# we1pingyu/CALD

Hardware: AMD Instinct MI355X
Metric: unlabeled images scored/sec (CALD consistency sweep) (higher is better)
Workload: dtype f32

## Files before the change

### cald_amd/_ffi.py

```python
import ctypes as C
import os

_HERE = os.path.dirname(os.path.abspath(__file__))
LIB_PATH = os.path.join(_HERE, "lib", "libcaldhip.so")
_lib = None

c_f = C.POINTER(C.c_float)
c_i = C.POINTER(C.c_int)
c_i64 = C.POINTER(C.c_int64)
c_d = C.POINTER(C.c_double)
c_u8 = C.POINTER(C.c_uint8)
c_i8 = C.POINTER(C.c_int8)


class ModelCfg(C.Structure):
    _fields_ = [("arch", C.c_int), ("depth", C.c_int), ("num_classes", C.c_int), ("min_size", C.c_int),
                ("max_size", C.c_int), ("box_score_thresh", C.c_float), ("box_nms_thresh", C.c_float),
                ("detections_per_img", C.c_int), ("rpn_pre_nms_top_n", C.c_int), ("rpn_post_nms_top_n", C.c_int),
                ("rpn_nms_thresh", C.c_float), ("precision", C.c_int)]


PRECISION = {"fp32": 0, "f16x3": 1}


class View(C.Structure):
    _fields_ = [("image_dev", C.c_void_p), ("H", C.c_int), ("W", C.c_int), ("flip", C.c_int), ("nrect", C.c_int),
                ("rects", C.c_int * 16), ("noise_dev", C.c_void_p)]


class Dets(C.Structure):
    _fields_ = [("boxes_dev", C.c_void_p), ("scores_dev", C.c_void_p), ("labels_dev", C.c_void_p),
                ("props_dev", C.c_void_p), ("prob_max_dev", C.c_void_p), ("scores_cls_dev", C.c_void_p),
                ("count_dev", C.c_void_p), ("cap", C.c_int)]


MAX_AUGS = 32
N_MARGINS = 16
MARGIN_NAMES = ['rpn_topk', 'rpn_iou', 'rpn_order', 'rpn_trunc', 'rpn_small', 'roi_level', 'roi_edge', 'post_thr', 'post_iou', 'post_order',
                'post_cap', 'ref_subsample', 'argmax', 'zero_row', 'cutout', 'reserved']
MARGIN_NOISE_F16X3 = [2e-5, 2e-6, 2e-5, 2e-5, 1e-5, 1e-6, 1e-4, 5e-6, 2e-6, 5e-6, 5e-6, 5e-6, 2e-6, 5e-6, 2e-6, 0.0]
AUG_FLIP, AUG_GAUSS, AUG_COLOR_ADJUST, AUG_COLOR_SWAP, AUG_SALT_PEPPER, AUG_CUTOUT, AUG_RESIZE, AUG_ROTATE = range(1, 9)
MAX_NOISE_SEG = 16


class AugSpec(C.Structure):
    _fields_ = [("kind", C.c_int), ("param", C.c_double)]


class PackJob(C.Structure):
    _fields_ = [("weight", C.c_void_p), ("bias", C.c_void_p), ("bn_scale", C.c_void_p), ("bn_shift", C.c_void_p),
                ("Cout", C.c_int), ("Cin", C.c_int), ("KH", C.c_int), ("KW", C.c_int), ("CinK", C.c_int), ("mode", C.c_int),
                ("packed", C.c_void_p)]


class LLCfg(C.Structure):
    _fields_ = [("batch_views", C.c_int), ("levels", C.c_int * 4)]


class VaalCfg(C.Structure):
    _fields_ = [("bn_mode", C.c_int), ("batch_images", C.c_int)]


VAAL_BN_BATCH, VAAL_BN_RUNNING = 0, 1


class LossNetTensors(C.Structure):
    _fields_ = [("fc_w", C.c_void_p * 4), ("fc_b", C.c_void_p * 4), ("lin_w", C.c_void_p), ("lin_b", C.c_void_p)]


class SweepCfg(C.Structure):
    _fields_ = [("base_seed", C.c_uint64), ("bp", C.c_float), ("batch_images", C.c_int), ("n_augs", C.c_int),
                ("augs", AugSpec * MAX_AUGS)]


PROBE_MAX_VIEWS = 8
PROBE_MAX_RECTS = 8


class ConvProbe(C.Structure):
    _fields_ = [("V", C.c_int), ("in_hw", (C.c_int * 2) * PROBE_MAX_VIEWS), ("up_hw", (C.c_int * 2) * PROBE_MAX_VIEWS),
                ("dyn_rows", C.c_int * PROBE_MAX_VIEWS), ("has_dyn", C.c_int), ("gather", C.c_int), ("nrect", C.c_int * PROBE_MAX_VIEWS),
                ("rect", ((C.c_int * 4) * PROBE_MAX_RECTS) * PROBE_MAX_VIEWS),
                ("Cin", C.c_int), ("Cout", C.c_int), ("KH", C.c_int), ("KW", C.c_int), ("stride", C.c_int), ("pad", C.c_int),
                ("relu", C.c_int), ("in_relu", C.c_int), ("out_ld", C.c_int), ("cin_true", C.c_int),
                ("weight", c_f), ("bias", c_f), ("bn_scale", c_f), ("bn_shift", c_f), ("in_", c_f), ("in16", C.POINTER(C.c_uint32)),
                ("residual", c_f), ("up", c_f), ("ex16", C.c_int), ("mask", c_f), ("row_map", c_i),
                ("out", c_f), ("out_n", C.c_int64), ("out16", C.POINTER(C.c_uint32)), ("out16_n", C.c_int64),
                ("energy4", c_f), ("energy4_n", C.c_int64),
                ("head_w", c_f), ("head_b", c_f), ("head_out", c_f), ("head_out_n", C.c_int64), ("head_ld", C.c_int)]


PRUNE_PROBE_MAX_VIEWS = 8


class RpnPruneProbe(C.Structure):
    _fields_ = [("V", C.c_int), ("guard", C.c_int), ("hw", ((C.c_int * 2) * PRUNE_PROBE_MAX_VIEWS) * 2),
                ("pre_n", C.c_int), ("head_ld", C.c_int), ("c1", C.c_float * 3), ("c0", C.c_float * 3),
                ("energy", c_f * 2), ("exact", c_f * 2), ("head", c_f * 2), ("pnorm", c_f * 2),
                ("tau_key", C.POINTER(C.c_uint32)), ("row_map", (c_i * 2) * 2), ("nsel", c_i * 2),
                ("check", C.c_float * 2), ("stat", C.c_uint64 * 4)]


class WgradPlan(C.Structure):
    _fields_ = [("variant", C.c_int), ("reduce", C.c_int), ("MT", C.c_int), ("JT", C.c_int), ("S", C.c_longlong), ("chunk", C.c_longlong),
                ("csplit", C.c_longlong), ("rows_per_block", C.c_longlong), ("scratch_bytes", C.c_longlong),
                ("kernel", C.c_char * 48), ("reduce_kernel", C.c_char * 32)]


SIGNATURES = {
    "cald_last_error": (C.c_char_p, []),
    "cald_version": (C.c_int, []),
    "cald_ctx_create": (C.c_int, [C.c_int, C.c_void_p, C.POINTER(C.c_void_p)]),
    "cald_ctx_destroy": (C.c_int, [C.c_void_p]),
    "cald_ctx_sync": (C.c_int, [C.c_void_p]),
    "cald_model_create": (C.c_int, [C.c_void_p, C.POINTER(ModelCfg), C.POINTER(C.c_void_p)]),
    "cald_model_load_tensor": (C.c_int, [C.c_void_p, C.c_char_p, c_f, c_i64, C.c_int]),
    "cald_model_finalize": (C.c_int, [C.c_void_p]),
    "cald_model_set_rpn_prune": (C.c_int, [C.c_void_p, C.c_int, c_i]),
    "cald_model_set_rpn_prune_capture": (C.c_int, [C.c_void_p, C.c_int]),
    "cald_model_rpn_prune_bound": (C.c_int, [C.c_void_p, c_f, c_f]),
    "cald_model_set_rpn_prune_bound": (C.c_int, [C.c_void_p, c_f, c_f]),
    "cald_profile_prune_fallbacks": (C.c_int, [C.c_void_p, C.POINTER(C.c_int64)]),
    "cald_model_destroy": (C.c_int, [C.c_void_p]),
    "cald_forward": (C.c_int, [C.c_void_p, C.c_int, C.POINTER(View), C.POINTER(Dets)]),
    "cald_sweep": (C.c_int, [C.c_void_p, C.c_int, C.POINTER(C.c_void_p), c_i, c_i, c_i64, C.POINTER(SweepCfg), c_d, c_d]),
    "cald_sweep_audit": (C.c_int, [C.c_void_p, C.c_int, C.POINTER(C.c_void_p), c_i, c_i, c_i64, C.POINTER(SweepCfg), c_d, c_d, c_f]),
    "cald_sweep_ltc": (C.c_int, [C.c_void_p, C.c_int, C.POINTER(C.c_void_p), c_i, c_i, C.c_int, c_d]),
    "cald_sweep_ssm": (C.c_int, [C.c_void_p, C.c_int, C.POINTER(C.c_void_p), c_i, c_i, C.c_int, C.c_int64, c_i, c_i, c_f, c_f, c_i8, c_i64]),
    "cald_sweep_lsc": (C.c_int, [C.c_void_p, C.c_int, C.POINTER(C.c_void_p), c_i, c_i, c_i64, C.c_uint64, C.c_int, c_d]),
    "cald_lossnet_create": (C.c_int, [C.c_void_p, C.POINTER(C.c_void_p)]),
    "cald_lossnet_load_tensor": (C.c_int, [C.c_void_p, C.c_char_p, c_f, c_i64, C.c_int]),
    "cald_lossnet_finalize": (C.c_int, [C.c_void_p]),
    "cald_lossnet_destroy": (C.c_int, [C.c_void_p]),
    "cald_sweep_ll": (C.c_int, [C.c_void_p, C.c_void_p, C.c_int, C.POINTER(C.c_void_p), c_i, c_i, c_i, C.POINTER(LLCfg), c_d, c_f]),
    "cald_vaal_create": (C.c_int, [C.c_void_p, C.POINTER(C.c_void_p)]),
    "cald_vaal_load_tensor": (C.c_int, [C.c_void_p, C.c_char_p, c_f, c_i64, C.c_int]),
    "cald_vaal_finalize": (C.c_int, [C.c_void_p]),
    "cald_vaal_destroy": (C.c_int, [C.c_void_p]),
    "cald_sweep_vaal": (C.c_int, [C.c_void_p, C.c_void_p, C.c_int, C.POINTER(C.c_void_p), c_i, c_i, C.POINTER(VaalCfg), c_f, c_f]),
    "cald_op_vaal_resize": (C.c_int, [C.c_void_p, c_u8, C.c_int, C.c_int, c_f]),
    "cald_op_vaal_bn_relu": (C.c_int, [C.c_void_p, c_f, C.c_longlong, C.c_int, C.c_int, C.c_int, c_f, c_f, c_f]),
    "cald_op_vaal_fc_mu": (C.c_int, [C.c_void_p, C.c_int, c_f, c_f]),
    "cald_op_vaal_head": (C.c_int, [C.c_void_p, C.c_int, c_f, c_f]),
    "cald_train_gap": (C.c_int, [C.c_void_p, C.c_int, C.POINTER(C.c_void_p), c_i, C.c_void_p]),
    "cald_lossnet_train_fwd": (C.c_int, [C.c_void_p, C.c_int, C.c_int, C.POINTER(LossNetTensors), C.c_void_p, C.c_void_p, C.c_void_p]),
    "cald_lossnet_train_bwd": (C.c_int, [C.c_void_p, C.c_int, C.c_int, C.POINTER(LossNetTensors), C.c_void_p, C.c_void_p, C.c_void_p, C.c_void_p,
                                         C.POINTER(LossNetTensors), C.c_int, C.c_void_p]),
    "cald_loss_pred_loss": (C.c_int, [C.c_void_p, C.c_int, C.c_void_p, C.c_void_p, C.c_float, C.c_int, C.c_void_p, C.c_void_p, C.c_void_p, C.c_void_p]),
    "cald_op_gap": (C.c_int, [C.c_void_p, c_f, C.c_int, C.c_int, C.c_int, c_f]),
    "cald_op_lossnet": (C.c_int, [C.c_void_p, C.c_int, c_f, c_f]),
    "cald_op_consistency": (C.c_int, [C.c_void_p, C.c_int, c_f, c_f, c_f, C.c_int, c_f, c_f, c_f, C.c_int, C.c_float, c_f]),
    "cald_op_cls_corr": (C.c_int, [C.c_void_p, C.c_int, c_f, c_i64, C.c_int, c_f]),
    "cald_op_pil_resize": (C.c_int, [C.c_void_p, C.c_void_p, C.c_int, C.c_int, C.c_void_p, C.c_int, C.c_int]),
    "cald_op_cutout_rects": (C.c_int, [C.c_uint64, C.c_int, C.c_int, C.c_int, c_f, C.c_int, c_i, c_i]),
    "cald_op_cutout_geometry": (C.c_int, [C.c_int, C.c_int, C.c_int, C.c_int, C.c_int, c_i, C.c_int, c_i, c_i]),
    "cald_op_augment": (C.c_int, [C.c_void_p, C.c_int, C.c_double, C.c_uint64, C.c_void_p, C.c_int, C.c_int, C.c_int, c_f,
                                  C.c_void_p, c_f, c_i]),
    "cald_op_noise_stream": (C.c_int, [C.c_void_p, C.c_uint64, C.c_void_p, C.c_int, C.c_int, C.c_int, c_i, c_d, C.POINTER(C.c_void_p)]),
    "cald_op_frcnn_postprocess": (C.c_int, [C.c_void_p, C.c_int, C.c_int, c_f, c_f, c_f, C.c_int, C.c_int, C.c_int, C.c_int, C.c_float, C.c_float,
                                            C.c_int, c_f, c_f, c_i64, c_f, c_f, c_f, c_i]),
    "cald_op_frcnn_postprocess_min": (C.c_int, [C.c_void_p, C.c_int, C.c_int, c_f, c_f, c_f, C.c_int, C.c_int, C.c_int, C.c_int, C.c_float, C.c_float,
                                                C.c_int, C.c_float, c_f, c_f, c_i64, c_f, c_f, c_f, c_i]),
    "cald_op_ssm_postprocess": (C.c_int, [C.c_void_p, C.c_int, C.c_int, c_f, c_f, c_f, C.c_int, C.c_int, C.c_int, C.c_int, C.c_float, C.c_int,
                                          c_i, c_i, c_f, c_f, c_i8]),
    "cald_op_retina_postprocess": (C.c_int, [C.c_void_p, C.POINTER(c_f), C.POINTER(c_f), c_i, C.c_int, C.c_int, c_f] + [C.c_int] * 6
                                   + [C.c_float, C.c_float, C.c_int, c_f, c_f, c_i64, c_f, c_f, c_i]),
    "cald_op_rpn_prune": (C.c_int, [C.c_void_p, C.POINTER(RpnPruneProbe)]),
    "cald_op_roi_align": (C.c_int, [C.c_void_p, C.POINTER(c_f), c_i, C.c_int, C.c_int, c_f, c_f]),
    "cald_op_conv2d": (C.c_int, [C.c_void_p, c_f, C.c_int, C.c_int, C.c_int, c_f, C.c_int, C.c_int, C.c_int, C.c_int,
                                 C.c_int, c_f, c_f, c_f, c_f, C.c_int, c_f]),
    "cald_op_conv_probe": (C.c_int, [C.c_void_p, C.c_int, C.POINTER(ConvProbe), C.c_int, C.c_int, C.c_int, C.c_char_p, C.c_int]),
    "cald_op_mfma_f16": (C.c_int, [C.c_void_p, C.POINTER(C.c_uint16), C.POINTER(C.c_uint16), C.POINTER(C.c_uint32), C.POINTER(C.c_uint32), C.c_int64]),
    "cald_op_conv2d_f16x3": (C.c_int, [C.c_void_p, c_f, C.c_int, C.c_int, C.c_int, c_f, C.c_int, C.c_int, C.c_int, C.c_int,
                                       C.c_int, c_f, c_f, c_f, c_f, C.c_int, c_f]),
    "cald_op_conv_bench": (C.c_int, [C.c_void_p] + [C.c_int] * 12 + [c_d, c_d]),
    "cald_op_transform_size": (C.c_int, [C.c_int, C.c_int, C.c_int, C.c_int, c_i, c_i, c_i, c_i]),
    "cald_debug_tensor": (C.c_int, [C.c_void_p, C.c_char_p, C.c_int, c_f, C.c_int64, c_i64]),
    "cald_jpeg_info": (C.c_int, [C.c_void_p, C.c_size_t, c_i, c_i, c_i]),
    "cald_jpeg_decode_batch": (C.c_int, [C.c_void_p, C.c_int, C.POINTER(C.c_void_p), C.POINTER(C.c_size_t), C.POINTER(C.c_void_p)]),
    "cald_jpeg_probe": (C.c_int, [C.c_void_p, C.c_size_t, c_i, c_i, c_i, c_i]),
    "cald_jpeg_decode_batch_any": (C.c_int, [C.c_void_p, C.c_int, C.POINTER(C.c_void_p), C.POINTER(C.c_size_t), C.POINTER(C.c_void_p)]),
    "cald_jpeg_decode_host": (C.c_int, [C.c_void_p, C.c_size_t, C.c_void_p]),
    "cald_profile_enable": (C.c_int, [C.c_void_p, C.c_int]),
    "cald_profile_read": (C.c_int, [C.c_void_p, c_d, c_d, c_i64, c_d]),
    "cald_profile_prune": (C.c_int, [C.c_void_p, c_d, c_d, c_d, c_d, c_d]),
    "cald_profile_roi_rows": (C.c_int, [C.c_void_p, c_d, c_i64]),
    "cald_profile_cutout": (C.c_int, [C.c_void_p, c_d, c_d, c_i64, c_i64]),
    "cald_model_set_cutout_reuse": (C.c_int, [C.c_void_p, C.c_int, c_i]),
    "cald_model_set_look_fuse": (C.c_int, [C.c_void_p, C.c_int, c_i]),
    "cald_model_set_box_min_size": (C.c_int, [C.c_void_p, C.c_float, c_f]),
    "cald_profile_dump": (C.c_int, [C.c_void_p, C.c_char_p]),
    "cald_train_packed_floats": (C.c_int, [C.c_int] * 6 + [c_i64]),
    "cald_train_pack_conv": (C.c_int, [C.c_void_p] * 5 + [C.c_int] * 6 + [C.c_void_p]),
    "cald_train_pack_plan_scratch_floats": (C.c_int, [C.c_int, C.POINTER(PackJob), c_i64]),
    "cald_train_pack_plan_create": (C.c_int, [C.c_void_p, C.c_int, C.POINTER(PackJob), C.c_void_p, C.c_int64, C.POINTER(C.c_void_p)]),
    "cald_train_pack_plan_run": (C.c_int, [C.c_void_p, C.c_void_p]),
    "cald_train_pack_plan_destroy": (C.c_int, [C.c_void_p]),
    "cald_train_conv": (C.c_int, [C.c_void_p, C.c_int, C.c_int, C.c_int, C.c_void_p, C.c_int, C.c_void_p] + [C.c_int] * 8
                        + [C.c_void_p, C.c_void_p, C.c_int, C.c_int, C.c_void_p, C.c_void_p, C.c_int]),
    "cald_train_conv_group": (C.c_int, [C.c_void_p, C.c_int, C.c_int, c_i, C.POINTER(C.c_void_p), C.c_int, C.POINTER(C.c_void_p)] + [C.c_int] * 8
                              + [C.POINTER(C.c_void_p), C.POINTER(C.c_void_p), C.c_int]),
    "cald_train_conv_wgrad": (C.c_int, [C.c_void_p, C.c_int, C.c_int, C.c_int, C.c_void_p, C.c_int, C.c_int, C.c_void_p, C.c_int,
                                        C.c_int, C.c_int, C.c_int, C.c_int, C.c_int, C.c_void_p, C.c_void_p, C.c_void_p, C.c_int]),
    "cald_train_linear_wgrad": (C.c_int, [C.c_void_p, C.c_int, C.c_void_p, C.c_int, C.c_void_p, C.c_int, C.c_int, C.c_int,
                                          C.c_void_p, C.c_void_p, C.c_int]),
    "cald_train_wgrad_plan": (C.c_int, [C.c_longlong] + [C.c_int] * 12 + [C.POINTER(WgradPlan)]),
    "cald_train_relu_bwd": (C.c_int, [C.c_void_p, C.c_longlong, C.c_int, C.c_void_p, C.c_void_p, C.c_void_p]),
    "cald_train_add": (C.c_int, [C.c_void_p, C.c_longlong, C.c_void_p, C.c_void_p, C.c_void_p]),
    "cald_train_dilate": (C.c_int, [C.c_void_p] + [C.c_int] * 7 + [C.c_void_p, C.c_void_p]),
    "cald_train_upsample_bwd": (C.c_int, [C.c_void_p] + [C.c_int] * 6 + [C.c_void_p, C.c_void_p]),
    "cald_train_rpn_proposals": (C.c_int, [C.c_void_p, C.c_int, C.c_int, C.c_int, c_i, C.POINTER(C.c_void_p), c_i, C.c_int, C.c_int, C.c_int,
                                           C.c_float, C.c_float, C.c_void_p, C.c_void_p]),
    "cald_train_roi_sample_host": (C.c_int, [C.c_int, c_i, c_i, c_i, C.c_void_p, C.c_void_p, C.c_void_p, C.c_int, C.c_double, C.c_int, C.c_int,
                                             C.c_void_p, C.c_void_p, C.c_void_p, C.c_void_p, C.c_void_p, C.c_void_p, c_i, c_i, c_i]),
    "cald_train_roi_gather": (C.c_int, [C.c_void_p, C.c_void_p, C.c_void_p, C.c_void_p, C.c_int, C.c_int, C.c_int] + [C.c_float] * 4 + [C.c_void_p, C.c_void_p]),
    "cald_train_anchors": (C.c_int, [C.c_void_p, C.c_int, C.c_int, C.c_int, c_i, C.c_void_p]),
    "cald_train_match": (C.c_int, [C.c_void_p, C.c_int, C.c_void_p, C.c_int, C.c_void_p, C.c_float, C.c_float, C.c_int, C.c_void_p, C.c_void_p]),
    "cald_train_box_encode": (C.c_int, [C.c_void_p, C.c_int, C.c_void_p, C.c_void_p, C.c_float, C.c_float, C.c_float, C.c_float, C.c_void_p]),
    "cald_train_roi_align": (C.c_int, [C.c_void_p, C.POINTER(C.c_void_p), c_i, C.c_int, C.c_int, C.c_void_p, C.c_void_p]),
    "cald_train_roi_align_bwd": (C.c_int, [C.c_void_p, C.c_int, C.POINTER(C.c_void_p), c_i, C.c_int, C.c_int, C.c_void_p, C.c_void_p]),
    "cald_train_softmax_ce": (C.c_int, [C.c_void_p, C.c_int, C.c_int, C.c_int, C.c_void_p, C.c_void_p, C.c_float, C.c_void_p, C.c_void_p]),
    "cald_train_smooth_l1": (C.c_int, [C.c_void_p, C.c_int, C.c_void_p, C.c_void_p, C.c_void_p, C.c_float, C.c_float, C.c_void_p, C.c_float,
                                       C.c_void_p, C.c_void_p]),
    "cald_train_focal_loss": (C.c_int, [C.c_void_p, C.c_int, c_i, C.c_int, C.c_int, C.c_int, C.c_void_p, C.c_void_p, C.c_void_p, C.c_void_p,
                                        C.c_void_p, C.c_float, C.c_float, C.c_void_p, C.c_void_p]),
    "cald_train_bce_logits": (C.c_int, [C.c_void_p, C.c_int, C.c_void_p, C.c_void_p, C.c_void_p, C.c_float, C.c_void_p, C.c_void_p]),
    "cald_train_softmax_ce_seg": (C.c_int, [C.c_void_p, C.c_int, c_i, C.c_int, C.c_int, C.c_void_p, C.c_void_p, C.c_void_p, C.c_void_p, C.c_void_p]),
    "cald_train_smooth_l1_seg": (C.c_int, [C.c_void_p, C.c_int, c_i, C.c_void_p, C.c_void_p, C.c_void_p, C.c_float, c_f, C.c_void_p, C.c_void_p,
                                           C.c_void_p]),
    "cald_train_bce_logits_seg": (C.c_int, [C.c_void_p, C.c_int, c_i, C.c_void_p, C.c_void_p, C.c_void_p, C.c_void_p, C.c_void_p, C.c_void_p]),
    "cald_train_focal_loss_seg": (C.c_int, [C.c_void_p, C.c_int, c_i, C.c_int, C.c_int, C.c_int, C.c_void_p, C.c_void_p, C.c_void_p, C.c_void_p,
                                            c_f, C.c_float, C.c_void_p, C.c_void_p, C.c_void_p, C.c_void_p]),
    "cald_train_seg_mean": (C.c_int, [C.c_void_p, C.c_int, C.c_void_p, C.c_void_p]),
    "cald_train_add_bcast": (C.c_int, [C.c_void_p, C.c_int, C.c_longlong, C.c_int, C.c_void_p, C.c_void_p, C.c_void_p, C.c_void_p, C.c_longlong]),
    "cald_train_preprocess": (C.c_int, [C.c_void_p, C.c_int, C.POINTER(C.c_void_p), C.POINTER(C.c_void_p), c_i, C.c_int, C.c_int, C.c_void_p]),
    "cald_train_maxpool": (C.c_int, [C.c_void_p, C.c_int, C.c_int, C.c_int, C.c_int, C.c_void_p, C.c_void_p]),
    "cald_train_subsample2": (C.c_int, [C.c_void_p, C.c_int, C.c_int, C.c_int, C.c_int, C.c_void_p, C.c_void_p]),
    "cald_train_sgd": (C.c_int, [C.c_void_p, C.c_longlong, C.c_void_p, C.c_void_p, C.c_void_p, C.c_float, C.c_float, C.c_float, C.c_int]),
    "cald_train_seg_cache_size": (C.c_int, []),
    "cald_comm_unique_id": (C.c_int, [C.c_void_p]),
    "cald_comm_init_rank": (C.c_int, [C.c_void_p, C.c_void_p, C.c_int, C.c_int, C.POINTER(C.c_void_p)]),
    "cald_comm_adopt": (C.c_int, [C.c_void_p, C.c_void_p, C.POINTER(C.c_void_p)]),
    "cald_comm_info": (C.c_int, [C.c_void_p, c_i, c_i]),
    "cald_comm_destroy": (C.c_int, [C.c_void_p]),
    "cald_allgather_scores": (C.c_int, [C.c_void_p, C.c_void_p, C.c_void_p, C.c_int64, C.c_int]),
}


def lib():
    global _lib
    if _lib is None:
        if not os.path.exists(LIB_PATH):
            raise RuntimeError("libcaldhip.so is not built (%s missing): run `python -c 'import __graft_entry__ as g; "
                               "g.build()'` or `make -C cald_amd/csrc`; there is no CPU fallback" % LIB_PATH)
        import torch
        L = C.CDLL(LIB_PATH, mode=C.RTLD_GLOBAL)
        for name, (res, args) in SIGNATURES.items():
            fn = getattr(L, name)
            fn.restype = res
            fn.argtypes = args
        _lib = L
    return _lib


ERR_UNSUPPORTED = -5


def check(rc):
    if rc == ERR_UNSUPPORTED:
        raise NotImplementedError("libcaldhip: %s (code %d)" % (lib().cald_last_error().decode(), rc))
    if rc != 0:
        raise RuntimeError("libcaldhip: %s (code %d)" % (lib().cald_last_error().decode(), rc))


def ptr(a, t=c_f):
    return a.ctypes.data_as(t) if a is not None else None
```

### cald_amd/csrc/common.h

```cpp
#pragma once
#include <hip/hip_runtime.h>
#include <stdint.h>
#include <math.h>

#define CALD_MAX_VIEWS 128
#define CALD_MAX_LEVELS 9
#define CALD_ROI_CAP 1000
#define CALD_MAX_CUT 4

struct LevelSeg {
    long long pix_off;
    int H, W;
    int tile_start;
    int pad_;
};

#if defined(__HIPCC__)
__device__ __forceinline__ int seg_find_view(const LevelSeg* __restrict__ seg, const int V, const int mt) {
    int lo = 0, hi = V - 1;
    while (lo < hi) {
        const int mid = (lo + hi + 1) >> 1;
        if (seg[mid].tile_start <= mt) lo = mid; else hi = mid - 1;
    }
    return lo;
}
#endif

struct BatchPlan {
    LevelSeg seg[CALD_MAX_LEVELS][CALD_MAX_VIEWS + 1];
};

#define CALD_GATHER_RECTS 8
struct GatherSet {
    int nr;
    int cum[CALD_GATHER_RECTS + 1];
    int x0[CALD_GATHER_RECTS], y0[CALD_GATHER_RECTS], w[CALD_GATHER_RECTS];
};
__device__ __forceinline__ int gather_pixel(const GatherSet& g, const int m, const int W) {
    int k = 0;
    while (k + 1 < g.nr && m >= g.cum[k + 1]) k++;
    const int j = m - g.cum[k], w = g.w[k], ry = j / w;
    return (g.y0[k] + ry) * W + g.x0[k] + (j - ry * w);
}

struct ConvArgs {
    const float* in;
    float* out;
    const float* w;
    const float* w4;
    const void* w16;
    float w16_unscale;
    const float* bias;
    const float* scale;
    const float* shift;
    const float* residual;
    const float* up;
    const LevelSeg* seg_in;
    const LevelSeg* seg_out;
    const LevelSeg* seg_up;
    const int* dyn_rows;
    const int* row_map;
    int V;
    int Cin, Cout, CoutPad, Kpad;
    int KH, KW, stride, pad;
    int relu;
    int total_mtiles;
    int out_ld;
    const float* zeros;
    int in_relu;
    const float* mask;
    const float* wstem;
    const unsigned* in16;
    unsigned* out16;
    float* energy4;
    int ex16;
    unsigned long long* trace;
    const GatherSet* gather;
    const float* head_w;
    float head_b[3];
    float* head_out;
    int head_ld;
};

#define CALD_MAX_GROUP 10
struct ConvGroup {
    int n;
    int blk0[CALD_MAX_GROUP + 1];
    ConvArgs p[CALD_MAX_GROUP];
};
static_assert(sizeof(ConvGroup) <= 4096, "ConvGroup is passed by value: it must fit the kernel argument segment");

__host__ __device__ inline int conv_k_index(int tap, int ci, int taps, int cinp) {
    return (cinp % 16 == 0 && taps <= 32) ? ((ci >> 4) * taps + tap) * 16 + (ci & 15) : tap * cinp + ci;
}
__host__ __device__ inline int round_up(int x, int m) { return (x + m - 1) / m * m; }
__host__ __device__ inline int cout_pad(int cout) { return cout >= 128 ? round_up(cout, 128) : (cout >= 64 ? round_up(cout, 64) : round_up(cout, 32)); }

__host__ __device__ inline float det_bits2f(uint32_t u) {
    union { uint32_t u; float f; } c; c.u = u; return c.f;
}
__host__ __device__ inline uint32_t det_f2bits(float f) {
    union { uint32_t u; float f; } c; c.f = f; return c.u;
}

__host__ __device__ inline float det_expf(float x) {
    if (x != x) return x;
    if (x > 88.72283f) return INFINITY;
    if (x < -87.0f) return 0.0f;
    float n = rintf(x * 1.44269504f);
    float r = fmaf(n, -0.693145752f, x);
    r = fmaf(n, -1.42860677e-6f, r);
    float p = 1.9875691500e-4f;
    p = fmaf(p, r, 1.3981999507e-3f);
    p = fmaf(p, r, 8.3334519073e-3f);
    p = fmaf(p, r, 4.1665795894e-2f);
    p = fmaf(p, r, 1.6666665459e-1f);
    p = fmaf(p, r, 5.0000001201e-1f);
    float r2 = r * r;
    float y = fmaf(p, r2, r) + 1.0f;
    int ni = (int)n;
    int n1 = ni / 2, n2 = ni - n1;
    y = y * det_bits2f((uint32_t)(n1 + 127) << 23);
    y = y * det_bits2f((uint32_t)(n2 + 127) << 23);
    return y;
}

__host__ __device__ inline float det_logf(float x) {
    if (x != x) return x;
    if (x < 0.0f) return NAN;
    if (x == 0.0f) return -INFINITY;
    if (x == INFINITY) return x;
    int e = 0;
    uint32_t u = det_f2bits(x);
    if (u < 0x00800000u) { x = x * 8388608.0f; u = det_f2bits(x); e = -23; }
    e += (int)(u >> 23) - 126;
    float m = det_bits2f((u & 0x007fffffu) | 0x3f000000u);
    float f;
    if (m < 0.70710678f) { e -= 1; f = (m + m) - 1.0f; } else { f = m - 1.0f; }
    float z = f * f;
    float p = 7.0376836292e-2f;
    p = fmaf(p, f, -1.1514610310e-1f);
    p = fmaf(p, f, 1.1676998740e-1f);
    p = fmaf(p, f, -1.2420140846e-1f);
    p = fmaf(p, f, 1.4249322787e-1f);
    p = fmaf(p, f, -1.6668057665e-1f);
    p = fmaf(p, f, 2.0000714765e-1f);
    p = fmaf(p, f, -2.4999993993e-1f);
    p = fmaf(p, f, 3.3333331174e-1f);
    float y = (p * f) * z;
    float fe = (float)e;
    y = fmaf(fe, -2.12194440e-4f, y);
    y = fmaf(z, -0.5f, y);
    float r = f + y;
    r = fmaf(fe, 0.693359375f, r);
    return r;
}
__host__ __device__ inline void det_sincosf(float x, float* s, float* c) {
    float q = rintf(x * 0.636619772f);
    float r = fmaf(q, -1.5703125f, x);
    r = fmaf(q, -4.837512969970703125e-4f, r);
    r = fmaf(q, -7.54978995489188216e-8f, r);
    float z = r * r;
    float ps = -1.9515295891e-4f;
    ps = fmaf(ps, z, 8.3321608736e-3f);
    ps = fmaf(ps, z, -1.6666654611e-1f);
    float sn = fmaf(ps * z, r, r);
    float pc = 2.443315711809948e-5f;
    pc = fmaf(pc, z, -1.388731625493765e-3f);
    pc = fmaf(pc, z, 4.166664568298827e-2f);
    float cs = fmaf(pc * z, z, fmaf(z, -0.5f, 1.0f));
    int qi = ((int)q) & 3;
    float ss = (qi & 1) ? cs : sn, cc = (qi & 1) ? sn : cs;
    if (qi == 2 || qi == 3) ss = -ss;
    if (qi == 1 || qi == 2) cc = -cc;
    *s = ss; *c = cc;
}
__host__ __device__ inline float det_log2f(float x) { return det_logf(x) * 1.44269504f; }
__host__ __device__ inline float det_sigmoidf(float x) { return 1.0f / (1.0f + det_expf(-x)); }

#ifdef __HIPCC__
__device__ __forceinline__ unsigned split16_word(const float x) {
    const float s = x * 16.0f;
    const _Float16 hi = (_Float16)s;
    const _Float16 lo = (_Float16)(s - (float)hi);
    return (unsigned)__builtin_bit_cast(unsigned short, hi) | ((unsigned)__builtin_bit_cast(unsigned short, lo) << 16);
}
__device__ __forceinline__ uint4 split16_word4(const float4 v) {
    return make_uint4(split16_word(v.x), split16_word(v.y), split16_word(v.z), split16_word(v.w));
}
#endif

#define BBOX_XFORM_CLIP_F 4.135166556742356f

__host__ __device__ inline void det_box_decode(const float* box, const float* d, float wx, float wy, float ww,
                                               float wh, float* o) {
    float width = box[2] - box[0], height = box[3] - box[1];
    float cx = box[0] + 0.5f * width, cy = box[1] + 0.5f * height;
    float dx = d[0] / wx, dy = d[1] / wy, dw = d[2] / ww, dh = d[3] / wh;
    if (dw > BBOX_XFORM_CLIP_F) dw = BBOX_XFORM_CLIP_F;
    if (dh > BBOX_XFORM_CLIP_F) dh = BBOX_XFORM_CLIP_F;
    float pcx = dx * width + cx, pcy = dy * height + cy;
    float pw = det_expf(dw) * width, ph = det_expf(dh) * height;
    o[0] = pcx - 0.5f * pw; o[1] = pcy - 0.5f * ph; o[2] = pcx + 0.5f * pw; o[3] = pcy + 0.5f * ph;
}
__host__ __device__ inline float det_clamp(float v, float lo, float hi) { return v < lo ? lo : (v > hi ? hi : v); }

__host__ __device__ inline uint32_t det_orderable(float f) {
    uint32_t u = det_f2bits(f);
    if ((u << 1) == 0u) u = 0u;
    return (u & 0x80000000u) ? ~u : (u | 0x80000000u);
}

#include <atomic>
struct PerDeviceOnce {
    std::atomic<bool> done[64];
    PerDeviceOnce() { for (auto& d : done) d.store(false); }
    bool first() {
        int dev = 0;
        if (hipGetDevice(&dev) != hipSuccess || dev < 0 || dev >= 64) return true;
        return !done[dev].exchange(true);
    }
};
template <typename K> static inline void allow_big_lds(PerDeviceOnce& once, K kernel) {
    if (once.first())
        hipFuncSetAttribute(reinterpret_cast<const void*>(kernel), hipFuncAttributeMaxDynamicSharedMemorySize, 160 * 1024 - 2048);
}

enum ConvPath { CONV_AUTO = 0, CONV_P4, CONV_P4_GROUP, CONV_P4_FUSED, CONV_GENERIC, CONV_STEM, CONV_H3, CONV_H3_GROUP, CONV_H4, CONV_H4_GROUP };
enum ConvTile { TILE_AUTO = 0, TILE_NARROW, TILE_WIDE };
struct ConvForce { int path = CONV_AUTO; int tile = TILE_AUTO; };

const char* launch_conv(const ConvArgs& a, hipStream_t stream, ConvForce f = ConvForce());
int launch_conv_group(const ConvArgs* probs, int n, hipStream_t stream, const char** names = nullptr, ConvForce f = ConvForce());
const char* launch_conv_p4(const ConvArgs& a, hipStream_t stream, ConvForce f = ConvForce());
// ... 10 lines not shown
```

### cald_amd/csrc/conv_p4.hip

```cpp
#include "h16.h"

typedef float f32x16 __attribute__((ext_vector_type(16)));
typedef int i32x4 __attribute__((ext_vector_type(4)));
typedef float f32x4 __attribute__((ext_vector_type(4)));

template <int EPI, bool MASK, int TM, int TN, bool GATHER = false>
__device__ __forceinline__ void p4_epilogue(const ConvArgs& a, const f32x16 (&acc)[TM][TN], float* smem, const int v, const LevelSeg& so,
                                            const int m0, const int Mv, const int n0) {
    constexpr int BM = 128, WN = 2;
    const int tid = threadIdx.x, lane = tid & 63, wave = tid >> 6;
    const int wm = wave / WN, wn = wave % WN;
    const int kh_lane = lane >> 5, l31 = lane & 31;
    const int Ho = so.H, Wo = so.W;
    const int out_ld = a.out_ld;
    float* __restrict__ out_v = a.out + so.pix_off * (long long)out_ld;
    const float* __restrict__ ex_v = nullptr;
    int upH = 1, upW = 1;
    float uph_s = 0.f, upw_s = 0.f;
    if (EPI == 1) ex_v = a.residual + so.pix_off * (long long)out_ld;
    if (EPI == 2) {
        const LevelSeg su = a.seg_up[v];
        ex_v = a.up + su.pix_off * (long long)out_ld;
        upH = su.H; upW = su.W;
        uph_s = (float)upH / (float)Ho; upw_s = (float)upW / (float)Wo;
    }
    const bool relu = a.relu != 0, has_bias = a.bias != nullptr, has_bn = a.scale != nullptr;
    constexpr bool has_mask = MASK;
    const float* __restrict__ mask_v = has_mask ? a.mask + so.pix_off * (long long)out_ld : out_v;
    const int row_b = out_ld * 4;
    const unsigned long long vb64 = (unsigned long long)(GATHER ? Ho * Wo : Mv) * (unsigned)row_b;
    const unsigned valid_b = vb64 < 0x7FFE0000ull ? (unsigned)vb64 : 0x7FFE0000u;
    const __amdgpu_buffer_rsrc_t rsO = __builtin_amdgcn_make_buffer_rsrc((void*)out_v, 0, valid_b, 0x00020000);
    const __amdgpu_buffer_rsrc_t rsX = __builtin_amdgcn_make_buffer_rsrc((void*)(EPI != 0 ? ex_v : out_v), 0, EPI == 1 ? valid_b : 0x7FFE0000, 0x00020000);
    const __amdgpu_buffer_rsrc_t rsM = __builtin_amdgcn_make_buffer_rsrc((void*)mask_v, 0, valid_b, 0x00020000);
    static_assert(!(GATHER && EPI == 2), "gathered rows take no top-down term");
    const int Mlast = Mv - 1;
    int* const s_src = reinterpret_cast<int*>(smem);
    if (EPI == 2 || GATHER) {
        if (tid < BM) {
            int m = m0 + tid;
            if (GATHER) {
                s_src[tid] = m < Mv ? gather_pixel(a.gather[v], m, Wo) * row_b : 0x7FFF0000;
            } else {
                m = m < Mlast ? m : Mlast;
                const int oy = m / Wo, ox = m - oy * Wo;
                int sy = (int)floorf((float)oy * uph_s); sy = sy > upH - 1 ? upH - 1 : sy;
                int sx = (int)floorf((float)ox * upw_s); sx = sx > upW - 1 ? upW - 1 : sx;
                s_src[tid] = (sy * upW + sx) * out_ld * 4;
            }
        }
        __syncthreads();
    }
    auto gather_offs = [&](const int i, const int n, const bool nok, int (&go)[16]) {
        const int rl = wm * TM * 32 + i * 32 + 4 * kh_lane;
#pragma unroll
        for (int q = 0; q < 4; q++) {
            const i32x4 so4 = *reinterpret_cast<const i32x4*>(s_src + rl + 8 * q);
#pragma unroll
            for (int jj = 0; jj < 4; jj++) go[4 * q + jj] = nok ? so4[jj] + n * 4 : 0x7FFF0000;
        }
    };
    constexpr bool EXTRA = EPI == 0 && !MASK && !GATHER;
    const bool want16 = EXTRA && a.out16 != nullptr, wantE = EXTRA && TN == 2 && a.energy4 != nullptr;
    unsigned char* const out16_v = want16 ? reinterpret_cast<unsigned char*>(a.out16) + so.pix_off * (long long)out_ld * 4 : nullptr;
    const __amdgpu_buffer_rsrc_t rsS = __builtin_amdgcn_make_buffer_rsrc((void*)(want16 ? (void*)out16_v : (void*)out_v), 0, valid_b, 0x00020000);
    const bool odd = (lane & 1) != 0;
    float sq[TM][16];
    if (EXTRA) {
#pragma unroll
        for (int i = 0; i < TM; i++)
#pragma unroll
            for (int r = 0; r < 16; r++) sq[i][r] = 0.0f;
    }
    float bs_[TN], sc_[TN], sh_[TN];
#pragma unroll
    for (int j = 0; j < TN; j++) {
        const int n = n0 + wn * TN * 32 + j * 32 + l31;
        const int nc = n < a.Cout ? n : 0;
        bs_[j] = has_bias ? a.bias[nc] : 0.0f;
        sc_[j] = has_bn ? a.scale[nc] : 1.0f;
        sh_[j] = has_bn ? a.shift[nc] : 0.0f;
    }
    constexpr int NTILE = TM * TN, PRE = GATHER ? 1 : NTILE;
    float extra_[EPI != 0 ? NTILE : 1][16];
    auto load_extra = [&](const int t, float (&extra)[16]) {
        const int j = t / TM, i = t - j * TM;
        const int n = n0 + wn * TN * 32 + j * 32 + l31;
        const bool nok = n < a.Cout;
        const int nc = nok ? n : 0;
        const int mbase = m0 + wm * TM * 32 + i * 32 + 4 * kh_lane;
        if (EPI == 1 && GATHER) {
            int go[16];
            gather_offs(i, n, nok, go);
#pragma unroll
            for (int r = 0; r < 16; r++) extra[r] = __builtin_bit_cast(float, __builtin_amdgcn_raw_buffer_load_b32(rsX, go[r], 0, 0));
        } else if (EPI == 1) {
            const int vo = nok ? (mbase * out_ld + n) * 4 : 0x7FFF0000;
#pragma unroll
            for (int r = 0; r < 16; r++)
                extra[r] = __builtin_bit_cast(float, __builtin_amdgcn_raw_buffer_load_b32(rsX, vo, ((r & 3) + 8 * (r >> 2)) * row_b, 0));
        } else if (EPI == 2) {
            const int rl = wm * TM * 32 + i * 32 + 4 * kh_lane;
#pragma unroll
            for (int q = 0; q < 4; q++) {
                const i32x4 so4 = *reinterpret_cast<const i32x4*>(s_src + rl + 8 * q);
#pragma unroll
                for (int jj = 0; jj < 4; jj++)
                    extra[4 * q + jj] = __builtin_bit_cast(float, __builtin_amdgcn_raw_buffer_load_b32(rsX, so4[jj] + nc * 4, 0, 0));
            }
        }
    };
    if (EPI != 0) {
#pragma unroll
        for (int t = 0; t < PRE; t++) load_extra(t, extra_[EPI != 0 ? t : 0]);
    }
#pragma unroll
    for (int j = 0; j < TN; j++) {
        const int n = n0 + wn * TN * 32 + j * 32 + l31;
        const bool nok = n < a.Cout;
        const int nc = nok ? n : 0;
        const float bs = bs_[j], sc = sc_[j], sh = sh_[j];
#pragma unroll
        for (int i = 0; i < TM; i++) {
            const int mbase = m0 + wm * TM * 32 + i * 32 + 4 * kh_lane;
            const float (&extra)[16] = extra_[EPI != 0 ? j * TM + i : 0];
            float val[16];
#pragma unroll
            for (int r = 0; r < 16; r++) val[r] = acc[i][j][r];
            if (has_bias) {
#pragma unroll
                for (int r = 0; r < 16; r++) val[r] = val[r] + bs;
            }
            if (has_bn) {
#pragma unroll
                for (int r = 0; r < 16; r++) { val[r] = val[r] * sc; val[r] = val[r] + sh; }
            }
            if (EPI != 0) {
#pragma unroll
                for (int r = 0; r < 16; r++) val[r] = val[r] + extra[r];
            }
            if (relu) {
#pragma unroll
                for (int r = 0; r < 16; r++) val[r] = val[r] > 0.0f ? val[r] : 0.0f;
            }
            if (EPI != 0 && j * TM + i + PRE < NTILE) load_extra(j * TM + i + PRE, extra_[EPI != 0 ? j * TM + i + PRE : 0]);
            const int vo = nok ? (mbase * out_ld + n) * 4 : 0x7FFF0000;
            if (has_mask) {
                float mk[16];
#pragma unroll
                for (int r = 0; r < 16; r++)
                    mk[r] = __builtin_bit_cast(float, __builtin_amdgcn_raw_buffer_load_b32(rsM, vo, ((r & 3) + 8 * (r >> 2)) * row_b, 0));
#pragma unroll
                for (int r = 0; r < 16; r++) val[r] = mk[r] > 0.0f ? val[r] : 0.0f;
            }
            if (GATHER) {
                int go[16];
                gather_offs(i, n, nok, go);
#pragma unroll
                for (int r = 0; r < 16; r++) __builtin_amdgcn_raw_buffer_store_b32(__builtin_bit_cast(unsigned, val[r]), rsO, go[r], 0, 0);
            } else {
#pragma unroll
                for (int r = 0; r < 16; r++)
                    __builtin_amdgcn_raw_buffer_store_b32(__builtin_bit_cast(unsigned, val[r]), rsO, vo, ((r & 3) + 8 * (r >> 2)) * row_b, 0);
            }
            if (EXTRA) {
                if (wantE) {
#pragma unroll
                    for (int r = 0; r < 16; r++) sq[i][r] = sq[i][r] + (nok ? val[r] * val[r] : 0.0f);
                }
                if (want16) {
                    const int poff = h16_pair_off(nc);
#pragma unroll
                    for (int r = 0; r < 16; r++) {
                        const unsigned w = h16_split(val[r]);
                        const unsigned pw = h16_pair_word(w, h16_partner(w), odd);
                        __builtin_amdgcn_raw_buffer_store_b32(pw, rsS, nok ? mbase * row_b + poff : 0x7FFF0000, ((r & 3) + 8 * (r >> 2)) * row_b, 0);
                    }
                }
            }
        }
    }
    if (EXTRA) {
        if (wantE) {
            __syncthreads();
            float* const red = smem + wave * (64 * 33);
#pragma unroll
            for (int i = 0; i < TM; i++)
#pragma unroll
                for (int r = 0; r < 16; r++) red[(i * 32 + 4 * kh_lane + (r & 3) + 8 * (r >> 2)) * 33 + l31] = sq[i][r];
            asm volatile("s_waitcnt lgkmcnt(0)" ::: "memory");
            float e = 0.0f;
#pragma unroll
            for (int q = 0; q < 32; q++) e = e + red[lane * 33 + q];
            const int m = m0 + wm * TM * 32 + lane;
            if (m < Mv) a.energy4[(so.pix_off + m) * 4 + (n0 / (64 * TN)) * 2 + wn] = e;
        }
    }
}

template <int EPIX, bool C4, int TN, int TAPS>
__device__ __forceinline__ void conv_p4_body(const ConvArgs& a, const int blk, const ConvArgs* a3 = nullptr) {
    constexpr int EPI = EPIX & 3;
    constexpr bool MASK = (EPIX & 4) != 0;
    constexpr bool FUSE = (EPIX & 8) != 0;
    constexpr bool GATHER = (EPIX & 16) != 0;
    static_assert(!(GATHER && (FUSE || MASK || C4)), "gathered rows: plain EPI 0 / 1 kernels only");
    constexpr int BM = 128, BN = 64 * TN, BK = 16, TM = 2, WN = 2;
    constexpr int TILE_A = 2 * BM * 8, TILE_F = TILE_A + 2 * BN * 8;
    constexpr int FUSE_T = 4 * TILE_A;
    __shared__ __attribute__((aligned(16))) float smem[FUSE ? FUSE_T + 4096 : 3 * TILE_F];

    const int tid = threadIdx.x, lane = tid & 63, wave = tid >> 6;
    const int wm = wave / WN, wn = wave % WN;
    const int NT = a.CoutPad / BN;
    unsigned long long* const trace = (a.trace && blockIdx.x < (1u << 17)) ? a.trace + (size_t)blockIdx.x * 8 : nullptr;
    if (trace && tid == 0) {
        trace[0] = __builtin_amdgcn_s_memtime();
        trace[5] = (unsigned)__builtin_amdgcn_s_getreg((31 << 11) | 4);
        trace[6] = (unsigned)__builtin_amdgcn_s_getreg((31 << 11) | 20);
        trace[7] = blockIdx.x;
    }
    int mt, nt;
    if (a.KH * a.KW > 1) {
        const int MT = a.total_mtiles, CH = (MT + 7) >> 3;
        const int xcd = blk & 7, idx = blk >> 3;
        mt = xcd * CH + idx / NT; nt = idx % NT;
        if (idx / NT >= CH || mt >= MT) return;
    } else {
        const int b = blk, MT = a.total_mtiles, MT8 = MT & ~7;
        if (b < MT8 * NT) { const int xcd = b & 7, idx = b >> 3; mt = (idx / NT) * 8 + xcd; nt = idx % NT; }
        else { const int r = b - MT8 * NT; mt = MT8 + r / NT; nt = r % NT; }
    }
    const int n0 = nt * BN;
    const int v = seg_find_view(a.seg_out, a.V, mt);
    const LevelSeg so = a.seg_out[v];
    const LevelSeg si = a.seg_in[v];
    const int Ho = so.H, Wo = so.W, Hi = si.H, Wi = si.W;
    int Mv = Ho * Wo;
    if (a.dyn_rows) { const int d = a.dyn_rows[v]; Mv = d < Mv ? d : Mv; }
    if (GATHER) Mv = a.gather[v].cum[a.gather[v].nr];
    const int m0 = (mt - so.tile_start) * BM;
    if (m0 >= Mv) return;
    const float* __restrict__ in_v = a.in + si.pix_off * (long long)a.Cin;
    const int Cin = a.Cin, KW = a.KW, KH = a.KH, CoutPad = a.CoutPad;
    const bool in_relu = a.in_relu != 0;

    const int g = tid & 3, arow = tid >> 2;
    unsigned rowmask[2];
    int rowvoff[2], riy0[2], rix0[2];
#pragma unroll
    for (int p = 0; p < 2; p++) {
        const int m = m0 + arow + 64 * p;
        const int mp = GATHER ? (m < Mv ? gather_pixel(a.gather[v], m, Wo) : 0) : (a.row_map && m < Mv) ? a.row_map[so.pix_off + m] : m;
        const int oy = mp / Wo, ox = mp - oy * Wo;
        const int iy0 = oy * a.stride - a.pad, ix0 = ox * a.stride - a.pad;
        unsigned msk = 0;
        if (!C4 && m < Mv)
            for (int t = 0; t < KH * KW; t++) {
                const int th = t / KW, tw = t - th * KW;
                const int iy = iy0 + th, ix = ix0 + tw;
                if (iy >= 0 && iy < Hi && ix >= 0 && ix < Wi) msk |= 1u << t;
            }
        rowmask[p] = msk;
        rowvoff[p] = (((oy * a.stride) * Wi + ox * a.stride) * Cin + (C4 ? 0 : 4 * g)) * 4;
        riy0[p] = m < Mv ? iy0 : -0x40000000; rix0[p] = ix0;
    }
    const __amdgpu_buffer_rsrc_t rsA = __builtin_amdgcn_make_buffer_rsrc(
        (void*)(in_v - (long long)a.pad * (Wi + 1) * Cin), 0, 0x7FFE0000, 0x00020000);
    const __amdgpu_buffer_rsrc_t rsB = __builtin_amdgcn_make_buffer_rsrc((void*)(a.w4 + (long long)n0 * 8), 0, 0x7FFE0000, 0x00020000);
    int u_kh = 0, u_kw = 0, u_ci = 0, u_kt = 0;
    const int a_kq = g >> 1, a_j = 2 * (g & 1);
    int aw_off[2][2];
#pragma unroll
    for (int p = 0; p < 2; p++) {
        const int r = arow + 64 * p;
#pragma unroll
        for (int h = 0; h < 2; h++) aw_off[p][h] = ((a_kq * BM + r) * 2 + (h ^ ((r >> 3) & 1))) * 4 + a_j;
    }
    const int b_t = TN == 2 ? tid : (tid & 127), b_kq = TN == 2 ? 0 : (tid >> 7);
    const int b_nl = b_t >> 1, b_h = b_t & 1;
    const int bvoff0 = (b_kq * CoutPad * 8 + b_nl * 8 + b_h * 4) * 4, bvoff1 = bvoff0 + CoutPad * 8 * 4;
    const int bw_off0 = TILE_A + ((b_kq * BN + b_nl) * 2 + (b_h ^ ((b_nl >> 3) & 1))) * 4, bw_off1 = bw_off0 + BN * 8;

    f32x4 ra0, ra1, rb0, rb1 = {0.f, 0.f, 0.f, 0.f};

#define P4_LOAD()                                                                                          \
    {                                                                                                      \
        const int soffB = u_kt * 2 * CoutPad * 8 * 4;                                                      \
        int soffA, v0, v1;                                                                                 \
        if (C4) {                                                                                          \
            const int tap = u_kt * 4 + g, th = tap / KW, tw = tap - th * KW;                               \
            const int toff = (th * Wi + tw) * 16;                                                          \
            const bool ok0 = th < KH && (unsigned)(riy0[0] + th) < (unsigned)Hi && (unsigned)(rix0[0] + tw) < (unsigned)Wi; \
            const bool ok1 = th < KH && (unsigned)(riy0[1] + th) < (unsigned)Hi && (unsigned)(rix0[1] + tw) < (unsigned)Wi; \
            soffA = 0;                                                                                     \
            v0 = ok0 ? rowvoff[0] + toff : 0x7FFF0000;                                                     \
            v1 = ok1 ? rowvoff[1] + toff : 0x7FFF0000;                                                     \
        } else {                                                                                           \
            const unsigned u_bit = 1u << (u_kh * KW + u_kw);                                               \
            soffA = ((u_kh * Wi + u_kw) * Cin + u_ci) * 4;                                                 \
            v0 = (rowmask[0] & u_bit) ? rowvoff[0] : 0x7FFF0000;                                           \
            v1 = (rowmask[1] & u_bit) ? rowvoff[1] : 0x7FFF0000;                                           \
        }                                                                                                  \
        ra0 = __builtin_bit_cast(f32x4, __builtin_amdgcn_raw_buffer_load_b128(rsA, v0, soffA, 0));         \
        ra1 = __builtin_bit_cast(f32x4, __builtin_amdgcn_raw_buffer_load_b128(rsA, v1, soffA, 0));         \
        rb0 = __builtin_bit_cast(f32x4, __builtin_amdgcn_raw_buffer_load_b128(rsB, bvoff0, soffB, 0));     \
        if (TN == 2) rb1 = __builtin_bit_cast(f32x4, __builtin_amdgcn_raw_buffer_load_b128(rsB, bvoff1, soffB, 0)); \
        u_kt++;                                                                                            \
                                        \
        u_kw++; if (u_kw == KW) { u_kw = 0; u_kh++; if (u_kh == KH) { u_kh = 0; u_ci += BK; } }            \
    }
#define P4_STORE(BUF)                                                                                      \
    {                                                                                                      \
        if (in_relu) {                                                                                     \
            _Pragma("unroll") for (int q = 0; q < 4; q++) { ra0[q] = ra0[q] < 0.f ? 0.f : ra0[q]; ra1[q] = ra1[q] < 0.f ? 0.f : ra1[q]; } \
        }                                                                                                  \
        float* tb = smem + (BUF) * TILE_F;                                                                 \
        *reinterpret_cast<float2*>(tb + aw_off[0][0]) = make_float2(ra0[0], ra0[2]);                       \
        *reinterpret_cast<float2*>(tb + aw_off[0][1]) = make_float2(ra0[1], ra0[3]);                       \
        *reinterpret_cast<float2*>(tb + aw_off[1][0]) = make_float2(ra1[0], ra1[2]);                       \
        *reinterpret_cast<float2*>(tb + aw_off[1][1]) = make_float2(ra1[1], ra1[3]);                       \
        *reinterpret_cast<f32x4*>(tb + bw_off0) = rb0;                                                     \
        if (TN == 2) *reinterpret_cast<f32x4*>(tb + bw_off1) = rb1;                                        \
    }

    f32x16 acc[TM][TN];
#pragma unroll
    for (int i = 0; i < TM; i++)
#pragma unroll
        for (int j = 0; j < TN; j++)
#pragma unroll
            for (int r = 0; r < 16; r++) acc[i][j][r] = 0.0f;

    const int KT = a.Kpad / BK;
    int voffA[2][TAPS > 0 ? TAPS : 1];
    int ci_ld = 0;
    if (TAPS == 13) {
#pragma unroll
        for (int p = 0; p < 2; p++)
#pragma unroll
            for (int t = 0; t < 13; t++) {
                const int tap = 4 * t + g, th = tap / 7, tw = tap - th * 7;
                const bool ok = th < 7 && (unsigned)(riy0[p] + th) < (unsigned)Hi && (unsigned)(rix0[p] + tw) < (unsigned)Wi;
                voffA[p][t] = ok ? rowvoff[p] + (th * Wi + tw) * 16 : 0x7FFF0000;
            }
    } else if (TAPS > 0) {
#pragma unroll
        for (int p = 0; p < 2; p++)
#pragma unroll
            for (int t = 0; t < (TAPS > 0 ? TAPS : 1); t++) voffA[p][t] = ((rowmask[p] >> t) & 1u) ? rowvoff[p] : 0x7FFF0000;
    }
    if (TAPS == 0) {
        P4_LOAD();
        P4_STORE(0);
        if (KT > 1) P4_LOAD();
    } else {
#define U_LOAD0(T)                                                                                         \
    {                                                                                                      \
        const int soffB = u_kt * 2 * CoutPad * 8 * 4;                                                      \
        const int soffA = (TAPS == 9 ? ((((T) / 3) * Wi + ((T) % 3)) * Cin + ci_ld) : ci_ld) * 4;          \
        ra0 = __builtin_bit_cast(f32x4, __builtin_amdgcn_raw_buffer_load_b128(rsA, voffA[0][T], soffA, 0)); \
        ra1 = __builtin_bit_cast(f32x4, __builtin_amdgcn_raw_buffer_load_b128(rsA, voffA[1][T], soffA, 0)); \
        rb0 = __builtin_bit_cast(f32x4, __builtin_amdgcn_raw_buffer_load_b128(rsB, bvoff0, soffB, 0));     \
        if (TN == 2) rb1 = __builtin_bit_cast(f32x4, __builtin_amdgcn_raw_buffer_load_b128(rsB, bvoff1, soffB, 0)); \
        u_kt++;                                                                                            \
        if ((T) == TAPS - 1) ci_ld += BK;                                                                  \
    }
        U_LOAD0(0)
        P4_STORE(0);
        if (KT > 1) U_LOAD0((TAPS == 9 || TAPS == 13) ? 1 : 0)
#undef U_LOAD0
    }
    asm volatile("s_waitcnt lgkmcnt(0)" ::: "memory");
    __builtin_amdgcn_s_barrier();
    if (trace && tid == 0) trace[1] = __builtin_amdgcn_s_memtime();

    const int kh_lane = lane >> 5, l31 = lane & 31;
    int fo_a[TM], fo_b[TN];
#pragma unroll
    for (int t = 0; t < TM; t++) { const int m = wm * 64 + t * 32 + l31; fo_a[t] = (m * 2 + (kh_lane ^ ((m >> 3) & 1))) * 4; }
#pragma unroll
    for (int t = 0; t < TN; t++) { const int n = wn * 32 * TN + t * 32 + l31; fo_b[t] = TILE_A + (n * 2 + (kh_lane ^ ((n >> 3) & 1))) * 4; }
    f32x4 fa0[TM], fb0[TN], fa1[TM], fb1[TN];
#pragma unroll
    for (int t = 0; t < TM; t++) fa0[t] = *reinterpret_cast<const f32x4*>(smem + fo_a[t]);
#pragma unroll
    for (int t = 0; t < TN; t++) fb0[t] = *reinterpret_cast<const f32x4*>(smem + fo_b[t]);

#define P4_MFMA(FA, FB, Q)                                                                                 \
    _Pragma("unroll") for (int i = 0; i < TM; i++)                                                         \
        _Pragma("unroll") for (int j = 0; j < TN; j++)                                                     \
            acc[i][j] = __builtin_amdgcn_mfma_f32_32x32x2f32(FA[i][Q], FB[j][Q], acc[i][j], 0, 0, 0);
#define P4_TILE(CUR, NXT)                                                                                  \
    {                                                                                                      \
        const float* tc = smem + (CUR) * TILE_F;                                                           \
        const float* tn = smem + (NXT) * TILE_F;                                                           \
        const bool has1 = kt + 1 < KT, has2 = kt + 2 < KT;                                                 \
        _Pragma("unroll") for (int t = 0; t < TM; t++) fa1[t] = *reinterpret_cast<const f32x4*>(tc + fo_a[t] + BM * 8); \
        _Pragma("unroll") for (int t = 0; t < TN; t++) fb1[t] = *reinterpret_cast<const f32x4*>(tc + fo_b[t] + BN * 8); \
        P4_MFMA(fa0, fb0, 0)                                                                               \
        P4_MFMA(fa0, fb0, 1)                                                                               \
        if (has1) P4_STORE(NXT)                                                                            \
        P4_MFMA(fa0, fb0, 2)                                                                               \
        if (has2) P4_LOAD()                                                                                \
        P4_MFMA(fa0, fb0, 3)                                                                               \
        P4_MFMA(fa1, fb1, 0)                                                                               \
        P4_MFMA(fa1, fb1, 1)                                                                               \
        asm volatile("s_waitcnt lgkmcnt(0)" ::: "memory");                                                 \
        __builtin_amdgcn_s_barrier();                                                                      \
        if (has1) {                                                                                        \
            _Pragma("unroll") for (int t = 0; t < TM; t++) fa0[t] = *reinterpret_cast<const f32x4*>(tn + fo_a[t]); \
            _Pragma("unroll") for (int t = 0; t < TN; t++) fb0[t] = *reinterpret_cast<const f32x4*>(tn + fo_b[t]); \
        }                                                                                                  \
        P4_MFMA(fa1, fb1, 2)                                                                               \
        P4_MFMA(fa1, fb1, 3)                                                                               \
    }

    if (TAPS == 0) {
        int cur = 0;
        for (int kt = 0; kt < KT; kt++) {
            const int nxtb = cur == 2 ? 0 : cur + 1;
            P4_TILE(cur, nxtb);
            cur = nxtb;
        }
    } else {
        unsigned awa[3][4];
#pragma unroll
        for (int b = 0; b < 3; b++) {
            awa[b][0] = (unsigned)(uintptr_t)(smem + b * TILE_F + aw_off[0][0]); awa[b][1] = (unsigned)(uintptr_t)(smem + b * TILE_F + aw_off[0][1]);
            awa[b][2] = (unsigned)(uintptr_t)(smem + b * TILE_F + aw_off[1][0]); awa[b][3] = (unsigned)(uintptr_t)(smem + b * TILE_F + aw_off[1][1]);
        }
        float* const bwp0 = smem + bw_off0; float* const bwp1 = smem + bw_off1;
        const float* fpa[TM]; const float* fpb[TN];
#pragma unroll
        for (int t = 0; t < TM; t++) fpa[t] = smem + fo_a[t];
#pragma unroll
        for (int t = 0; t < TN; t++) fpb[t] = smem + fo_b[t];
#define U_LOAD(T)                                                                                          \
    {                                                                                                      \
        const int soffB = u_kt * 2 * CoutPad * 8 * 4;                                                      \
        const int soffA = (TAPS == 9 ? ((((T) / 3) * Wi + ((T) % 3)) * Cin + ci_ld) : ci_ld) * 4;          \
        ra0 = __builtin_bit_cast(f32x4, __builtin_amdgcn_raw_buffer_load_b128(rsA, voffA[0][T], soffA, 0)); \
        ra1 = __builtin_bit_cast(f32x4, __builtin_amdgcn_raw_buffer_load_b128(rsA, voffA[1][T], soffA, 0)); \
        rb0 = __builtin_bit_cast(f32x4, __builtin_amdgcn_raw_buffer_load_b128(rsB, bvoff0, soffB, 0));     \
        if (TN == 2) rb1 = __builtin_bit_cast(f32x4, __builtin_amdgcn_raw_buffer_load_b128(rsB, bvoff1, soffB, 0)); \
        u_kt++;                                                                                            \
        if ((T) == TAPS - 1) ci_ld += BK;                                                                  \
    }
#define U_W2(ADDR, D0, D1)                                                                                 \
    asm volatile("ds_write2_b32 %0, %1, %2 offset1:1" ::"v"(ADDR), "v"(D0), "v"(D1) : "memory");
#define U_STORE(BUF)                                                                                       \
    {                                                                                                      \
        if (in_relu) {                                                                                     \
            _Pragma("unroll") for (int q = 0; q < 4; q++) { ra0[q] = ra0[q] < 0.f ? 0.f : ra0[q]; ra1[q] = ra1[q] < 0.f ? 0.f : ra1[q]; } \
        }                                                                                                  \
                                   \
        U_W2(awa[BUF][0], ra0[0], ra0[2]) U_W2(awa[BUF][1], ra0[1], ra0[3])                                \
        U_W2(awa[BUF][2], ra1[0], ra1[2]) U_W2(awa[BUF][3], ra1[1], ra1[3])                                \
        *reinterpret_cast<f32x4*>(bwp0 + (BUF) * TILE_F) = rb0;                                            \
        if (TN == 2) *reinterpret_cast<f32x4*>(bwp1 + (BUF) * TILE_F) = rb1;                               \
    }
#define U_TILE(CUR, NXT, TLD, KTX)                                                                         \
    {                                                                                                      \
        const bool has1 = (KTX) + 1 < KT, has2 = (KTX) + 2 < KT;                                           \
        _Pragma("unroll") for (int t = 0; t < TM; t++) fa1[t] = *reinterpret_cast<const f32x4*>(fpa[t] + (CUR) * TILE_F + BM * 8); \
        _Pragma("unroll") for (int t = 0; t < TN; t++) fb1[t] = *reinterpret_cast<const f32x4*>(fpb[t] + (CUR) * TILE_F + BN * 8); \
        P4_MFMA(fa0, fb0, 0)                                                                               \
        P4_MFMA(fa0, fb0, 1)                                                                               \
        if (has1) U_STORE(NXT)                                                                             \
        P4_MFMA(fa0, fb0, 2)                                                                               \
        if (has2) U_LOAD(TLD)                                                                              \
        P4_MFMA(fa0, fb0, 3)                                                                               \
        P4_MFMA(fa1, fb1, 0)                                                                               \
        P4_MFMA(fa1, fb1, 1)                                                                               \
        asm volatile("s_waitcnt lgkmcnt(0)" ::: "memory");                                                 \
        __builtin_amdgcn_s_barrier();                                                                      \
        if (has1) {                                                                                        \
            _Pragma("unroll") for (int t = 0; t < TM; t++) fa0[t] = *reinterpret_cast<const f32x4*>(fpa[t] + (NXT) * TILE_F); \
            _Pragma("unroll") for (int t = 0; t < TN; t++) fb0[t] = *reinterpret_cast<const f32x4*>(fpb[t] + (NXT) * TILE_F); \
        }                                                                                                  \
        P4_MFMA(fa1, fb1, 2)                                                                               \
        P4_MFMA(fa1, fb1, 3)                                                                               \
    }
        if (TAPS == 13) {
            U_TILE(0, 1, 2, 0)  U_TILE(1, 2, 3, 1)  U_TILE(2, 0, 4, 2)  U_TILE(0, 1, 5, 3)  U_TILE(1, 2, 6, 4)
            U_TILE(2, 0, 7, 5)  U_TILE(0, 1, 8, 6)  U_TILE(1, 2, 9, 7)  U_TILE(2, 0, 10, 8) U_TILE(0, 1, 11, 9)
            U_TILE(1, 2, 12, 10) U_TILE(2, 0, 12, 11) U_TILE(0, 1, 12, 12)
        } else if (TAPS == 9) {
            for (int kt = 0; kt < KT; kt += 9) {
                U_TILE(0, 1, 2, kt)     U_TILE(1, 2, 3, kt + 1) U_TILE(2, 0, 4, kt + 2)
                U_TILE(0, 1, 5, kt + 3) U_TILE(1, 2, 6, kt + 4) U_TILE(2, 0, 7, kt + 5)
                U_TILE(0, 1, 8, kt + 6) U_TILE(1, 2, 0, kt + 7) U_TILE(2, 0, 1, kt + 8)
            }
        } else {
            for (int kt = 0; kt < KT; kt += 3) {
                U_TILE(0, 1, 0, kt)
                if (kt + 1 < KT) U_TILE(1, 2, 0, kt + 1)
                if (kt + 2 < KT) U_TILE(2, 0, 0, kt + 2)
            }
        }
#undef U_LOAD
#undef U_STORE
#undef U_W2
#undef U_TILE
    }
#undef P4_LOAD
#undef P4_STORE
#undef P4_MFMA
#undef P4_TILE

    if (trace && tid == 0) trace[2] = __builtin_amdgcn_s_memtime();
    if constexpr (FUSE) {
        const ConvArgs& b = *a3;
        float* const Tl = smem;
        float* const Wl = smem + FUSE_T;
        {
            const int c = wn * 32 + l31;
            const float sc = a.scale ? a.scale[c] : 1.0f, sh = a.scale ? a.shift[c] : 0.0f, bs = a.bias ? a.bias[c] : 0.0f;
            const bool relu2 = a.relu != 0, has_bias2 = a.bias != nullptr, has_bn2 = a.scale != nullptr;
            float* const tc = Tl + (c >> 4) * TILE_A + ((c >> 3) & 1) * BM * 8 + ((c & 7) >> 1) + (wm * 64 + 4 * kh_lane) * 8;
            float* const tcb[2] = {tc + (c & 1) * 4, tc + ((c & 1) ^ 1) * 4};
#pragma unroll
            for (int i = 0; i < TM; i++)
#pragma unroll
                for (int r = 0; r < 16; r++) {
                    float val = acc[i][0][r];
                    if (has_bias2) val = val + bs;
                    if (has_bn2) { val = val * sc; val = val + sh; }
                    if (relu2) val = val > 0.0f ? val : 0.0f;
                    tcb[(r >> 2) & 1][(i * 32 + (r & 3) + 8 * (r >> 2)) * 8] = val;
                }
        }
        const int CoutPad3 = b.CoutPad;
        const LevelSeg so3 = b.seg_out[v];
        const int ld3 = b.out_ld;
        const bool relu3 = b.relu != 0;
        const __amdgpu_buffer_rsrc_t rsO3 = __builtin_amdgcn_make_buffer_rsrc((void*)(b.out + so3.pix_off * (long long)ld3), 0, Mv * ld3 * 4, 0x00020000);
        const __amdgpu_buffer_rsrc_t rsX3 = __builtin_amdgcn_make_buffer_rsrc((void*)(b.residual + so3.pix_off * (long long)ld3), 0, Mv * ld3 * 4, 0x00020000);
        int foa2[2], fob2;
#pragma unroll
        for (int t = 0; t < 2; t++) { const int m = wm * 64 + t * 32 + l31; foa2[t] = (m * 2 + (kh_lane ^ ((m >> 3) & 1))) * 4; }
        { const int n = wn * 32 + l31; fob2 = (n * 2 + (kh_lane ^ ((n >> 3) & 1))) * 4; }
        const int w_t = tid & 127, w_kq = tid >> 7, w_nl = w_t >> 1, w_h = w_t & 1;
        const int wvoff = (w_kq * CoutPad3 * 8 + w_nl * 8 + w_h * 4) * 4;
        const int ww_off = ((w_kq * 64 + w_nl) * 2 + (w_h ^ ((w_nl >> 3) & 1))) * 4;
        f32x4 wr[4];
        auto fetch_w = [&](int n0c) {
            const __amdgpu_buffer_rsrc_t rsW = __builtin_amdgcn_make_buffer_rsrc((void*)(b.w4 + (long long)n0c * 8), 0, 0x7FFE0000, 0x00020000);
#pragma unroll
            for (int kt = 0; kt < 4; kt++)
                wr[kt] = __builtin_bit_cast(f32x4, __builtin_amdgcn_raw_buffer_load_b128(rsW, wvoff, kt * 2 * CoutPad3 * 8 * 4, 0));
        };
        fetch_w(0);
        for (int n0c = 0; n0c < CoutPad3; n0c += 64) {
            if (n0c > 0) __syncthreads();
#pragma unroll
            for (int kt = 0; kt < 4; kt++) *reinterpret_cast<f32x4*>(Wl + kt * 1024 + ww_off) = wr[kt];
            __syncthreads();
            if (n0c + 64 < CoutPad3) fetch_w(n0c + 64);
            const int n3 = n0c + wn * 32 + l31;
            int vo3[2];
            float ex[2][16];
#pragma unroll
            for (int i = 0; i < 2; i++) vo3[i] = ((m0 + wm * 64 + i * 32 + 4 * kh_lane) * ld3 + n3) * 4;
#pragma unroll
            for (int i = 0; i < 2; i++)
#pragma unroll
                for (int r = 0; r < 16; r++)
                    ex[i][r] = __builtin_bit_cast(float, __builtin_amdgcn_raw_buffer_load_b32(rsX3, vo3[i], ((r & 3) + 8 * (r >> 2)) * ld3 * 4, 0));
            __builtin_amdgcn_sched_barrier(0);
            f32x16 acc2[2][1];
#pragma unroll
            for (int i = 0; i < 2; i++)
#pragma unroll
                for (int r = 0; r < 16; r++) acc2[i][0][r] = 0.0f;
#pragma unroll
            for (int kt = 0; kt < 4; kt++) {
                f32x4 ga0[2], ga1[2];
#pragma unroll
                for (int t = 0; t < 2; t++) {
                    ga0[t] = *reinterpret_cast<const f32x4*>(Tl + kt * TILE_A + foa2[t]);
                    ga1[t] = *reinterpret_cast<const f32x4*>(Tl + kt * TILE_A + foa2[t] + BM * 8);
                }
                const f32x4 gb0 = *reinterpret_cast<const f32x4*>(Wl + kt * 1024 + fob2);
                const f32x4 gb1 = *reinterpret_cast<const f32x4*>(Wl + kt * 1024 + fob2 + 64 * 8);
#pragma unroll
                for (int q = 0; q < 4; q++)
#pragma unroll
                    for (int i = 0; i < 2; i++) acc2[i][0] = __builtin_amdgcn_mfma_f32_32x32x2f32(ga0[i][q], gb0[q], acc2[i][0], 0, 0, 0);
#pragma unroll
                for (int q = 0; q < 4; q++)
#pragma unroll
                    for (int i = 0; i < 2; i++) acc2[i][0] = __builtin_amdgcn_mfma_f32_32x32x2f32(ga1[i][q], gb1[q], acc2[i][0], 0, 0, 0);
            }
            {
                const float sc3 = b.scale[n3], sh3 = b.shift[n3];
#pragma unroll
                for (int i = 0; i < 2; i++) {
#pragma unroll
                    for (int r = 0; r < 16; r++) {
                        float val = acc2[i][0][r] * sc3;
                        val = val + sh3;
                        val = val + ex[i][r];
                        if (relu3) val = val > 0.0f ? val : 0.0f;
                        __builtin_amdgcn_raw_buffer_store_b32(__builtin_bit_cast(unsigned, val), rsO3, vo3[i], ((r & 3) + 8 * (r >> 2)) * ld3 * 4, 0);
                    }
                }
            }
        }
    } else {
        p4_epilogue<EPI, MASK, TM, TN, GATHER>(a, acc, smem, v, so, m0, Mv, n0);
    }
    if (trace && tid == 0) {
        trace[3] = __builtin_amdgcn_s_memtime();
        asm volatile("s_waitcnt vmcnt(0)" ::: "memory");
        trace[4] = __builtin_amdgcn_s_memtime();
    }
}

template <int EPI, bool C4, int TN, int TAPS>
__global__ __launch_bounds__(256, 3) void conv_p4_kernel(const ConvArgs a) { conv_p4_body<EPI, C4, TN, TAPS>(a, blockIdx.x); }
template <int EPI, bool C4, int TN, int TAPS>
__global__ __launch_bounds__(256, 3) void conv_p4_group_kernel(const ConvGroup g) {
    int i = 0;
    while (i + 1 < g.n && g.blk0[i + 1] <= (int)blockIdx.x) i++;
    conv_p4_body<EPI, C4, TN, TAPS>(g.p[i], (int)blockIdx.x - g.blk0[i]);
}
__global__ __launch_bounds__(256, 3) void conv_p4_fused_kernel(const ConvGroup g) { conv_p4_body<8, false, 1, 9>(g.p[0], blockIdx.x, &g.p[1]); }

static inline int p4_taps(const ConvArgs& a) {
    if (a.Cin % 16 != 0) return 0;
    if (a.KH == 3 && a.KW == 3) return 9;
    if (a.KH == 1 && a.KW == 1) return 1;
    return 0;
}

static inline int p4_grid_mtiles(const ConvArgs& a) { return a.KH * a.KW > 1 ? 8 * ((a.total_mtiles + 7) / 8) : a.total_mtiles; }

static inline bool p4_refuses(const ConvArgs& a) {
    if (!a.w4 || !a.out || a.in16 || a.ex16 || a.CoutPad % 64 != 0 || (a.residual && a.up)) return true;
    const bool extra = a.out16 || a.energy4;
    if (extra && (a.residual || a.up || a.mask || a.gather)) return true;
    if (a.energy4 && a.CoutPad != 256) return true;
    if (a.row_map && (a.residual || a.up || a.mask || a.gather)) return true;
    return false;
}
static inline bool p4_tile_ok(const ConvArgs& a, const bool wide, const ConvForce f) {
    if (f.tile == TILE_NARROW && wide) return false;
    if (f.tile == TILE_WIDE && !wide) return false;
    return !(a.energy4 && !wide);
}

#define P4_NAME(K, EPIV, C4V, TNV, TAPSV) K "<" #EPIV "," #C4V "," #TNV "," #TAPSV ">"
template <int EPI, bool C4, int TN, int TAPS>
static const char* p4_go(const dim3 grid, hipStream_t stream, const ConvArgs& a, const char* name) {
    hipLaunchKernelGGL((conv_p4_kernel<EPI, C4, TN, TAPS>), grid, dim3(256), 0, stream, a);
    return name;
}
template <int EPI, int TN, int TAPS>
static const char* p4_group_go(const dim3 grid, hipStream_t stream, const ConvGroup& g, const char* name) {
    hipLaunchKernelGGL((conv_p4_group_kernel<EPI, false, TN, TAPS>), grid, dim3(256), 0, stream, g);
    return name;
}

const char* launch_conv_p4_group(const ConvArgs* p, int n, hipStream_t stream, ConvForce f) {
    if (n < 1 || n > CALD_MAX_GROUP) return nullptr;
    const bool wide = f.tile == TILE_NARROW ? false : p[0].CoutPad % 128 == 0;
    ConvGroup g; g.n = n; int blk = 0;
    for (int i = 0; i < n; i++) {
        const ConvArgs& a = p[i];
        if (p4_refuses(a) || !p4_tile_ok(a, wide, f) || (a.CoutPad % 128 == 0) != (p[0].CoutPad % 128 == 0)) return nullptr;
        if (a.Cin % 16 != 0 || a.KH * a.KW > 32 || a.residual || a.up || a.gather) return nullptr;
        if ((a.mask != nullptr) != (p[0].mask != nullptr)) return nullptr;
        if (a.mask && (a.out16 || a.energy4)) return nullptr;
        g.blk0[i] = blk; blk += p4_grid_mtiles(a) * (a.CoutPad / (wide ? 128 : 64)); g.p[i] = a;
    }
    g.blk0[n] = blk;
    const int taps = p4_taps(p[0]);
    for (int i = 1; i < n; i++) if (p4_taps(p[i]) != taps) return nullptr;
    const dim3 grid((unsigned)blk);
#define P4_GROUP(EV, TNV, TAPSV) p4_group_go<EV, TNV, TAPSV>(grid, stream, g, P4_NAME("conv_p4_group_kernel", EV, false, TNV, TAPSV))
#define P4_GROUP_T(EV) (wide ? (taps == 9 ? P4_GROUP(EV, 2, 9) : taps == 1 ? P4_GROUP(EV, 2, 1) : P4_GROUP(EV, 2, 0)) \
                             : (taps == 9 ? P4_GROUP(EV, 1, 9) : taps == 1 ? P4_GROUP(EV, 1, 1) : P4_GROUP(EV, 1, 0)))
    const char* name = p[0].mask ? P4_GROUP_T(4) : P4_GROUP_T(0);
#undef P4_GROUP_T
#undef P4_GROUP
    return name;
}

const char* launch_conv_p4_fused(const ConvArgs& c2, const ConvArgs& c3, hipStream_t stream) {
    if (!c2.w4 || !c3.w4 || c2.w16 || c3.w16) return nullptr;
    if (c2.KH != 3 || c2.KW != 3 || c2.stride != 1 || c2.pad != 1 || c2.Cin % 16 || c2.Cout != 64 || c2.CoutPad != 64 || c2.out_ld != 64) return nullptr;
    if (c2.residual || c2.up || c2.mask || c2.dyn_rows || c2.in_relu || c2.gather || c3.gather || p4_taps(c2) != 9) return nullptr;
    if (c3.KH != 1 || c3.KW != 1 || c3.stride != 1 || c3.pad != 0 || c3.Cin != 64 || c3.Kpad != 64 || c3.CoutPad % 64 || c3.Cout != c3.CoutPad) return nullptr;
    if (!c3.residual || !c3.scale || c3.bias || c3.out_ld != c3.Cout || c3.up || c3.mask || c3.dyn_rows || c3.in_relu || c3.in != c2.out || c3.total_mtiles != c2.total_mtiles || c3.V != c2.V) return nullptr;
    if (c2.row_map || c3.row_map || c2.in16 || c3.in16 || c2.out16 || c3.out16 || c2.energy4 || c3.energy4 || c2.ex16 || c3.ex16 || !c3.out) return nullptr;
    ConvGroup g; g.n = 2; g.blk0[0] = 0; g.p[0] = c2; g.p[1] = c3;
    const unsigned grid = (unsigned)p4_grid_mtiles(c2);
    hipLaunchKernelGGL(conv_p4_fused_kernel, dim3(grid), dim3(256), 0, stream, g);
    return "conv_p4_fused_kernel";
}

const char* launch_conv_p4(const ConvArgs& a, hipStream_t stream, ConvForce f) {
    if (p4_refuses(a)) return nullptr;
    bool wide = a.CoutPad % 128 == 0;
    if (wide) {
        const long long b2 = (long long)a.total_mtiles * (a.CoutPad / 128), b1 = 2 * b2;
        const double e2 = (double)b2 / (double)(((b2 + 767) / 768) * 768), e1 = 0.88 * (double)b1 / (double)(((b1 + 767) / 768) * 768);
        if (e1 > e2 && !a.dyn_rows && !a.energy4) wide = false;
    }
    if (f.tile == TILE_NARROW) wide = false;
    else if (f.tile == TILE_WIDE) wide = a.CoutPad % 128 == 0;
    if (!p4_tile_ok(a, wide, f)) return nullptr;
    const dim3 grid((unsigned)(p4_grid_mtiles(a) * (a.CoutPad / (wide ? 128 : 64))));
#define P4_ONE(EPIV, C4V, TNV, TAPSV) p4_go<EPIV, C4V, TNV, TAPSV>(grid, stream, a, P4_NAME("conv_p4_kernel", EPIV, C4V, TNV, TAPSV))
    if (a.gather) {
        const int taps = p4_taps(a);
        if (a.Cin == 4 || a.up || a.mask || a.in_relu || a.dyn_rows || a.row_map || (taps != 1 && taps != 9)) return nullptr;
        if (a.total_mtiles == 0) return "none (no gathered rows)";
#define P4_G(EPIV, TNV) (taps == 9 ? P4_ONE(EPIV, false, TNV, 9) : P4_ONE(EPIV, false, TNV, 1))
        return wide ? (a.residual ? P4_G(17, 2) : P4_G(16, 2)) : (a.residual ? P4_G(17, 1) : P4_G(16, 1));
#undef P4_G
    }
    if (a.Cin == 4) {
        if (a.residual || a.up || a.in_relu || a.mask) return nullptr;
        if (a.KH == 7 && a.KW == 7 && a.Kpad == 208)
            return wide ? P4_ONE(0, true, 2, 13) : P4_ONE(0, true, 1, 13);
        return wide ? P4_ONE(0, true, 2, 0) : P4_ONE(0, true, 1, 0);
    }
    if (a.Cin % 16 != 0 || a.KH * a.KW > 32) return nullptr;
    const int taps = p4_taps(a);
#define P4_TAPS(EPIV, TNV) (taps == 9 ? P4_ONE(EPIV, false, TNV, 9) : taps == 1 ? P4_ONE(EPIV, false, TNV, 1) : P4_ONE(EPIV, false, TNV, 0))
    const char* name;
    if (a.mask) {
        if (a.up) return nullptr;
        name = wide ? (a.residual ? P4_TAPS(5, 2) : P4_TAPS(4, 2)) : (a.residual ? P4_TAPS(5, 1) : P4_TAPS(4, 1));
    } else if (wide) {
        name = a.residual ? P4_TAPS(1, 2) : a.up ? P4_TAPS(2, 2) : P4_TAPS(0, 2);
    } else {
        name = a.residual ? P4_TAPS(1, 1) : a.up ? P4_TAPS(2, 1) : P4_TAPS(0, 1);
    }
#undef P4_TAPS
#undef P4_ONE
    return name;
}
#undef P4_NAME
```

### cald_amd/csrc/forward.hip

```cpp
#include "host.h"

#define ROI_DENSE_VIEWS 32
void cald_host::build_plan(BatchPlan& P, int V, const ViewDesc* views, const int (*hp)[2], bool retina) {
    memset(&P, 0, sizeof(P));
    for (int l = 0; l < CALD_MAX_LEVELS; l++) {
        long long off = 0; int tile = 0;
        for (int v = 0; v <= V; v++) {
            LevelSeg& s = P.seg[l][v];
            s.pix_off = off; s.tile_start = tile;
            if (v == V) break;
            int H, W;
            if (l == 7 && retina) { int h6 = (hp[v][0] / 32 - 1) / 2 + 1, w6 = (hp[v][1] / 32 - 1) / 2 + 1; H = (h6 - 1) / 2 + 1; W = (w6 - 1) / 2 + 1; }
            else if (l == 7) { H = 1; W = CALD_ROI_CAP; }
            else if (l == 8) {
                const int first = v * ROI_DENSE_VIEWS, cnt = first < V ? (V - first < ROI_DENSE_VIEWS ? V - first : ROI_DENSE_VIEWS) : 0;
                H = cnt ? 1 : 0; W = cnt * CALD_ROI_CAP;
            }
            else if (l == 6) { H = (hp[v][0] / 32 - 1) / 2 + 1; W = (hp[v][1] / 32 - 1) / 2 + 1; }
            else { H = hp[v][0] >> l; W = hp[v][1] >> l; }
            s.H = H; s.W = W;
            off += (long long)H * W;
            tile += (H * W + 127) / 128;
        }
    }
}
static int level_tiles(const BatchPlan& P, int l, int V) { return P.seg[l][V].tile_start; }

struct SplitReg {
    cald_model* m; Bump& B; bool on;
    void only(float* t) { if (on) m->split[t] = {reinterpret_cast<unsigned*>(t), true}; }
    void both(float* t, unsigned*& twin, size_t n) { if (on) { twin = B.get<unsigned>(n); m->split[t] = {twin, false}; } }
};
static const int CCH[4] = {256, 512, 1024, 2048};
struct BodyBufs {
    float *in0, *c1, *p1, *X[2], *T1, *T2, *D, *Cf[4];
    void layout(Bump& B, SplitReg& S, const long long* px) {
        in0 = B.get<float>(px[0] * 4); c1 = B.get<float>(px[1] * 64); p1 = B.get<float>(px[2] * 64);
        X[0] = B.get<float>(px[2] * 256); X[1] = B.get<float>(px[2] * 256);
        T1 = B.get<float>(px[2] * 128); T2 = B.get<float>(px[2] * 64); D = B.get<float>(px[2] * 256);
        for (int i = 0; i < 4; i++) { Cf[i] = B.get<float>(px[2 + i] * CCH[i]); S.only(Cf[i]); }
        S.only(p1); S.only(T1); S.only(T2); S.only(X[0]); S.only(X[1]); S.only(D);
    }
};
struct PyramidBufs {
    float *inner[4], *Pf[5]; unsigned* Pf16[5];
    void layout(Bump& B, SplitReg& S, const long long* px, bool retina) {
        const int first = retina ? 3 : 2, nl = retina ? 3 : 4;
        for (int i = 0; i < nl; i++) { inner[i] = B.get<float>(px[first + i] * 256); S.only(inner[i]); }
        for (int i = 0; i < 5; i++) {
            Pf[i] = B.get<float>(px[first + i] * 256);
            if (i == 4 || (retina && i < 3)) S.only(Pf[i]); else S.both(Pf[i], Pf16[i], px[first + i] * 256);
        }
    }
};
void cald_host::RetinaTailBufs::layout(Bump& B, int V, int K, int per_class, int maxa) {
    max_anchors = maxa;
    cand_cap = 1024; while (cand_cap < maxa) cand_cap <<= 1;
    cand_count = B.get<int>((size_t)V * K); cand_key = B.get<unsigned long long>((size_t)V * K * cand_cap);
    cand_box = B.get<float>((size_t)V * K * cand_cap * 4); cand_skip = B.get<unsigned char>((size_t)V * K * cand_cap);
    kept_anchor = B.get<int>((size_t)V * K * per_class); kept_box = B.get<float>((size_t)V * K * per_class * 4); kept_count = B.get<int>((size_t)V * K);
}
struct RetinaBufs {
    float *ret_t[2][2][5], *cls_h[5], *reg_h[5]; RetinaTailBufs tail;
    void layout(Bump& B, SplitReg& S, const long long* px, int V, int cls_ld, int K, int per_class, int max_anchors) {
        for (int h = 0; h < 2; h++) for (int q = 0; q < 2; q++) for (int i = 0; i < 5; i++) { ret_t[h][q][i] = B.get<float>(px[3 + i] * 256); S.only(ret_t[h][q][i]); }
        for (int i = 0; i < 5; i++) { cls_h[i] = B.get<float>(px[3 + i] * cls_ld); reg_h[i] = B.get<float>(px[3 + i] * 36); }
        tail.layout(B, V, K, per_class, max_anchors);
    }
};
void cald_host::ProposalBufs::layout(Bump& B, int V) { proposals = B.get<float>((size_t)V * CALD_ROI_CAP * 4); prop_count = B.get<int>(V); }
struct RpnBufs {
    float *rpn_tl[5], *rpn_h[5], *cand_box, *sorted_box, *sorted_raw; unsigned long long* cand_key; int* sorted_count; ProposalBufs prop;
    void layout(Bump& B, const long long* px, int V, int pre) {
        for (int i = 0; i < 5; i++) { rpn_tl[i] = B.get<float>(px[2 + i] * 256); rpn_h[i] = B.get<float>(px[2 + i] * 15); }
        cand_key = B.get<unsigned long long>((size_t)V * 5 * pre); cand_box = B.get<float>((size_t)V * 5 * pre * 4);
        sorted_box = B.get<float>((size_t)V * 5 * pre * 4); sorted_raw = B.get<float>((size_t)V * 5 * pre * 4); sorted_count = B.get<int>(V);
        prop.layout(B, V);
    }
};
struct PruneBufs {
    float *energy[2] = {}, *pn[2] = {}, *rows[2][2] = {}; int *map[2][2] = {}, *nsel[2] = {}; unsigned* p16[2] = {}; unsigned* tau = nullptr;
    float* look[2] = {};
    void layout(Bump& B, const long long* px, int V, bool capture) {
        for (int i = 0; i < 2; i++) {
            energy[i] = B.get<float>(px[2 + i] * 4); pn[i] = B.get<float>(px[2 + i]); p16[i] = B.get<unsigned>(px[2 + i] * 256);
            for (int s2 = 0; s2 < 2; s2++) { rows[s2][i] = B.get<float>(px[2 + i] * 15); map[s2][i] = B.get<int>(px[2 + i]); }
            if (capture) look[i] = B.get<float>(px[2 + i] * 15);
        }
        for (int s2 = 0; s2 < 2; s2++) nsel[s2] = B.get<int>((size_t)2 * V);
        tau = B.get<unsigned>((size_t)2 * V);
    }
};
void cald_host::RoiBufs::layout(Bump& B, int V, int C) { order = B.get<int>((size_t)V * 1024); roi = B.get<float>((size_t)V * CALD_ROI_CAP * 49 * C); }
void cald_host::PostBufs::layout(Bump& B, int V, int C, int cap) {
    key_cap = cap;
    prob = B.get<float>((size_t)V * CALD_ROI_CAP * C); pmax = B.get<float>((size_t)V * CALD_ROI_CAP);
    keys = B.get<unsigned long long>((size_t)V * key_cap); cbox = B.get<float>((size_t)V * 2 * key_cap * 4); key_count = B.get<int>(V);
    skip = B.get<unsigned char>((size_t)V * key_cap);
}
void cald_host::SsmBufs::layout(Bump& B, int V, int C, int cap) {
    const size_t K = (size_t)(C - 1), rows = (size_t)V * K * cap;
    prob = B.get<float>((size_t)V * CALD_ROI_CAP * C); vmax = B.get<unsigned>(V);
    kept_prop = B.get<int>(rows); kept_box = B.get<float>(rows * 4); cls_count = B.get<int>((size_t)V * K); row_off = B.get<int>((size_t)V * K);
    al = B.get<int>(V); count = B.get<int>(V); total = B.get<int>(1);
    boxes = B.get<float>(rows * 4); scores = B.get<float>(rows * K); labels = B.get<signed char>(rows * K);
}
struct BoxBufs {
    RoiBufs roi; float *f6, *f7, *pr; PostBufs post;
    void layout(Bump& B, SplitReg& S, int V, int pred_ld, int C, int key_cap) {
        roi.layout(B, V, 256);
        f6 = B.get<float>((size_t)V * CALD_ROI_CAP * 1024); f7 = B.get<float>((size_t)V * CALD_ROI_CAP * 1024);
        S.only(roi.roi); S.only(f6); S.only(f7);
        pr = B.get<float>((size_t)V * CALD_ROI_CAP * pred_ld);
        post.layout(B, V, C, key_cap);
    }
};
struct AuditBufs {
    unsigned long long *next_key, *trunc_key, *kept_key; float* post_maxc;
    void layout(Bump& B, int V, int det_cap) {
        next_key = B.get<unsigned long long>((size_t)V * 10); trunc_key = B.get<unsigned long long>((size_t)V * 2);
        kept_key = B.get<unsigned long long>((size_t)V * det_cap); post_maxc = B.get<float>(V);
    }
};

RoiArgs cald_host::roi_args(const RoiBufs& S, const float* const* feat, const BatchPlan* plan, int C, int V, const ProposalBufs& P, bool out16) {
    RoiArgs ro{};
    for (int i = 0; i < 4; i++) { ro.feat[i] = feat[i]; ro.seg[i] = plan->seg[2 + i]; }
    ro.C = C; ro.V = V; ro.proposals = P.proposals; ro.prop_count = P.prop_count; ro.out = S.roi; ro.order = S.order; ro.out16 = out16 ? 1 : 0;
    return ro;
}
PostArgs cald_host::post_args(const PostBufs& S, const float* pred, int pred_ld, int C, int V, const ProposalBufs& P, const ViewDesc* views,
                              float score_thr, float nms_thr, const DetBuffers& det) {
    PostArgs pa{};
    pa.pred = pred; pa.pred_ld = pred_ld; pa.C = C; pa.V = V; pa.proposals = P.proposals; pa.prop_count = P.prop_count; pa.views = views; pa.score_thr = score_thr; pa.nms_thr = nms_thr;
    pa.prob = S.prob; pa.pmax = S.pmax; pa.keys = S.keys; pa.cbox = S.cbox; pa.key_count = S.key_count; pa.key_cap = S.key_cap; pa.det = det;
    pa.skip = S.skip;
    return pa;
}
SsmArgs cald_host::ssm_args(const SsmBufs& S, const float* pred, int pred_ld, int C, int V, const ProposalBufs& P, const ViewDesc* views, float score_thr, int cap) {
    SsmArgs sa{};
    sa.pred = pred; sa.pred_ld = pred_ld; sa.C = C; sa.V = V; sa.proposals = P.proposals; sa.prop_count = P.prop_count; sa.views = views;
    sa.score_thr = score_thr; sa.nms_thr = SSM_NMS_THR; sa.conf_thr = SSM_CONF_THR; sa.cap = cap;
    sa.prob = S.prob; sa.vmax = S.vmax; sa.kept_prop = S.kept_prop; sa.kept_box = S.kept_box; sa.cls_count = S.cls_count; sa.row_off = S.row_off;
    sa.al = S.al; sa.count = S.count; sa.total = S.total; sa.boxes = S.boxes; sa.scores = S.scores; sa.labels = S.labels;
    return sa;
}
RetinaArgs cald_host::retina_args(const RetinaTailBufs& S, const float* const* cls, const float* const* reg, const BatchPlan* plan, const ViewDesc* views,
                                  const float* base_anchors, int A, int K, int V, float score_thr, float nms_thr, int per_class, const DetBuffers& det) {
    RetinaArgs ra{};
    for (int i = 0; i < 5; i++) { ra.cls[i] = cls[i]; ra.reg[i] = reg[i]; ra.seg[i] = plan->seg[3 + i]; }
    ra.seg0 = plan->seg[0]; ra.views = views; ra.base_anchors = base_anchors;
    ra.cls_ld = A * K; ra.reg_ld = A * 4; ra.A = A; ra.K = K; ra.V = V; ra.score_thr = score_thr; ra.nms_thr = nms_thr; ra.min_box = 1e-2f;
    ra.per_class = per_class; ra.cand_cap = S.cand_cap;
    ra.cand_count = S.cand_count; ra.cand_key = S.cand_key; ra.cand_box = S.cand_box; ra.cand_skip = S.cand_skip;
    ra.kept_anchor = S.kept_anchor; ra.kept_box = S.kept_box; ra.kept_count = S.kept_count; ra.det = det;
    return ra;
}

bool cald_host::stem_grid_exact(const LevelSeg* seg, int V) {
    for (int v = 0; v < V; v++) {
        const LevelSeg& s = seg[v];
        if (!(s.H % 8 == 0 && s.W % 16 == 0 && seg[v + 1].tile_start - s.tile_start == (s.H / 8) * (s.W / 16))) return false;
    }
    return true;
}
static double fill_conv_args(cald_model* m, ConvArgs& a, const ConvLayer& L, const float* in, float* out, int lin, int lout, int V, bool relu,
                             const float* residual = nullptr, const float* up = nullptr, int lup = 0, const int* dyn = nullptr,
                             bool in_relu = false) {
    const BatchPlan* dp = m->ctx->d_plan;
    a.in = in; a.out = out; a.w = L.w; a.w4 = L.w4; a.w16 = L.w16; a.w16_unscale = L.w16_unscale; a.bias = L.bias; a.scale = L.scale; a.shift = L.shift;
    a.residual = residual; a.up = up;
    a.seg_in = dp->seg[lin]; a.seg_out = dp->seg[lout]; a.seg_up = dp->seg[lup];
    a.dyn_rows = dyn; a.row_map = nullptr; a.gather = nullptr; a.V = V;
    a.Cin = L.Cin; a.Cout = L.Cout; a.CoutPad = L.CoutPad; a.Kpad = L.Kpad;
    a.KH = L.KH; a.KW = L.KW; a.stride = L.stride; a.pad = L.pad; a.relu = relu ? 1 : 0;
    a.total_mtiles = level_tiles(m->plan, lout, V);
    a.out_ld = L.Cout; a.in_relu = in_relu ? 1 : 0; a.zeros = m->ctx->d_zeros;
    a.mask = nullptr;
    for (int v = 0; v < V; v++) {
        const long long pin = (long long)m->plan.seg[lin][v].H * m->plan.seg[lin][v].W, pout = (long long)m->plan.seg[lout][v].H * m->plan.seg[lout][v].W;
        if (pin * L.Cin * 4 > 0x7FFE0000LL || pout * L.Cout * 4 > 0x7FFE0000LL) {
            return (double)fail(CALD_ERR_UNSUPPORTED, "a view's activation tensor exceeds 2 GB (level %d -> %d, %lld x %d / %lld x %d elements)", lin, lout, pin, L.Cin, pout, L.Cout);
        }
    }
    a.in16 = nullptr; a.out16 = nullptr; a.ex16 = 0; a.energy4 = nullptr; a.trace = nullptr;
    a.head_w = nullptr; a.head_out = nullptr; a.head_ld = 0; a.head_b[0] = a.head_b[1] = a.head_b[2] = 0.0f;
    if (!m->split.empty()) {
        const float* ex = residual ? residual : up;
        if (ex) {
            auto fe = m->split.find(ex);
            if (fe != m->split.end() && fe->second.fp32_dead) {
                if (!a.w16) return (double)fail(CALD_ERR_STATE, "a layer outside conv_h3 / conv_h4 adds a tensor kept in split form only");
                a.ex16 = 1;
            }
        }
        auto fi = m->split.find(in);
        if (fi != m->split.end()) {
            if (a.w16 && !in_relu) a.in16 = fi->second.s16;
            else if (fi->second.fp32_dead) return (double)fail(CALD_ERR_STATE, "a layer outside conv_h3 reads a tensor kept in split form only");
        }
        auto fo = m->split.find(out);
        if (fo != m->split.end()) {
            if (!a.w16) return (double)fail(CALD_ERR_STATE, "a layer outside conv_h3 writes a tensor with a split twin");
            a.out16 = fo->second.s16;
            if (fo->second.fp32_dead) a.out = nullptr;
        }
    }
    a.wstem = L.wstem && stem_grid_exact(m->plan.seg[lout], V) ? L.wstem : nullptr;
    return 2.0 * (double)level_pix(m->plan, lout, V) * (double)L.Cout * (double)(L.KH * L.KW * L.CinTrue);
}
static int conv_on(cald_model* m, const ConvLayer& L, const float* in, float* out, int lin, int lout, int V, bool relu,
                   const float* residual = nullptr, const float* up = nullptr, int lup = 0, const int* dyn = nullptr,
                   bool in_relu = false) {
    ConvArgs a;
    const double flops = fill_conv_args(m, a, L, in, out, lin, lout, V, relu, residual, up, lup, dyn, in_relu);
    if (flops < 0.0) return (int)flops;
    return run_conv(m->ctx, a, flops);
}
static int conv_pair_on(cald_model* m, const ConvLayer& L2, const ConvLayer& L3, const float* in, float* mid, float* out, int lin, int lout,
                        int V, const float* residual) {
    cald_ctx* c = m->ctx;
    if (m->cfg.precision == CALD_PRECISION_FP32 && L2.stride == 1 && lin == lout) {
        ConvArgs a2, a3;
            const double f2 = fill_conv_args(m, a2, L2, in, mid, lin, lout, V, true);
        const double f3 = fill_conv_args(m, a3, L3, mid, out, lout, lout, V, true, residual);
        if (f2 < 0.0 || f3 < 0.0) return (int)(f2 < 0.0 ? f2 : f3);
        ProfLaunch t; int rc;
        if ((rc = prof_begin(c, t))) return rc;
        if (launch_conv_p4_fused(a2, a3, c->stream) != nullptr)
            return prof_end(c, t, f2 + f3, 0, "mt=%d,Cin=%d,Cout=%d,k=3x3+1x1,s=1,fused->%d", a2.total_mtiles, a2.Cin, a2.Cout, a3.Cout);
        if (c->prof) { hipEventDestroy(t.e0); hipEventDestroy(t.e1); }
    }
    int rc = conv_on(m, L2, in, mid, lin, lout, V, true);
    if (rc) return rc;
    return conv_on(m, L3, mid, out, lout, lout, V, true, residual);
}
static int conv_group_on(cald_model* m, const ConvSpec* sp, int n, int V) {
    ConvArgs a[CALD_MAX_GROUP];
    double flops = 0.0; int tiles = 0;
    for (int i = 0; i < n; i++) {
        const double f = fill_conv_args(m, a[i], *sp[i].L, sp[i].in, sp[i].out, sp[i].level, sp[i].level, V, sp[i].relu, nullptr, nullptr, 0, sp[i].dyn);
        if (f < 0.0) return (int)f;
        a[i].row_map = sp[i].row_map;
        if (sp[i].in16) a[i].in16 = sp[i].in16;
        if (sp[i].out16) a[i].out16 = sp[i].out16;
        a[i].energy4 = sp[i].energy4;
        flops += f; tiles += a[i].total_mtiles;
    }
    cald_ctx* c = m->ctx;
    const char* names[CALD_MAX_GROUP];
    ProfLaunch t; int rc;
    if ((rc = prof_begin(c, t))) return rc;
    const int launches = launch_conv_group(a, n, c->stream, names);
    if (c->prof) c->prof_extra_launches += launches - 1;
    if ((rc = prof_end(c, t, flops, c->prof_tag_now, "mt=%d,Cin=%d,Cout=%d,k=%dx%d,s=%d,group=%d", tiles, a[0].Cin, a[0].Cout, a[0].KH, a[0].KW, a[0].stride, n))) return rc;
    for (int i = 0; i < n; i++) if (!names[i]) return conv_refused(a[i]);
    return 0;
}

static int gconv_on(cald_model* m, const ConvLayer& L, const float* in, float* out, int lin, int lout, int V, bool relu, const float* residual,
                    const FwdReuse& ru, int b, int kind) {
    if (!ru.tiles[b][kind]) return 0;
    ConvArgs a;
    const double f = fill_conv_args(m, a, L, in, out, lin, lout, V, relu, residual);
    if (f < 0.0) return (int)f;
    const char* base = ru.d_gp + (size_t)(2 * b + kind) * cut_plan_set_bytes(V);
    a.seg_out = reinterpret_cast<const LevelSeg*>(base);
    a.gather = reinterpret_cast<const GatherSet*>(base + (size_t)(V + 1) * sizeof(LevelSeg));
    a.total_mtiles = ru.tiles[b][kind];
    return run_conv(m->ctx, a, 2.0 * ru.rows[b][kind] * (double)L.Cout * (double)(L.KH * L.KW * L.CinTrue));
}

__global__ void accumulate_rows_kernel(const int* __restrict__ counts, int V, unsigned long long* acc) {
    unsigned long long s = 0;
    for (int v = threadIdx.x; v < V; v += 64) s += (unsigned long long)counts[v];
    for (int o = 32; o > 0; o >>= 1) s += __shfl_down(s, o);
    if (threadIdx.x == 0) atomicAdd(acc, s);
}

static const float RPN_MIN_SIZE = 1e-3f;
struct ForwardRun {
    cald_model* m; int V; ViewDesc* views; const DetBuffers& det; float* audit_out; bool prune_ok; const FwdReuse* ru; FwdFeatures* feat; FwdSsm* ssm;
    cald_ctx* c = nullptr; hipStream_t st = nullptr; const BatchPlan* dp = nullptr;
    bool retina = false, prune = false;
    int hp[CALD_MAX_VIEWS][2], max_pix0 = 0, max_pix2 = 0, max_pix6 = 0;
    BodyBufs Fb; PyramidBufs Fp; RetinaBufs Fr; RpnBufs Fn; PruneBufs Fq; BoxBufs Fx; AuditBufs Fa;
    void layout(Bump& B) {
        const BatchPlan& P = m->plan; long long px[8];
        for (int l = 0; l < 8; l++) px[l] = level_pix(P, l, V);
        m->split.clear();
        static const bool split_on = !(getenv("CALD_H3_S16") && atoi(getenv("CALD_H3_S16")) == 0);
        SplitReg S{m, B, m->cfg.precision == CALD_PRECISION_F16X3 && split_on};
        Fb.layout(B, S, px);
        Fp.layout(B, S, px, retina);
        if (feat) return;
        if (retina) {
            int maxa = 0;
            for (int v = 0; v < V; v++) { int t = 0; for (int l = 3; l < 8; l++) t += P.seg[l][v].H * P.seg[l][v].W * 9; if (t > maxa) maxa = t; }
            Fr.layout(B, S, px, V, m->cls_out.Cout, m->cfg.num_classes, m->cfg.detections_per_img, maxa);
            return;
        }
        Fn.layout(B, px, V, m->cfg.rpn_pre_nms_top_n);
        if (m->prune) Fq.layout(B, px, V, m->prune_capture);
        Fx.layout(B, S, V, m->pred.Cout, m->cfg.num_classes, m->key_cap);
        Fa.layout(B, V, m->det_cap());
        if (ssm) ssm->out.layout(B, V, m->cfg.num_classes, m->cfg.detections_per_img);
    }
    int prepare() {
        c = m->ctx;
        if (!m->finalized) return fail(CALD_ERR_STATE, "model not finalized (call cald_model_finalize)");
        if (V < 1 || V > CALD_MAX_VIEWS) return fail(CALD_ERR_INVALID, "n_views must be 1..%d", CALD_MAX_VIEWS);
        if (feat && (audit_out || prune_ok || ru)) return fail(CALD_ERR_INVALID, "a features-only forward takes no audit, pruning or cut_out reuse");
        if (ssm && (feat || audit_out || ru || m->cfg.arch != CALD_ARCH_FRCNN)) return fail(CALD_ERR_INVALID, "the SSM forward is a plain Faster R-CNN forward");
        if (!feat && !ssm && det.cap < m->det_cap()) return fail(CALD_ERR_INVALID, "detection capacity %d < required %d", det.cap, m->det_cap());
        HIPCHK(hipSetDevice(c->device));
        for (int v = 0; v < V; v++) {
            ViewDesc& d = views[v];
            if (!d.src || d.H <= 0 || d.W <= 0 || d.nrect < 0 || d.nrect > CALD_MAX_CUT) return fail(CALD_ERR_INVALID, "view %d is malformed", v);
            int Hp, Wp;
            transform_size(d.H, d.W, m->cfg.min_size, m->cfg.max_size, &d.Hr, &d.Wr, &Hp, &Wp);
            d.Ho = d.H; d.Wo = d.W;
            if (feat && feat->pad_to) {
                const int Hq = feat->pad_to[v][0], Wq = feat->pad_to[v][1];
                if (Hq % 32 || Wq % 32 || Hq < Hp || Wq < Wp)
                    return fail(CALD_ERR_INVALID, "view %d: pad_to %d x %d must be a multiple of 32 and at least the view's own %d x %d", v, Hq, Wq, Hp, Wp);
                Hp = Hq; Wp = Wq;
            }
            hp[v][0] = Hp; hp[v][1] = Wp;
            if (Hp * Wp > max_pix0) max_pix0 = Hp * Wp;
        }
        retina = m->cfg.arch == CALD_ARCH_RETINANET;
        prune = m->prune && prune_ok;
        if (audit_out && m->box_min_size > 0.0f) return fail(CALD_ERR_UNSUPPORTED, "the decision-margin audit does not cover small-box removal (box_min_size > 0)");
        if (audit_out && (retina || m->cfg.rpn_pre_nms_top_n > 1024 || m->det_cap() > 512))
            return fail(CALD_ERR_UNSUPPORTED, "the decision-margin audit covers Faster R-CNN with rpn_pre_nms_top_n <= 1024 and <= 512 detections per image");
        build_plan(m->plan, V, views, hp, retina);
        m->last_V = V; m->last_views.assign(views, views + V);
        for (int v = 0; v < V; v++) {
            int p2 = m->plan.seg[2][v].H * m->plan.seg[2][v].W; if (p2 > max_pix2) max_pix2 = p2;
            int p6 = m->plan.seg[6][v].H * m->plan.seg[6][v].W; if (p6 > max_pix6) max_pix6 = p6;
        }
        { Bump dry(nullptr, true); layout(dry); int rc = arena_reserve(c, dry.off); if (rc) return rc; }
        { Bump real(c->arena, false); layout(real); }
        const int si = c->stage_i; c->stage_i = (si + 1) % cald_ctx::NSTAGE;
        HIPCHK(hipEventSynchronize(c->stage_ev[si]));
        memcpy(c->h_stage[si], &m->plan, sizeof(BatchPlan));
        memcpy(c->h_stage[si] + sizeof(BatchPlan), views, sizeof(ViewDesc) * V);
        HIPCHK(hipMemcpyAsync(c->d_plan, c->h_stage[si], sizeof(BatchPlan), hipMemcpyHostToDevice, c->stream));
        HIPCHK(hipMemcpyAsync(c->d_views, c->h_stage[si] + sizeof(BatchPlan), sizeof(ViewDesc) * V, hipMemcpyHostToDevice, c->stream));
        HIPCHK(hipEventRecord(c->stage_ev[si], c->stream));
        dp = c->d_plan; st = c->stream;
        m->dbg.clear();
        return 0;
    }
    int dense_block(const Bottleneck& B, const float* cur, float* dst, int lvl, int lout) {
        int rc; const float* idn = cur;
        if (B.has_down) { if ((rc = conv_on(m, B.down, cur, Fb.D, lvl, lout, V, false))) return rc; idn = Fb.D; }
        if ((rc = conv_on(m, B.c1, cur, Fb.T1, lvl, lvl, V, true))) return rc;
        return conv_pair_on(m, B.c2, B.c3, Fb.T1, Fb.T2, dst, lvl, lout, V, idn);
    }
    int gathered_block(const Bottleneck& B, int b, const float* cur, float* dst, int lvl, int lout) {
        int rc; const float* idn = cur;
        if (B.has_down) { if ((rc = gconv_on(m, B.down, cur, Fb.D, lvl, lout, V, false, nullptr, *ru, b, 0))) return rc; idn = Fb.D; }
        if ((rc = gconv_on(m, B.c1, cur, Fb.T1, lvl, lvl, V, true, nullptr, *ru, b, 1))) return rc;
        if ((rc = gconv_on(m, B.c2, Fb.T1, Fb.T2, lvl, lout, V, true, nullptr, *ru, b, 0))) return rc;
        return gconv_on(m, B.c3, Fb.T2, dst, lout, lout, V, true, idn, *ru, b, 0);
    }
    int body() {
        int rc;
        launch_preprocess(c->d_views, dp->seg[0], Fb.in0, V, max_pix0, st);
        m->dbg["input"] = {Fb.in0, 0, 4, 0};
        if ((rc = conv_on(m, m->conv1, Fb.in0, Fb.c1, 0, 1, V, true))) return rc;
        m->dbg["conv1"] = {Fb.c1, 1, 64, 0};
        launch_maxpool(Fb.c1, Fb.p1, dp->seg[1], dp->seg[2], 64, V, max_pix2, st, m->split.count(Fb.p1) != 0);
        m->dbg["pool1"] = {Fb.p1, 2, 64, 0};
        const float* cur = Fb.p1; int lvl = 2, layer = 0, xi = 0;
        for (size_t b = 0; b < m->blocks.size(); b++) {
            const Bottleneck& B = m->blocks[b];
            const int lout = lvl + (B.c2.stride == 2 ? 1 : 0);
            const bool kept = ru && (int)b < ru->nblk;
            float* dst = kept ? ru->out[b] : (B.layer_end ? Fb.Cf[layer] : Fb.X[xi]);
            if ((rc = kept && ru->mode == 2 && ru->gather[layer] ? gathered_block(B, (int)b, cur, dst, lvl, lout) : dense_block(B, cur, dst, lvl, lout))) return rc;
            if (B.layer_end) Fb.Cf[layer] = dst;
            cur = dst; lvl = lout;
            if (B.layer_end) layer++; else xi ^= 1;
        }
        const char* cn[4] = {"C2", "C3", "C4", "C5"};
        for (int i = 0; i < 4; i++) m->dbg[cn[i]] = {Fb.Cf[i], 2 + i, CCH[i], 0};
        return 0;
    }
    void name_pyramid(int first, int n) { for (int i = 0; i < n; i++) m->dbg["P" + std::to_string(first + i)] = {Fp.Pf[i], first + i, 256, 0}; }
    int fpn() {
        const int first = retina ? 3 : 2, nl = retina ? 3 : 4, c0 = 4 - nl;
        int rc; ConvSpec sp[4];
        if ((rc = conv_on(m, m->fpn_inner[nl - 1], Fb.Cf[3], Fp.inner[nl - 1], 5, 5, V, false))) return rc;
        for (int i = nl - 2; i >= 0; i--)
            if ((rc = conv_on(m, m->fpn_inner[i], Fb.Cf[c0 + i], Fp.inner[i], first + i, first + i, V, false, nullptr, Fp.inner[i + 1], first + 1 + i))) return rc;
        for (int i = 0; i < nl; i++) sp[i] = {&m->fpn_layer[i], Fp.inner[i], Fp.Pf[i], first + i, false};
        if (prune)
// ... 253 lines not shown
```

### cald_amd/csrc/host.h

```cpp
#pragma once
#include "../../include/cald_hip.h"
#include "common.h"
#include "kernels.h"
#include "host_logic.h"

#include <climits>
#include <cmath>
#include <cstdarg>
#include <cstdio>
#include <cstring>
#include <algorithm>
#include <map>
#include <string>
#include <vector>

namespace cald_host {
int fail(int code, const char* fmt, ...);
#define HIPCHK(x) do { hipError_t e_ = (x); if (e_ != hipSuccess) return fail(CALD_ERR_HIP, "%s failed: %s (%s:%d)", #x, hipGetErrorString(e_), __FILE__, __LINE__); } while (0)

struct PilCoef { int ksize; int* d_bounds; int* d_kk; };
struct PilKey { int in, out, fid; bool operator<(const PilKey& o) const { return in != o.in ? in < o.in : (out != o.out ? out < o.out : fid < o.fid); } };
struct ProfLaunch {
    hipEvent_t e0 = nullptr, e1 = nullptr;
    double flops = 0.0;
    int tag = 0;
    std::string desc;
};
}
using namespace cald_host;

#define CALD_PRUNE_LOG 4096
struct cald_ctx {
    int device = 0;
    hipStream_t stream = nullptr;
    bool own_stream = false;
    char* arena = nullptr; size_t arena_cap = 0, arena_off = 0;
    BatchPlan* d_plan = nullptr;
    ViewDesc* d_views = nullptr;
    float* d_zeros = nullptr;
    static const int NSTAGE = 8;
    char* h_stage[NSTAGE] = {nullptr}; hipEvent_t stage_ev[NSTAGE] = {nullptr}; int stage_i = 0;
    bool prof = false;
    std::vector<ProfLaunch> prof_launches;
    double prof_flops = 0.0; int64_t prof_extra_launches = 0;
    int prof_tag_now = 0;
    double prof_prune_flops_cap[2] = {0.0, 0.0};
    hipEvent_t tot0 = nullptr, tot1 = nullptr; bool tot_open = false; double tot_ms = 0.0;
    float prune_worst = 0.0f;
    long long prune_fallbacks = 0;
    float* d_prune_check = nullptr;
    unsigned long long* d_prune_stat = nullptr;
    unsigned long long* d_prune_log = nullptr; int prune_log_n = 0;
    struct GatherNote { int log; double cap[2]; };
    std::map<size_t, GatherNote> prof_gather;
    unsigned long long* d_roi_rows = nullptr; double prof_roi_rows_cap = 0.0, prof_roi_flops_cap = 0.0; long long prof_roi_views = 0;
    std::map<PilKey, PilCoef> pil;
    char* train_scratch = nullptr; size_t train_scratch_cap = 0;
    double cut_rows[3] = {0.0, 0.0, 0.0}, cut_dense[3] = {0.0, 0.0, 0.0};
    long long cut_batches = 0, cut_fallbacks = 0;
};

namespace cald_host {
struct ScopedDev {
    std::vector<void*> ptrs;
    hipStream_t st;
    explicit ScopedDev(hipStream_t s) : st(s) {}
    ~ScopedDev() { if (!ptrs.empty()) { hipStreamSynchronize(st); for (void* p : ptrs) hipFree(p); } }
    void release() { ptrs.clear(); }
    template <typename T> int alloc(T** out, size_t bytes) {
        HIPCHK(hipMalloc((void**)out, bytes ? bytes : 1));
        ptrs.push_back((void*)*out);
        return 0;
    }
    template <typename T> int upload(T** out, const void* h, size_t bytes) {
        *out = nullptr;
        if (!h) return 0;
        if (int rc = alloc(out, bytes)) return rc;
        HIPCHK(hipMemcpy((void*)*out, h, bytes, hipMemcpyHostToDevice));
        return 0;
    }
};
struct Bump {
    char* base; size_t off = 0; bool dry;
    explicit Bump(char* b, bool d) : base(b), dry(d) {}
    template <typename T> T* get(size_t count) {
        size_t bytes = (count * sizeof(T) + 255) & ~(size_t)255;
        T* p = dry ? nullptr : reinterpret_cast<T*>(base + off);
        off += bytes;
        return p;
    }
};

struct HostTensor { std::vector<float> data; std::vector<int64_t> shape; };
struct ConvLayer {
    float *w = nullptr, *w4 = nullptr, *bias = nullptr, *scale = nullptr, *shift = nullptr;
    float* wstem = nullptr;
    uint16_t* w16 = nullptr; float w16_unscale = 1.0f;
    int Cin = 0, Cout = 0, CoutPad = 0, K = 0, Kpad = 0, KH = 1, KW = 1, stride = 1, pad = 0;
    int CinTrue = 0;
};
struct Bottleneck { ConvLayer c1, c2, c3, down; bool has_down = false; bool layer_end = false; };
struct DebugEntry { const float* ptr; int level; int C; int kind; };
}

struct cald_model {
    cald_ctx* ctx = nullptr;
    cald_model_cfg cfg;
    std::map<std::string, HostTensor> sd;
    bool finalized = false;
    ConvLayer conv1; std::vector<Bottleneck> blocks;
    ConvLayer fpn_inner[4], fpn_layer[4], rpn_conv, rpn_head, fc6, fc7, pred;
    ConvLayer rpn_conv16; bool prune = false; float prune_c1[3] = {0, 0, 0}, prune_c0[3] = {0, 0, 0};
    bool prune_allowed = false;
    int look_fuse = 1; float* look_head_w = nullptr; float look_head_b[3] = {0, 0, 0};
    bool prune_bound_voided = false;
    bool prune_capture = false;
    ConvLayer p6, p7, cls_tower[4], reg_tower[4], cls_out, reg_out;
    int det_cap() const { return cfg.arch == CALD_ARCH_RETINANET ? cfg.num_classes * cfg.detections_per_img : cfg.detections_per_img; }
    float* d_anchors = nullptr;
    std::vector<void*> owned;
    std::map<std::string, DebugEntry> dbg;
    BatchPlan plan; int last_V = 0;
    struct SplitFmt { unsigned* s16; bool fp32_dead; };
    std::map<const float*, SplitFmt> split;
    std::vector<ViewDesc> last_views;
    DetBuffers sweep_det; int sweep_det_views = 0;
    DetBuffers sweep_det2; int sweep_det2_views = 0;
    struct SweepScratch {
        size_t dev_bytes = 0, pin_bytes = 0, aug_cap = 0;
        char* dev = nullptr; char* pin = nullptr; uint8_t* d_aug = nullptr;
        hipEvent_t ev_ref[2] = {nullptr, nullptr}, ev_score[2] = {nullptr, nullptr};
    } ss;
    float box_min_size = 0.0f;
    int key_cap = 32768;
    struct CutReuse {
        int mode = -1;
        char* slot[2] = {nullptr, nullptr}; size_t cap[2] = {0, 0};
        char* h_gp[2] = {nullptr, nullptr}; char* d_gp = nullptr;
    } cr;
};

namespace cald_host {
struct ConvPack {
    std::vector<float> w, w4, wstem;
    std::vector<uint16_t> w16; float w16_unscale = 1.0f;
    int Cout = 0, CoutPad = 0, K = 0, Kpad = 0;
};
struct ConvSpec { const ConvLayer* L; const float* in; float* out; int level; bool relu; const int* dyn = nullptr; const int* row_map = nullptr; const unsigned* in16 = nullptr;
                  unsigned* out16 = nullptr; float* energy4 = nullptr; };

#define CUT_MAX_BLOCKS 32
struct FwdReuse {
    int mode = 0;
    int nblk = 0;
    float* out[CUT_MAX_BLOCKS] = {};
    bool gather[3] = {false, false, false};
    const char* d_gp = nullptr;
    int tiles[CUT_MAX_BLOCKS][2] = {};
    double rows[CUT_MAX_BLOCKS][2] = {};
};
struct FwdFeatures {
    const int (*pad_to)[2] = nullptr;
    bool p7 = false;
    const float* P[5] = {}; bool split_only[5] = {}; int plan_level[5] = {};
};
struct ProposalBufs { float* proposals = nullptr; int* prop_count = nullptr; void layout(Bump& B, int V); };
struct RoiBufs { float* roi = nullptr; int* order = nullptr; void layout(Bump& B, int V, int C); };
struct PostBufs {
    float *prob = nullptr, *pmax = nullptr, *cbox = nullptr; unsigned long long* keys = nullptr; int* key_count = nullptr; int key_cap = 0;
    unsigned char* skip = nullptr;
    void layout(Bump& B, int V, int C, int key_cap);
};
struct SsmBufs {
    float *prob = nullptr, *kept_box = nullptr, *boxes = nullptr, *scores = nullptr; unsigned* vmax = nullptr; signed char* labels = nullptr;
    int *kept_prop = nullptr, *cls_count = nullptr, *row_off = nullptr, *al = nullptr, *count = nullptr, *total = nullptr;
    void layout(Bump& B, int V, int C, int cap);
};
struct FwdSsm { SsmBufs out; };
#define SSM_NMS_THR 0.3f
#define SSM_CONF_THR 0.5f
struct RetinaTailBufs {
    int *cand_count = nullptr, *kept_anchor = nullptr, *kept_count = nullptr, cand_cap = 0, max_anchors = 0; unsigned long long* cand_key = nullptr;
    float *cand_box = nullptr, *kept_box = nullptr; unsigned char* cand_skip = nullptr;
    void layout(Bump& B, int V, int K, int per_class, int max_anchors);
};
RoiArgs roi_args(const RoiBufs& S, const float* const* feat, const BatchPlan* plan, int C, int V, const ProposalBufs& P, bool out16);
PostArgs post_args(const PostBufs& S, const float* pred, int pred_ld, int C, int V, const ProposalBufs& P, const ViewDesc* views,
                   float score_thr, float nms_thr, const DetBuffers& det);
SsmArgs ssm_args(const SsmBufs& S, const float* pred, int pred_ld, int C, int V, const ProposalBufs& P, const ViewDesc* views, float score_thr, int cap);
RetinaArgs retina_args(const RetinaTailBufs& S, const float* const* cls, const float* const* reg, const BatchPlan* plan, const ViewDesc* views,
                       const float* base_anchors, int A, int K, int V, float score_thr, float nms_thr, int per_class, const DetBuffers& det);
inline size_t cut_plan_set_bytes(int V) { return (size_t)(V + 1) * sizeof(LevelSeg) + (size_t)V * sizeof(GatherSet); }
inline long long level_pix(const BatchPlan& P, int l, int V) { return P.seg[l][V].pix_off; }

int arena_reserve(cald_ctx* c, size_t bytes);
int prof_begin(cald_ctx* c, ProfLaunch& t);
int prof_end(cald_ctx* c, ProfLaunch& t, double flops, int tag, const char* fmt, ...);
int conv_refused(const ConvArgs& a);
int run_conv(cald_ctx* c, const ConvArgs& a, double flops);
int pil_resize(cald_ctx* c, const uint8_t* src, int H, int W, uint8_t* dst, int oh, int ow, uint8_t* tmp, int fid = 0);
std::vector<float> pack_w4(const std::vector<float>& w, int Kpad, int CoutPad);
void pack_conv(const std::vector<const float*>& ts, const std::vector<int>& couts, int cin, int cinp, int kh, int kw, int stride, int pad,
               bool want16, ConvPack* P);
void build_plan(BatchPlan& P, int V, const ViewDesc* views, const int (*hp)[2], bool retina);
bool stem_grid_exact(const LevelSeg* seg, int V);
int forward_model(cald_model* m, int V, ViewDesc* views, const DetBuffers& det, float* audit_out = nullptr, bool prune_ok = false,
                  const FwdReuse* ru = nullptr, FwdFeatures* feat = nullptr, FwdSsm* ssm = nullptr);
void free_det(DetBuffers& d);
int alloc_det(DetBuffers& d, int V, int cap, int C);
struct ScopedDet { DetBuffers d{}; ~ScopedDet() { free_det(d); } int alloc(int V, int cap, int C) { return alloc_det(d, V, cap, C); } };
}
```

### cald_amd/csrc/model.hip

```cpp
#include "host.h"

extern "C" int cald_model_create(cald_ctx* ctx, const cald_model_cfg* cfg, cald_model** out) {
    if (!ctx || !cfg || !out) return fail(CALD_ERR_INVALID, "null argument");
    if (cfg->arch != CALD_ARCH_FRCNN && cfg->arch != CALD_ARCH_RETINANET) return fail(CALD_ERR_INVALID, "unknown arch %d", cfg->arch);
    if (cfg->depth != 50 && cfg->depth != 101) return fail(CALD_ERR_INVALID, "depth must be 50 or 101");
    if (cfg->num_classes < 2 || cfg->num_classes > 256) return fail(CALD_ERR_INVALID, "num_classes out of range");
    if (cfg->rpn_pre_nms_top_n > 1024 || cfg->rpn_post_nms_top_n > CALD_ROI_CAP || cfg->rpn_pre_nms_top_n < 1 || cfg->rpn_post_nms_top_n < 1)
        return fail(CALD_ERR_INVALID, "rpn top-n out of range (pre <= 1024, post <= %d)", CALD_ROI_CAP);
    if (cfg->detections_per_img < 1 || cfg->detections_per_img > 1024) return fail(CALD_ERR_INVALID, "detections_per_img out of range");
    if (cfg->precision != CALD_PRECISION_FP32 && cfg->precision != CALD_PRECISION_F16X3) return fail(CALD_ERR_INVALID, "unknown precision %d", cfg->precision);
    cald_model* m = new cald_model();
    m->ctx = ctx; m->cfg = *cfg;
    {
        const float thr = cfg->box_score_thresh;
        long long per = cfg->num_classes - 1;
        if (thr > 0.0f && std::isfinite(thr)) { const long long lim = (long long)std::ceil(1.0 / (double)thr) - 1; if (lim < per) per = lim < 1 ? 1 : lim; }
        long long need = (long long)CALD_ROI_CAP * per;
        int kc = 1024; while (kc < need) kc <<= 1;
        m->key_cap = kc;
    }
    memset(&m->sweep_det, 0, sizeof(m->sweep_det)); memset(&m->sweep_det2, 0, sizeof(m->sweep_det2));
    *out = m;
    return 0;
}
// ... 144 lines not shown
            char pre[128]; snprintf(pre, sizeof(pre), "backbone.body.layer%d.%d", li + 1, bi);
            std::string p(pre);
            int stride = (bi == 0 && li > 0) ? 2 : 1;
            if ((rc = make_conv(m, B.c1, {p + ".conv1.weight"}, {}, p + ".bn1", 1, 0))) return rc;
            if ((rc = make_conv(m, B.c2, {p + ".conv2.weight"}, {}, p + ".bn2", stride, 1))) return rc;
            if ((rc = make_conv(m, B.c3, {p + ".conv3.weight"}, {}, p + ".bn3", 1, 0))) return rc;
            if (m->sd.count(p + ".downsample.0.weight")) {
                B.has_down = true;
                if ((rc = make_conv(m, B.down, {p + ".downsample.0.weight"}, {}, p + ".downsample.1", stride, 0))) return rc;
            }
            B.layer_end = (bi == nb[li] - 1);
            m->blocks.push_back(B);
        }
    const bool retina = m->cfg.arch == CALD_ARCH_RETINANET;
    if (!retina) {
    for (int i = 0; i < 4; i++) {
            char k[128];
            snprintf(k, sizeof(k), "backbone.fpn.inner_blocks.%d", i);
            if ((rc = make_conv(m, m->fpn_inner[i], {std::string(k) + ".weight"}, {std::string(k) + ".bias"}, "", 1, 0))) return rc;
            snprintf(k, sizeof(k), "backbone.fpn.layer_blocks.%d", i);
            if ((rc = make_conv(m, m->fpn_layer[i], {std::string(k) + ".weight"}, {std::string(k) + ".bias"}, "", 1, 1))) return rc;
        }
        if ((rc = make_conv(m, m->rpn_conv, {"rpn.head.conv.weight"}, {"rpn.head.conv.bias"}, "", 1, 1))) return rc;
        if ((rc = make_conv(m, m->rpn_head, {"rpn.head.cls_logits.weight", "rpn.head.bbox_pred.weight"},
                            {"rpn.head.cls_logits.bias", "rpn.head.bbox_pred.bias"}, "", 1, 0))) return rc;
        static const bool prune_env = !(getenv("CALD_RPN_PRUNE") && atoi(getenv("CALD_RPN_PRUNE")) == 0);
        if (prune_env && m->cfg.precision == CALD_PRECISION_FP32 && m->rpn_conv.Cin == 256 && m->rpn_conv.Cout == 256 && m->rpn_head.Cout == 15 &&
            m->cfg.rpn_pre_nms_top_n <= 1024) {
            if ((rc = make_conv(m, m->rpn_conv16, {"rpn.head.conv.weight"}, {"rpn.head.conv.bias"}, "", 1, 1, 0, true))) return rc;
            const HostTensor *wc, *bc, *wl;
            if ((rc = get_t(m, "rpn.head.conv.weight", &wc)) || (rc = get_t(m, "rpn.head.conv.bias", &bc)) || (rc = get_t(m, "rpn.head.cls_logits.weight", &wl))) return rc;
            const int K = 2304;
            const double u = std::ldexp(1.0, -24), gK = K * u / (1.0 - K * u);
            std::vector<double> wn(256, 0.0), wa(256, 0.0);
            for (int c = 0; c < 256; c++) {
                double q = 0.0, qa = 0.0;
                for (int ci = 0; ci < 256; ci++)
                    for (int tap = 0; tap < 9; tap++) {
                        const double t = wc->data[((size_t)c * 256 + ci) * 9 + tap];
                        const double r = (double)(K - conv_k_index(tap, ci, 9, 256));
                        q += t * t; qa += r * r * t * t;
                    }
                wn[c] = std::sqrt(q); wa[c] = std::sqrt(qa);
            }
            const double k_pos = u * (1.0 + gK) + (6.0 / 16.0) * std::ldexp(1.0, -23) * (1.0 + std::ldexp(1.0, -6));
            const double g_h = 257 * u / (1.0 - 257 * u);
            const double k_flat = 10.0 * std::ldexp(1.0, -24) * (1.0 + std::ldexp(1.0, -10)) + 3.0 * std::ldexp(1.0, -22) + 6.0 * std::ldexp(1.0, -23) * (1.0 + std::ldexp(1.0, -6)) + 2.0 * u + 2.0 * g_h;
            const int S16 = -(int)std::lround(std::log2((double)m->rpn_conv16.w16_unscale)) - 4;
            std::vector<double> w1(256, 0.0), wmax(256, 0.0);
            for (int c = 0; c < 256; c++)
                for (size_t q = 0; q < 2304; q++) { const double t = std::fabs((double)wc->data[(size_t)c * 2304 + q]); w1[c] += t; if (t > wmax[c]) wmax[c] = t; }
            const HostTensor* bl; if ((rc = get_t(m, "rpn.head.cls_logits.bias", &bl))) return rc;
            bool finite = true;
            for (int a = 0; a < 3; a++) {
                double c1 = 0.0, c0 = 0.0;
                for (int c = 0; c < 256; c++) {
                    const double v = std::fabs((double)wl->data[(size_t)a * 256 + c]);
                    c1 += v * (k_pos * wa[c] + k_flat * wn[c] + 48.0 * std::ldexp(1.0, -(25 + S16)));
                    c0 += v * (std::fabs((double)bc->data[c]) * (2.0 * u + 2.0 * g_h) + std::ldexp(1.0, -29) * w1[c] + 8640.0 * std::ldexp(1.0, -42) * wmax[c]);
                }
                c0 += 2.0 * u * std::fabs((double)bl->data[a]) * (1.0 + g_h);
                m->prune_c1[a] = (float)(1.02 * c1);
                m->prune_c0[a] = (float)(1.02 * c0);
                finite = finite && std::isfinite(m->prune_c1[a]) && std::isfinite(m->prune_c0[a]) && m->prune_c0[a] > 0.0f;
            }
            m->prune_allowed = finite && m->rpn_conv16.w16 != nullptr;
            m->prune = m->prune_allowed;
            std::vector<float> hw(wl->data.begin(), wl->data.begin() + 3 * 256);
            if ((rc = upload(m, hw, &m->look_head_w))) return rc;
            for (int a = 0; a < 3; a++) m->look_head_b[a] = bl->data[a];
        }
        {
            const HostTensor* t; if ((rc = get_t(m, "roi_heads.box_head.fc6.weight", &t))) return rc;
            if (t->shape.size() != 2 || t->shape[1] != 256 * 49) return fail(CALD_ERR_INVALID, "fc6 weight must be [N][12544]");
            HostTensor p; p.shape = {t->shape[0], t->shape[1]}; p.data.resize(t->data.size());
            int N = (int)t->shape[0];
            for (int n = 0; n < N; n++)
                for (int c = 0; c < 256; c++)
                    for (int b = 0; b < 49; b++) p.data[(size_t)n * 12544 + b * 256 + c] = t->data[(size_t)n * 12544 + c * 49 + b];
            m->sd["__fc6_perm"] = std::move(p);
            if ((rc = make_conv(m, m->fc6, {"__fc6_perm"}, {"roi_heads.box_head.fc6.bias"}, "", 1, 0))) return rc;
            m->sd.erase("__fc6_perm");
        }
        if ((rc = make_conv(m, m->fc7, {"roi_heads.box_head.fc7.weight"}, {"roi_heads.box_head.fc7.bias"}, "", 1, 0))) return rc;
        if ((rc = make_conv(m, m->pred, {"roi_heads.box_predictor.cls_score.weight", "roi_heads.box_predictor.bbox_pred.weight"},
                            {"roi_heads.box_predictor.cls_score.bias", "roi_heads.box_predictor.bbox_pred.bias"}, "", 1, 0))) return rc;
        if (m->pred.Cout != 5 * m->cfg.num_classes) return fail(CALD_ERR_INVALID, "box predictor has %d outputs, expected 5*num_classes=%d", m->pred.Cout, 5 * m->cfg.num_classes);
        {
            std::vector<float> base(5 * 3 * 4);
            const float sizes[5] = {32.f, 64.f, 128.f, 256.f, 512.f}, ratios[3] = {0.5f, 1.0f, 2.0f};
            for (int l = 0; l < 5; l++)
                for (int r = 0; r < 3; r++) {
                    float hr = sqrtf(ratios[r]), wr = 1.0f / hr;
                    float ws = wr * sizes[l], hs = hr * sizes[l];
                    float* b = &base[(l * 3 + r) * 4];
                    b[0] = rintf(-ws / 2.0f); b[1] = rintf(-hs / 2.0f); b[2] = rintf(ws / 2.0f); b[3] = rintf(hs / 2.0f);
                }
            if ((rc = upload(m, base, &m->d_anchors))) return rc;
        }
    } else {
        for (int i = 0; i < 3; i++) {
            char k[128];
            snprintf(k, sizeof(k), "backbone.fpn.inner_blocks.%d", i);
            if ((rc = make_conv(m, m->fpn_inner[i], {std::string(k) + ".weight"}, {std::string(k) + ".bias"}, "", 1, 0))) return rc;
            snprintf(k, sizeof(k), "backbone.fpn.layer_blocks.%d", i);
            if ((rc = make_conv(m, m->fpn_layer[i], {std::string(k) + ".weight"}, {std::string(k) + ".bias"}, "", 1, 1))) return rc;
        }
        if ((rc = make_conv(m, m->p6, {"backbone.fpn.extra_blocks.p6.weight"}, {"backbone.fpn.extra_blocks.p6.bias"}, "", 2, 1))) return rc;
        if ((rc = make_conv(m, m->p7, {"backbone.fpn.extra_blocks.p7.weight"}, {"backbone.fpn.extra_blocks.p7.bias"}, "", 2, 1))) return rc;
        for (int i = 0; i < 4; i++) {
            char k[128];
            snprintf(k, sizeof(k), "head.classification_head.conv.%d", 2 * i);
            if ((rc = make_conv(m, m->cls_tower[i], {std::string(k) + ".weight"}, {std::string(k) + ".bias"}, "", 1, 1))) return rc;
            snprintf(k, sizeof(k), "head.regression_head.conv.%d", 2 * i);
            if ((rc = make_conv(m, m->reg_tower[i], {std::string(k) + ".weight"}, {std::string(k) + ".bias"}, "", 1, 1))) return rc;
        }
        if ((rc = make_conv(m, m->cls_out, {"head.classification_head.cls_logits.weight"}, {"head.classification_head.cls_logits.bias"}, "", 1, 1))) return rc;
        if ((rc = make_conv(m, m->reg_out, {"head.regression_head.bbox_reg.weight"}, {"head.regression_head.bbox_reg.bias"}, "", 1, 1))) return rc;
        if (m->cls_out.Cout != 9 * m->cfg.num_classes || m->reg_out.Cout != 36)
            return fail(CALD_ERR_INVALID, "RetinaNet heads must have 9*num_classes / 36 outputs (got %d / %d)", m->cls_out.Cout, m->reg_out.Cout);
        std::vector<float> base(5 * 9 * 4);
        const float ratios[3] = {0.5f, 1.0f, 2.0f};
        for (int l = 0; l < 5; l++) {
            const int x = 32 << l;
            const float sizes[3] = {(float)x, (float)(int)((double)x * pow(2.0, 1.0 / 3)), (float)(int)((double)x * pow(2.0, 2.0 / 3))};
            for (int r = 0; r < 3; r++) {
                float hr = sqrtf(ratios[r]), wr = 1.0f / hr;
                for (int sidx = 0; sidx < 3; sidx++) {
                    float ws = wr * sizes[sidx], hs = hr * sizes[sidx];
                    float* b = &base[((l * 9) + r * 3 + sidx) * 4];
                    b[0] = rintf(-ws / 2.0f); b[1] = rintf(-hs / 2.0f); b[2] = rintf(ws / 2.0f); b[3] = rintf(hs / 2.0f);
                }
            }
        }
        if ((rc = upload(m, base, &m->d_anchors))) return rc;
    }
    m->sd.clear();
    m->finalized = true;
    return 0;
}
extern "C" int cald_model_set_rpn_prune(cald_model* m, int on, int* was) {
    if (!m) return fail(CALD_ERR_INVALID, "model is null");
    if (!m->finalized) return fail(CALD_ERR_STATE, "model not finalized");
    if (was) *was = m->prune ? 1 : 0;
    m->prune = on != 0 && m->prune_allowed;
    return 0;
}
extern "C" int cald_model_set_cutout_reuse(cald_model* m, int mode, int* was) {
    if (!m || mode < -1 || mode > 2) return fail(CALD_ERR_INVALID, "bad argument");
    if (was) *was = m->cr.mode;
    m->cr.mode = mode;
    return 0;
}
extern "C" int cald_model_set_look_fuse(cald_model* m, int mode, int* was) {
    if (!m || mode < 0 || mode > 2) return fail(CALD_ERR_INVALID, "bad argument");
    if (was) *was = m->look_fuse;
    m->look_fuse = mode;
    return 0;
}
extern "C" int cald_model_set_box_min_size(cald_model* m, float min_size, float* was) {
    if (!m || !(min_size >= 0.0f)) return fail(CALD_ERR_INVALID, "bad argument");
    if (m->cfg.arch != CALD_ARCH_FRCNN) return fail(CALD_ERR_INVALID, "box_min_size belongs to the Faster R-CNN tail (RetinaNet's always removes small boxes)");
    if (was) *was = m->box_min_size;
    m->box_min_size = min_size;
    return 0;
}
extern "C" int cald_model_set_rpn_prune_capture(cald_model* m, int on) {
    if (!m) return fail(CALD_ERR_INVALID, "model is null");
    if (on && !(m->prune && m->prune_allowed)) return fail(CALD_ERR_STATE, "certified RPN pruning is not active on this model");
    m->prune_capture = on != 0;
    return 0;
}
extern "C" int cald_model_rpn_prune_bound(cald_model* m, float* c1, float* c0) {
    if (!m || !c1 || !c0) return fail(CALD_ERR_INVALID, "null argument");
    if (!m->rpn_conv16.w16) return fail(CALD_ERR_STATE, "the model has no look-ahead layer (not an exact Faster R-CNN model)");
    for (int a = 0; a < 3; a++) { c1[a] = m->prune_c1[a]; c0[a] = m->prune_c0[a]; }
    return 0;
}
extern "C" int cald_model_set_rpn_prune_bound(cald_model* m, const float* c1, const float* c0) {
    if (!m || !c1 || !c0) return fail(CALD_ERR_INVALID, "null argument");
    if (!m->rpn_conv16.w16) return fail(CALD_ERR_STATE, "the model has no look-ahead layer (not an exact Faster R-CNN model)");
    for (int a = 0; a < 3; a++) { m->prune_c1[a] = c1[a]; m->prune_c0[a] = c0[a]; }
    m->prune_bound_voided = true;
    return 0;
}
extern "C" int cald_model_destroy(cald_model* m) {
    if (!m) return 0;
    hipSetDevice(m->ctx->device);
    hipStreamSynchronize(m->ctx->stream);
    for (void* p : m->owned) hipFree(p);
    if (m->sweep_det_views) free_det(m->sweep_det);
    if (m->sweep_det2_views) free_det(m->sweep_det2);
    if (m->ss.dev) hipFree(m->ss.dev);
    if (m->ss.pin) hipHostFree(m->ss.pin);
    if (m->ss.d_aug) hipFree(m->ss.d_aug);
    for (int i = 0; i < 2; i++) { if (m->cr.slot[i]) hipFree(m->cr.slot[i]); if (m->cr.h_gp[i]) hipHostFree(m->cr.h_gp[i]); }
    if (m->cr.d_gp) hipFree(m->cr.d_gp);
    for (int i = 0; i < 2; i++) { if (m->ss.ev_ref[i]) hipEventDestroy(m->ss.ev_ref[i]); if (m->ss.ev_score[i]) hipEventDestroy(m->ss.ev_score[i]); }
    delete m;
    return 0;
}
```

### cald_amd/csrc/ops.hip

```cpp
#include "host.h"

extern "C" int cald_op_transform_size(int H, int W, int min_size, int max_size, int* Hr, int* Wr, int* Hp, int* Wp) {
    if (H <= 0 || W <= 0 || min_size <= 0 || max_size <= 0) return fail(CALD_ERR_INVALID, "bad sizes");
    transform_size(H, W, min_size, max_size, Hr, Wr, Hp, Wp);
    return 0;
}

extern "C" int cald_op_cutout_rects(uint64_t seed, int H, int W, int N, const float* boxes, int cut_num, int* rects_out, int* n_out) {
    if (cut_num < 0 || cut_num > CALD_MAX_CUT) return fail(CALD_ERR_INVALID, "cut_num must be 0..%d", CALD_MAX_CUT);
    *n_out = cutout_rects(seed, H, W, N, boxes, cut_num, rects_out);
    return 0;
}

extern "C" int cald_op_cutout_geometry(int H, int W, int min_size, int max_size, int nrect, const int* rects, int nblk, const int* strides, int* out) {
    if (H < 1 || W < 1 || nrect < 0 || nrect > CALD_MAX_CUT || (nrect && !rects) || nblk < 0 || nblk > 64 || (nblk && !strides) || !out)
        return fail(CALD_ERR_INVALID, "bad argument");
    int Hr, Wr, Hp, Wp;
    transform_size(H, W, min_size, max_size, &Hr, &Wr, &Hp, &Wp);
    std::vector<CutSet> o(nblk + 1), t(nblk + 1);
    cut_geometry(H, W, Hr, Wr, Hp, Wp, nrect, rects, nblk, strides, &o[0], o.data() + 1, t.data() + 1);
    t[0].n = 0;
    for (int e = 0; e <= nblk; e++)
        for (int k = 0; k < 2; k++) {
            const CutSet& sset = k ? t[e] : o[e];
// ... 92 lines not shown
        if ((rc = sd.alloc(&tmp, nbytes + 256))) return rc;
        unsigned long long* lsum = reinterpret_cast<unsigned long long*>(tmp + ((nbytes + 7) & ~(size_t)7));
        launch_color_adjust(src_dev, H, W, (float)param, tmp, lsum, reinterpret_cast<uint8_t*>(dst_dev), c->stream);
        const hipError_t e = hipStreamSynchronize(c->stream);
        if (e != hipSuccess) return fail(CALD_ERR_HIP, "color adjust failed: %s", hipGetErrorString(e));
        return CALD_OK;
    }
    if (kind == CALD_AUG_ROTATE) {
        if (n_boxes < 0 || (n_boxes && (!boxes || !boxes_out))) return fail(CALD_ERR_INVALID, "rotate: null boxes");
        int fx[6], nh, nw; pil_rotate_setup(H, W, param, fx, &nh, &nw);
        uint8_t* ws;
        const size_t a = ((size_t)nh * nw * 3 + 255) & ~(size_t)255;
        if ((rc = sd.alloc(&ws, a + (size_t)nh * W * 3))) return rc;
        launch_affine_nearest(src_dev, H, W, ws, nh, nw, fx, c->stream);
        if ((rc = pil_resize(c, ws, nh, nw, reinterpret_cast<uint8_t*>(dst_dev), H, W, ws + a, 1))) return rc;
        const hipError_t e = hipStreamSynchronize(c->stream);
        if (e != hipSuccess) return fail(CALD_ERR_HIP, "rotate failed: %s", hipGetErrorString(e));
        float par[12]; rotate_box_params(H, W, param, nw, nh, par);
        rotate_boxes_host(par, boxes, n_boxes, boxes_out);
        return CALD_OK;
    }
    return fail(CALD_ERR_INVALID, "cald_op_augment: kind %d has its own entry point or needs no device work", kind);
}

static int upload_layer(ScopedDev& sd, const ConvPack& pk, const float* bias, const float* scale, const float* shift, int n, ConvArgs& a) {
    int rc;
    const float* src[3] = {bias, scale, shift}; const float** dst[3] = {&a.bias, &a.scale, &a.shift};
    for (int i = 0; i < 3; i++) {
        std::vector<float> v(pk.CoutPad, 0.0f);
        if (src[i]) std::copy(src[i], src[i] + n, v.begin());
        if ((rc = sd.upload(dst[i], src[i] ? v.data() : nullptr, v.size() * 4))) return rc;
    }
    if ((rc = sd.upload(&a.w, pk.w.data(), pk.w.size() * 4)) || (rc = sd.upload(&a.w4, pk.w4.empty() ? nullptr : pk.w4.data(), pk.w4.size() * 4)) ||
        (rc = sd.upload(&a.w16, pk.w16.empty() ? nullptr : pk.w16.data(), pk.w16.size() * 2)) ||
        (rc = sd.upload(&a.wstem, pk.wstem.empty() ? nullptr : pk.wstem.data(), pk.wstem.size() * 4))) return rc;
    a.w16_unscale = pk.w16_unscale; a.CoutPad = pk.CoutPad; a.Kpad = pk.Kpad;
    return 0;
}
static int op_conv2d(cald_ctx* c, int precision, const float* in, int H, int W, int Cin, const float* weight, int Cout, int KH, int KW,
                     int stride, int pad, const float* bias, const float* bn_scale, const float* bn_shift,
                     const float* residual, int relu, float* out) {
    if (!c || !in || !weight || !out) return fail(CALD_ERR_INVALID, "null argument");
    if (Cin % 4) return fail(CALD_ERR_INVALID, "Cin must be a multiple of 4");
    HIPCHK(hipSetDevice(c->device));
    const int Ho = (H + 2 * pad - KH) / stride + 1, Wo = (W + 2 * pad - KW) / stride + 1;
    ConvPack pk;
    pack_conv({weight}, {Cout}, Cin, Cin, KH, KW, stride, pad, precision == CALD_PRECISION_F16X3, &pk);
    pk.wstem.clear();
    BatchPlan P; memset(&P, 0, sizeof(P));
    P.seg[0][0].H = H; P.seg[0][0].W = W; P.seg[0][1].pix_off = (long long)H * W; P.seg[0][1].tile_start = (H * W + 127) / 128;
    P.seg[1][0].H = Ho; P.seg[1][0].W = Wo; P.seg[1][1].pix_off = (long long)Ho * Wo; P.seg[1][1].tile_start = (Ho * Wo + 127) / 128;
    ScopedDev sd(c->stream);
    ConvArgs a; memset(&a, 0, sizeof(a));
    BatchPlan* d_p; int rc;
    if ((rc = upload_layer(sd, pk, bias, bn_scale, bn_scale ? bn_shift : nullptr, Cout, a)) || (rc = sd.upload(&a.in, in, (size_t)H * W * Cin * 4)) ||
        (rc = sd.alloc(&a.out, (size_t)Ho * Wo * Cout * 4)) || (rc = sd.upload(&a.residual, residual, (size_t)Ho * Wo * Cout * 4)) ||
        (rc = sd.upload(&d_p, &P, sizeof(P)))) return rc;
    a.seg_in = d_p->seg[0]; a.seg_out = d_p->seg[1]; a.seg_up = d_p->seg[1];
    a.V = 1; a.Cin = Cin; a.Cout = Cout; a.KH = KH; a.KW = KW; a.stride = stride; a.pad = pad;
    a.relu = relu; a.total_mtiles = (Ho * Wo + 127) / 128; a.out_ld = Cout; a.zeros = c->d_zeros;
    const bool launched = launch_conv(a, c->stream) != nullptr;
    HIPCHK(hipGetLastError());
    HIPCHK(hipStreamSynchronize(c->stream));
    HIPCHK(hipMemcpy(out, a.out, (size_t)Ho * Wo * Cout * 4, hipMemcpyDeviceToHost));
    return launched ? 0 : conv_refused(a);
}
extern "C" int cald_op_conv2d(cald_ctx* c, const float* in, int H, int W, int Cin, const float* weight, int Cout, int KH, int KW,
                              int stride, int pad, const float* bias, const float* bn_scale, const float* bn_shift,
                              const float* residual, int relu, float* out) {
    return op_conv2d(c, CALD_PRECISION_FP32, in, H, W, Cin, weight, Cout, KH, KW, stride, pad, bias, bn_scale, bn_shift, residual, relu, out);
}
extern "C" int cald_op_conv_probe(cald_ctx* c, int precision, cald_conv_probe* pr, int n, int path, int tile, char* kernel, int kernel_cap) {
    if (!c || !pr || n < 1 || n > CALD_MAX_GROUP || !kernel || kernel_cap < 1) return fail(CALD_ERR_INVALID, "cald_op_conv_probe: bad arguments");
    if (path < CONV_AUTO || path > CONV_H4_GROUP || tile < TILE_AUTO || tile > TILE_WIDE) return fail(CALD_ERR_INVALID, "cald_op_conv_probe: bad path / tile");
    if (path == CONV_P4_FUSED && n != 2) return fail(CALD_ERR_INVALID, "cald_op_conv_probe: the fused mode takes two problems (conv2, conv3)");
    HIPCHK(hipSetDevice(c->device));
    kernel[0] = 0;
    ScopedDev sd(c->stream);
    ConvArgs a[CALD_MAX_GROUP];
    struct Back { void* dev; void* host; size_t bytes; };
    std::vector<Back> back;
    int rc;
    for (int i = 0; i < n; i++) {
        const cald_conv_probe& p = pr[i];
        if (p.V < 1 || p.V > CALD_PROBE_MAX_VIEWS || p.Cin < 4 || p.Cin % 4 || p.Cout < 1 || p.KH < 1 || p.KW < 1 || p.stride < 1 || p.pad < 0 ||
            p.out_ld < p.Cout || !p.weight || !p.in)
            return fail(CALD_ERR_INVALID, "cald_op_conv_probe: problem %d: bad layer", i);
        std::vector<LevelSeg> seg(3 * (CALD_PROBE_MAX_VIEWS + 1));
        memset(seg.data(), 0, seg.size() * sizeof(LevelSeg));
        LevelSeg* si = &seg[0]; LevelSeg* so = &seg[CALD_PROBE_MAX_VIEWS + 1]; LevelSeg* su = &seg[2 * (CALD_PROBE_MAX_VIEWS + 1)];
        std::vector<GatherSet> gs(p.V);
        long long rows_out = 0;
        for (int v = 0; v < p.V; v++) {
            const int H = p.in_hw[v][0], W = p.in_hw[v][1];
            if (H < 0 || W < 0) return fail(CALD_ERR_INVALID, "cald_op_conv_probe: negative view size");
            const int Ho = H && W ? (H + 2 * p.pad - p.KH) / p.stride + 1 : 0, Wo = H && W ? (W + 2 * p.pad - p.KW) / p.stride + 1 : 0;
            if (Ho < 0 || Wo < 0 || (H && W && (Ho < 1 || Wo < 1))) return fail(CALD_ERR_INVALID, "cald_op_conv_probe: view %d smaller than the filter", v);
            si[v].H = H; si[v].W = W; so[v].H = Ho; so[v].W = Wo; su[v].H = p.up_hw[v][0]; su[v].W = p.up_hw[v][1];
            long long m = (long long)Ho * Wo;
            if (p.gather) {
                GatherSet& g = gs[v]; memset(&g, 0, sizeof(g));
                if (p.nrect[v] < 0 || p.nrect[v] > CALD_GATHER_RECTS) return fail(CALD_ERR_INVALID, "cald_op_conv_probe: 0..%d rectangles", CALD_GATHER_RECTS);
                g.nr = p.nrect[v];
                for (int k = 0; k < g.nr; k++) {
                    const int* r = p.rect[v][k];
                    if (r[0] < 0 || r[1] < 0 || r[2] < 1 || r[3] < 1 || r[0] + r[2] > Wo || r[1] + r[3] > Ho)
                        return fail(CALD_ERR_INVALID, "cald_op_conv_probe: rectangle outside view %d", v);
                    g.x0[k] = r[0]; g.y0[k] = r[1]; g.w[k] = r[2]; g.cum[k + 1] = g.cum[k] + r[2] * r[3];
                }
                m = g.cum[g.nr];
            }
            si[v + 1].pix_off = si[v].pix_off + (long long)H * W;
            so[v + 1].pix_off = so[v].pix_off + (long long)Ho * Wo;
            su[v + 1].pix_off = su[v].pix_off + (long long)su[v].H * su[v].W;
            so[v + 1].tile_start = so[v].tile_start + (int)((m + 127) / 128);
            si[v + 1].tile_start = si[v].tile_start + (H * W + 127) / 128;
            rows_out = so[v + 1].pix_off;
        }
        const long long pix_in = si[p.V].pix_off, pix_up = su[p.V].pix_off;
        if ((p.out && p.out_n < rows_out * p.out_ld) || (p.out16 && p.out16_n < rows_out * p.out_ld) || (p.energy4 && p.energy4_n < rows_out * 4))
            return fail(CALD_ERR_INVALID, "cald_op_conv_probe: problem %d: an output buffer is smaller than the output", i);
        ConvPack pk;
        const int cin_true = p.cin_true > 0 ? p.cin_true : p.Cin;
        if (cin_true > p.Cin) return fail(CALD_ERR_INVALID, "cald_op_conv_probe: cin_true > Cin");
        pack_conv({p.weight}, {p.Cout}, cin_true, p.Cin, p.KH, p.KW, p.stride, p.pad, precision == CALD_PRECISION_F16X3, &pk);
        if (!stem_grid_exact(so, p.V)) pk.wstem.clear();
        ConvArgs& A = a[i]; memset(&A, 0, sizeof(A));
        const LevelSeg* d_seg;
        const size_t out_b = (size_t)p.out_ld * 4;
        if ((rc = upload_layer(sd, pk, p.bias, p.bn_scale, p.bn_scale ? p.bn_shift : nullptr, p.Cout, A)) ||
            (rc = sd.upload(&A.in, p.in, (size_t)pix_in * p.Cin * 4)) || (rc = sd.upload(&A.in16, p.in16, (size_t)pix_in * p.Cin * 4)) ||
            (rc = sd.upload(&A.residual, p.residual, (size_t)rows_out * out_b)) || (rc = sd.upload(&A.up, p.up, (size_t)pix_up * out_b)) ||
            (rc = sd.upload(&A.mask, p.mask, (size_t)rows_out * out_b)) || (rc = sd.upload(&A.row_map, p.row_map, (size_t)rows_out * 4)) ||
            (rc = sd.upload(&A.dyn_rows, p.has_dyn ? p.dyn_rows : nullptr, (size_t)p.V * 4)) ||
            (rc = sd.upload(&A.gather, p.gather ? gs.data() : nullptr, gs.size() * sizeof(GatherSet))) ||
            (rc = sd.upload(&d_seg, seg.data(), seg.size() * sizeof(LevelSeg))) || (rc = sd.upload(&A.out, p.out, (size_t)p.out_n * 4)) ||
            (rc = sd.upload(&A.out16, p.out16, (size_t)p.out16_n * 4)) || (rc = sd.upload(&A.energy4, p.energy4, (size_t)p.energy4_n * 4))) return rc;
        if (p.head_out) {
            if (path != CONV_H4_GROUP || !p.head_w || !p.head_b || p.head_ld < 3 || p.head_out_n < rows_out * p.head_ld)
                return fail(CALD_ERR_INVALID, "cald_op_conv_probe: problem %d: head fields need path 9, head_w, head_b, head_ld >= 3 and a buffer of the output's rows", i);
            if ((rc = sd.upload(&A.head_w, p.head_w, (size_t)3 * p.Cout * 4)) || (rc = sd.upload(&A.head_out, p.head_out, (size_t)p.head_out_n * 4))) return rc;
            for (int q = 0; q < 3; q++) A.head_b[q] = p.head_b[q];
            A.head_ld = p.head_ld;
            back.push_back({A.head_out, p.head_out, (size_t)p.head_out_n * 4});
        }
        A.seg_in = d_seg; A.seg_out = d_seg + CALD_PROBE_MAX_VIEWS + 1; A.seg_up = d_seg + 2 * (CALD_PROBE_MAX_VIEWS + 1);
        if (p.out) back.push_back({A.out, p.out, (size_t)p.out_n * 4});
        if (p.out16) back.push_back({A.out16, p.out16, (size_t)p.out16_n * 4});
        if (p.energy4) back.push_back({A.energy4, p.energy4, (size_t)p.energy4_n * 4});
        A.ex16 = p.ex16 ? 1 : 0;
        A.V = p.V; A.Cin = p.Cin; A.Cout = p.Cout;
        A.KH = p.KH; A.KW = p.KW; A.stride = p.stride; A.pad = p.pad; A.relu = p.relu ? 1 : 0; A.in_relu = p.in_relu ? 1 : 0;
        A.total_mtiles = so[p.V].tile_start; A.out_ld = p.out_ld; A.zeros = c->d_zeros;
    }
    if (path == CONV_P4_FUSED) a[1].in = a[0].out;
    const ConvForce f{path, tile};
    const char* names[CALD_MAX_GROUP] = {nullptr};
    if (path == CONV_P4_FUSED) names[0] = names[1] = launch_conv_p4_fused(a[0], a[1], c->stream);
    else if (n > 1 || path == CONV_P4_GROUP || path == CONV_H3_GROUP || path == CONV_H4_GROUP) launch_conv_group(a, n, c->stream, names, f);
    else names[0] = launch_conv(a[0], c->stream, f);
    HIPCHK(hipGetLastError());
    HIPCHK(hipStreamSynchronize(c->stream));
    std::string all;
    for (int i = 0; i < n; i++) {
        if (!names[i]) return fail(CALD_ERR_UNSUPPORTED, "cald_op_conv_probe: problem %d refused under path %d tile %d", i, path, tile);
        if (all.find(names[i]) == std::string::npos) { if (!all.empty()) all += ";"; all += names[i]; }
    }
    for (const Back& b : back) HIPCHK(hipMemcpy(b.host, b.dev, b.bytes, hipMemcpyDeviceToHost));
    snprintf(kernel, (size_t)kernel_cap, "%s", all.c_str());
    return 0;
}
void launch_mfma_f16_probe(const unsigned short* A, const unsigned short* B, const unsigned* C, unsigned* D, long long n, hipStream_t stream);
extern "C" int cald_op_mfma_f16(cald_ctx* c, const uint16_t* A, const uint16_t* B, const uint32_t* C, uint32_t* D, int64_t n) {
    if (!c || !A || !B || !C || !D || n < 1) return fail(CALD_ERR_INVALID, "cald_op_mfma_f16: null argument or n < 1");
    HIPCHK(hipSetDevice(c->device));
    ScopedDev sd(c->stream);
    const unsigned short *dA, *dB; const unsigned* dC; unsigned* dD; int rc;
    if ((rc = sd.upload(&dA, A, (size_t)n * 32)) || (rc = sd.upload(&dB, B, (size_t)n * 32)) || (rc = sd.upload(&dC, C, (size_t)n * 4)) ||
        (rc = sd.alloc(&dD, (size_t)n * 4))) return rc;
    launch_mfma_f16_probe(dA, dB, dC, dD, (long long)n, c->stream);
    HIPCHK(hipGetLastError());
    HIPCHK(hipMemcpyAsync(D, dD, (size_t)n * 4, hipMemcpyDeviceToHost, c->stream));
    HIPCHK(hipStreamSynchronize(c->stream));
    return 0;
}
extern "C" int cald_op_conv2d_f16x3(cald_ctx* c, const float* in, int H, int W, int Cin, const float* weight, int Cout, int KH, int KW,
                                    int stride, int pad, const float* bias, const float* bn_scale, const float* bn_shift,
                                    const float* residual, int relu, float* out) {
    return op_conv2d(c, CALD_PRECISION_F16X3, in, H, W, Cin, weight, Cout, KH, KW, stride, pad, bias, bn_scale, bn_shift, residual, relu, out);
}

__global__ void fill_random_kernel(float* p, long long n, unsigned seed) {
    for (long long i = blockIdx.x * (long long)blockDim.x + threadIdx.x; i < n; i += (long long)gridDim.x * blockDim.x) {
        unsigned x = (unsigned)i * 2654435761u ^ seed; x ^= x >> 15; x *= 2246822519u; x ^= x >> 13; x *= 3266489917u; x ^= x >> 16;
        p[i] = ((float)(x >> 8) * (1.0f / 8388608.0f) - 1.0f) * ((x & 7u) ? 1.0f : 0.0f);
    }
}
extern "C" int cald_op_conv_bench(cald_ctx* c, int V, int H, int W, int Cin, int Cout, int KH, int stride, int pad, int residual,
                                  int relu, int iters, int group, double* ms_out, double* tflops_out) {
    if (!c || V < 1 || V > CALD_MAX_VIEWS || iters < 1 || !ms_out || group < 1 || group > CALD_MAX_GROUP) return fail(CALD_ERR_INVALID, "bad arguments");
    if (Cin % 4) return fail(CALD_ERR_INVALID, "Cin must be a multiple of 4");
    HIPCHK(hipSetDevice(c->device));
    const int KW = KH, Ho = (H + 2 * pad - KH) / stride + 1, Wo = (W + 2 * pad - KW) / stride + 1;
    const int K = KH * KW * Cin;
    ConvPack pk; pk.CoutPad = cout_pad(Cout); pk.Kpad = round_up(K, 16);
    const int CoutPad = pk.CoutPad, Kpad = pk.Kpad;
    pk.w.assign((size_t)Kpad * CoutPad, 0.0f);
    const std::vector<float> b(CoutPad, 0.1f), sc(CoutPad, 1.0f), sh(CoutPad, 0.01f);
    unsigned r = 12345u;
    for (int k = 0; k < K; k++) for (int n = 0; n < Cout; n++) { r = r * 1664525u + 1013904223u; pk.w[(size_t)k * CoutPad + n] = ((float)(r >> 8) / 8388608.0f - 1.0f) * 0.05f; }
    if (CoutPad % 64 == 0 && ((Cin % 16 == 0 && KH * KW <= 32) || Cin == 4)) pk.w4 = pack_w4(pk.w, Kpad, CoutPad);
    BatchPlan P; memset(&P, 0, sizeof(P));
    for (int v = 0; v <= V; v++) {
        P.seg[0][v].pix_off = (long long)v * H * W; P.seg[0][v].tile_start = v * ((H * W + 127) / 128); P.seg[0][v].H = H; P.seg[0][v].W = W;
        P.seg[1][v].pix_off = (long long)v * Ho * Wo; P.seg[1][v].tile_start = v * ((Ho * Wo + 127) / 128); P.seg[1][v].H = Ho; P.seg[1][v].W = Wo;
    }
    ScopedDev sd(c->stream);
    float *d_in, *d_out, *d_res = nullptr; BatchPlan* d_p;
    const size_t n_in = (size_t)V * H * W * Cin, n_out = (size_t)V * Ho * Wo * Cout;
    ConvArgs a[CALD_MAX_GROUP]; memset(a, 0, sizeof(a));
    int rc;
    if ((rc = sd.alloc(&d_in, n_in * 4)) || (rc = sd.alloc(&d_out, n_out * 4 * group)) || (rc = upload_layer(sd, pk, b.data(), sc.data(), sh.data(), CoutPad, a[0])) ||
        (rc = sd.upload(&d_p, &P, sizeof(P)))) return rc;
    if (residual && (rc = sd.alloc(&d_res, n_out * 4))) return rc;
    hipLaunchKernelGGL(fill_random_kernel, dim3(4096), dim3(256), 0, c->stream, d_in, (long long)n_in, 1u);
    if (d_res) hipLaunchKernelGGL(fill_random_kernel, dim3(4096), dim3(256), 0, c->stream, d_res, (long long)n_out, 2u);
    a[0].in = d_in; a[0].residual = d_res; a[0].seg_in = d_p->seg[0]; a[0].seg_out = d_p->seg[1]; a[0].seg_up = d_p->seg[1]; a[0].V = V; a[0].Cin = Cin; a[0].Cout = Cout;
    a[0].KH = KH; a[0].KW = KW; a[0].stride = stride; a[0].pad = pad; a[0].relu = relu; a[0].total_mtiles = V * ((Ho * Wo + 127) / 128); a[0].out_ld = Cout; a[0].zeros = c->d_zeros;
    for (int gi = 0; gi < group; gi++) { a[gi] = a[0]; a[gi].out = d_out + (size_t)gi * n_out; }
    auto launch = [&]() { if (group > 1) launch_conv_group(a, group, c->stream); else launch_conv(a[0], c->stream); };
    launch(); launch();
    HIPCHK(hipGetLastError());
    hipEvent_t e0, e1; HIPCHK(hipEventCreate(&e0)); HIPCHK(hipEventCreate(&e1));
    HIPCHK(hipEventRecord(e0, c->stream));
    for (int i = 0; i < iters; i++) launch();
    HIPCHK(hipEventRecord(e1, c->stream));
    HIPCHK(hipEventSynchronize(e1));
    float ms = 0.f; HIPCHK(hipEventElapsedTime(&ms, e0, e1));
    hipEventDestroy(e0); hipEventDestroy(e1);
    if (const char* tp = getenv("CALD_CONV_TRACE")) {
        const size_t nblk = 1u << 17;
        unsigned long long* d_tr;
        if ((rc = sd.alloc(&d_tr, nblk * 64))) return rc;
        HIPCHK(hipMemsetAsync(d_tr, 0, nblk * 64, c->stream));
        for (int gi = 0; gi < group; gi++) a[gi].trace = d_tr;
        launch();
        HIPCHK(hipStreamSynchronize(c->stream));
        std::vector<unsigned long long> h(nblk * 8);
        HIPCHK(hipMemcpy(h.data(), d_tr, nblk * 64, hipMemcpyDeviceToHost));
        size_t used = nblk; while (used > 0 && h[(used - 1) * 8] == 0) used--;
        if (FILE* f = fopen(tp, "wb")) { fwrite(h.data(), 64, used, f); fclose(f); }
        for (int gi = 0; gi < group; gi++) a[gi].trace = nullptr;
    }
    *ms_out = (double)ms / iters;
    if (tflops_out) *tflops_out = 2.0 * (double)V * Ho * Wo * Cout * (double)K * group / (*ms_out * 1e-3) / 1e12;
    return 0;
}

extern "C" int cald_op_consistency(cald_ctx* c, int N, const float* aug_box, const float* ref_scores_cls, const float* ref_pm,
                                   int M, const float* boxes, const float* scores_cls, const float* pm, int C, float bp,
                                   float* consistency_out) {
    if (!c || !consistency_out || N < 0 || M < 0 || C < 2 || C > 256) return fail(CALD_ERR_INVALID, "bad arguments");
    if (N > 50) return fail(CALD_ERR_INVALID, "at most 50 reference boxes (cald_train.py:110-113)");
    HIPCHK(hipSetDevice(c->device));
    const int cap = (N > M ? N : M) > 0 ? (N > M ? N : M) : 1;
    ScopedDev sd(c->stream); ScopedDet sdet;
    int rc = sdet.alloc(2, cap, C); if (rc) return rc;
    const DetBuffers& d = sdet.d;
    if (N) {
        HIPCHK(hipMemcpy(d.boxes, aug_box, (size_t)N * 16, hipMemcpyHostToDevice));
        HIPCHK(hipMemcpy(d.scores_cls, ref_scores_cls, (size_t)N * C * 4, hipMemcpyHostToDevice));
        HIPCHK(hipMemcpy(d.prob_max, ref_pm, (size_t)N * 4, hipMemcpyHostToDevice));
    }
    if (M) {
        HIPCHK(hipMemcpy(d.boxes + (size_t)cap * 4, boxes, (size_t)M * 16, hipMemcpyHostToDevice));
        HIPCHK(hipMemcpy(d.scores_cls + (size_t)cap * C, scores_cls, (size_t)M * C * 4, hipMemcpyHostToDevice));
        HIPCHK(hipMemcpy(d.prob_max + cap, pm, (size_t)M * 4, hipMemcpyHostToDevice));
    }
    int counts[2] = {N, M};
    HIPCHK(hipMemcpy(d.count, counts, 8, hipMemcpyHostToDevice));
    int h[4 + 50 + 1] = {0};
    h[0] = 0; h[1] = 1; h[2] = 0; h[3] = 0;
    for (int i = 0; i < 50; i++) h[4 + i] = i;
    h[54] = N;
    int* dh; float* dpar; float* dcons;
    if ((rc = sd.upload(&dh, h, sizeof(h))) || (rc = sd.alloc(&dpar, 48)) || (rc = sd.alloc(&dcons, 4))) return rc;
    HIPCHK(hipMemset(dpar, 0, 48));
    ScoreArgs a; a.det = d; a.ref_view = dh; a.aug_view = dh + 1; a.aug_kind = dh + 2; a.pair_img = dh + 3; a.ref_sel = dh + 4; a.ref_n = dh + 54;
    a.aug_param = dpar; a.P = 1; a.bp = bp; a.cons = dcons;
    launch_consistency(a, c->stream);
    HIPCHK(hipGetLastError());
    HIPCHK(hipStreamSynchronize(c->stream));
    HIPCHK(hipMemcpy(consistency_out, dcons, 4, hipMemcpyDeviceToHost));
    return 0;
}

template <typename F> static int carve(ScopedDev& sd, F lay) {
    Bump dry(nullptr, true), real(nullptr, false); lay(dry);
    int rc = sd.alloc(&real.base, dry.off); if (rc) return rc;
    lay(real);
    return 0;
}
static int put_proposals(const ProposalBufs& P, const float* rois, int R) {
    HIPCHK(hipMemset(P.proposals, 0, (size_t)CALD_ROI_CAP * 16));
    if (R) HIPCHK(hipMemcpy(P.proposals, rois, (size_t)R * 16, hipMemcpyHostToDevice));
    HIPCHK(hipMemcpy(P.prop_count, &R, 4, hipMemcpyHostToDevice));
    return 0;
}
static int download_dets(cald_ctx* c, const DetBuffers& det, const char* what, float* boxes_out, float* scores_out, int64_t* labels_out, float* props_out,
                         float* prob_max_out, float* scores_cls_out, int* n_out) {
    HIPCHK(hipStreamSynchronize(c->stream));
    int n = 0;
    HIPCHK(hipMemcpy(&n, det.count, 4, hipMemcpyDeviceToHost));
    if (n < 0 || n > det.cap) return fail(CALD_ERR_HIP, "%s postprocess returned %d detections (cap %d)", what, n, det.cap);
    if (!n) { *n_out = 0; return 0; }
    HIPCHK(hipMemcpy(boxes_out, det.boxes, (size_t)n * 16, hipMemcpyDeviceToHost)); HIPCHK(hipMemcpy(scores_out, det.scores, (size_t)n * 4, hipMemcpyDeviceToHost));
    HIPCHK(hipMemcpy(labels_out, det.labels, (size_t)n * 8, hipMemcpyDeviceToHost)); HIPCHK(hipMemcpy(prob_max_out, det.prob_max, (size_t)n * 4, hipMemcpyDeviceToHost));
    HIPCHK(hipMemcpy(scores_cls_out, det.scores_cls, (size_t)n * det.C * 4, hipMemcpyDeviceToHost));
    if (props_out) HIPCHK(hipMemcpy(props_out, det.props, (size_t)n * 16, hipMemcpyDeviceToHost));
    *n_out = n;
    return 0;
}
// ... 231 lines not shown
```

### include/cald_hip.h

```cpp
#ifndef CALD_HIP_H
#define CALD_HIP_H
#include <stddef.h>
#include <stdint.h>
#ifdef __cplusplus
extern "C" {
#endif

typedef struct cald_ctx cald_ctx;
typedef struct cald_model cald_model;

#define CALD_OK 0
#define CALD_ERR_INVALID (-1)
#define CALD_ERR_HIP (-2)
#define CALD_ERR_STATE (-3)
#define CALD_ERR_MISSING_WEIGHT (-4)
#define CALD_ERR_UNSUPPORTED (-5)

#define CALD_PRECISION_FP32 0
#define CALD_PRECISION_F16X3 1

#define CALD_ARCH_FRCNN 0
#define CALD_ARCH_RETINANET 1

const char* cald_last_error(void);
// ... 75 lines not shown
#define CALD_MARGIN_RPN_TOPK 0
#define CALD_MARGIN_RPN_IOU 1
#define CALD_MARGIN_RPN_ORDER 2
#define CALD_MARGIN_RPN_TRUNC 3
#define CALD_MARGIN_RPN_SMALL 4
#define CALD_MARGIN_ROI_LEVEL 5
#define CALD_MARGIN_ROI_EDGE 6
#define CALD_MARGIN_POST_THR 7
#define CALD_MARGIN_POST_IOU 8
#define CALD_MARGIN_POST_ORDER 9
#define CALD_MARGIN_POST_CAP 10
#define CALD_MARGIN_REF_SUBSAMPLE 11
#define CALD_MARGIN_ARGMAX 12
#define CALD_MARGIN_ZERO_ROW 13
#define CALD_MARGIN_CUTOUT 14
int cald_sweep_audit(cald_model* m, int n_images, const uint8_t* const* images_dev, const int* H, const int* W,
                     const int64_t* pool_pos, const cald_sweep_cfg* cfg, double* consistency_out, double* cls_corr_out,
                     float* margins_out);

int cald_sweep_ltc(cald_model* m, int n_images, const uint8_t* const* images_dev, const int* H, const int* W,
                   int batch_images, double* uncertainty_out);
int cald_sweep_ssm(cald_model* m, int n_images, const uint8_t* const* images_dev, const int* H, const int* W, int batch_images,
                   int64_t rows_cap, int* al_out, int* count_out, float* boxes_out, float* scores_out, int8_t* labels_out,
                   int64_t* rows_needed_out);
int cald_sweep_lsc(cald_model* m, int n_images, const uint8_t* const* images_dev, const int* H, const int* W,
                   const int64_t* pool_pos, uint64_t base_seed, int batch_images, double* stability_out);

typedef struct cald_lossnet cald_lossnet;
int cald_lossnet_create(cald_ctx* ctx, cald_lossnet** out);
int cald_lossnet_load_tensor(cald_lossnet* ln, const char* key, const float* data, const int64_t* shape, int ndim);
int cald_lossnet_finalize(cald_lossnet* ln);
int cald_lossnet_destroy(cald_lossnet* ln);
typedef struct cald_ll_cfg {
    int batch_views;
    int levels[4];
} cald_ll_cfg;
int cald_sweep_ll(cald_model* m, cald_lossnet* ln, int n_images, const uint8_t* const* images_dev, const int* H, const int* W,
                  const int* group, const cald_ll_cfg* cfg, double* uncertainty_out, float* pooled_out);

int cald_train_gap(cald_ctx* ctx, int N, const float* const* maps, const int* level_hw, float* pooled);
typedef struct cald_lossnet_tensors {
    float* fc_w[4];
    float* fc_b[4];
    float* lin_w;
    float* lin_b;
} cald_lossnet_tensors;
int cald_lossnet_train_fwd(cald_ctx* ctx, int B, int D, const cald_lossnet_tensors* params, const float* pooled, float* hidden, float* pred);
int cald_lossnet_train_bwd(cald_ctx* ctx, int B, int D, const cald_lossnet_tensors* params, const float* pooled, const float* hidden,
                           const float* g_pred, float* gh_scratch, const cald_lossnet_tensors* grads, int accumulate, float* g_pooled);
int cald_loss_pred_loss(cald_ctx* ctx, int B, const float* input, const float* target, float margin, int per_pair, const float* g_up_dev,
                        float* loss_out, float* terms_out, float* grad_out);

typedef struct cald_vaal cald_vaal;
int cald_vaal_create(cald_ctx* ctx, cald_vaal** out);
int cald_vaal_load_tensor(cald_vaal* v, const char* key, const float* data, const int64_t* shape, int ndim);
int cald_vaal_finalize(cald_vaal* v);
int cald_vaal_destroy(cald_vaal* v);
#define CALD_VAAL_BN_BATCH 0
#define CALD_VAAL_BN_RUNNING 1
typedef struct cald_vaal_cfg {
    int bn_mode;
    int batch_images;
} cald_vaal_cfg;
int cald_sweep_vaal(cald_ctx* ctx, cald_vaal* v, int n_images, const uint8_t* const* images_dev, const int* H, const int* W,
                    const cald_vaal_cfg* cfg, float* preds_out, float* mu_out);

int cald_op_vaal_resize(cald_ctx* ctx, const uint8_t* image, int H, int W, float* out);
int cald_op_vaal_bn_relu(cald_ctx* ctx, const float* x, long long x_floats, int n, int HW, int C, const float* gamma, const float* beta,
                         float* out);
int cald_op_vaal_fc_mu(cald_vaal* v, int n, const float* act, float* mu_out);
int cald_op_vaal_head(cald_vaal* v, int n, const float* mu, float* preds_out);
int cald_op_gap(cald_ctx* ctx, const float* x, int H, int W, int C, float* mean_out);
int cald_op_lossnet(cald_lossnet* ln, int n, const float* pooled, float* out);
int cald_op_consistency(cald_ctx* ctx, int N, const float* aug_box, const float* ref_scores_cls, const float* ref_pm,
                        int M, const float* boxes, const float* scores_cls, const float* pm, int C, float bp,
                        float* consistency_out);
int cald_op_cls_corr(cald_ctx* ctx, int n, const float* scores, const int64_t* labels, int C, float* out);
int cald_op_pil_resize(cald_ctx* ctx, const uint8_t* src_dev, int H, int W, uint8_t* dst_dev, int oh, int ow);
int cald_op_cutout_rects(uint64_t seed, int H, int W, int N, const float* boxes, int cut_num, int* rects_out, int* n_out);
int cald_op_cutout_geometry(int H, int W, int min_size, int max_size, int nrect, const int* rects, int nblk, const int* strides, int* out);
int cald_op_augment(cald_ctx* ctx, int kind, double param, uint64_t seed, const uint8_t* src_dev, int H, int W,
                    int n_boxes, const float* boxes, void* dst_dev, float* boxes_out, int* aux_out);
int cald_op_noise_stream(cald_ctx* ctx, uint64_t seed, const uint8_t* src_dev, int H, int W, int nseg, const int* kinds,
                         const double* params, void* const* dsts);
int cald_op_frcnn_postprocess(cald_ctx* ctx, int R, int C, const float* logits, const float* deltas, const float* proposals,
                              int Hr, int Wr, int Ho, int Wo, float score_thr, float nms_thr, int det_max,
                              float* boxes_out, float* scores_out, int64_t* labels_out, float* props_out, float* prob_max_out,
                              float* scores_cls_out, int* n_out);
int cald_op_frcnn_postprocess_min(cald_ctx* ctx, int R, int C, const float* logits, const float* deltas, const float* proposals,
                                  int Hr, int Wr, int Ho, int Wo, float score_thr, float nms_thr, int det_max, float box_min_size,
                                  float* boxes_out, float* scores_out, int64_t* labels_out, float* props_out, float* prob_max_out,
                                  float* scores_cls_out, int* n_out);
int cald_op_ssm_postprocess(cald_ctx* ctx, int R, int C, const float* logits, const float* deltas, const float* proposals,
                            int Hr, int Wr, int Ho, int Wo, float score_thr, int det_max,
                            int* al_out, int* n_out, float* boxes_out, float* scores_out, int8_t* labels_out);
int cald_op_retina_postprocess(cald_ctx* ctx, const float* const* cls, const float* const* reg, const int* level_hw, int A, int K,
                               const float* base_anchors, int Hp, int Wp, int Hr, int Wr, int Ho, int Wo,
                               float score_thr, float nms_thr, int per_class,
                               float* boxes_out, float* scores_out, int64_t* labels_out, float* prob_max_out,
                               float* scores_cls_out, int* n_out);
#define CALD_PRUNE_PROBE_MAX_VIEWS 8
typedef struct {
    int V, guard;
    int hw[2][CALD_PRUNE_PROBE_MAX_VIEWS][2];
    int pre_n, head_ld;
    float c1[3], c0[3];
    const float* energy[2];
    const float* exact[2];
    float* head[2];
    float* pnorm[2];
    uint32_t* tau_key;
    int* row_map[2][2];
    int* nsel[2];
    float check[2];
    uint64_t stat[4];
} cald_rpn_prune_probe;
int cald_op_rpn_prune(cald_ctx* ctx, cald_rpn_prune_probe* p);
int cald_op_roi_align(cald_ctx* ctx, const float* const* feats, const int* level_hw, int C, int R, const float* rois, float* out);
int cald_op_conv2d(cald_ctx* ctx, const float* in, int H, int W, int Cin, const float* weight, int Cout, int KH, int KW,
                   int stride, int pad, const float* bias, const float* bn_scale, const float* bn_shift,
                   const float* residual, int relu, float* out);
int cald_op_conv2d_f16x3(cald_ctx* ctx, const float* in, int H, int W, int Cin, const float* weight, int Cout, int KH, int KW,
                         int stride, int pad, const float* bias, const float* bn_scale, const float* bn_shift,
                         const float* residual, int relu, float* out);
#define CALD_PROBE_MAX_VIEWS 8
#define CALD_PROBE_MAX_RECTS 8
typedef struct cald_conv_probe {
    int V;
    int in_hw[CALD_PROBE_MAX_VIEWS][2];
    int up_hw[CALD_PROBE_MAX_VIEWS][2];
    int dyn_rows[CALD_PROBE_MAX_VIEWS];
    int has_dyn;
    int gather;
    int nrect[CALD_PROBE_MAX_VIEWS];
    int rect[CALD_PROBE_MAX_VIEWS][CALD_PROBE_MAX_RECTS][4];
    int Cin, Cout, KH, KW, stride, pad, relu, in_relu, out_ld;
    int cin_true;
    const float* weight;
    const float* bias;
    const float* bn_scale;
    const float* bn_shift;
    const float* in;
    const uint32_t* in16;
    const float* residual;
    const float* up;
    int ex16;
    const float* mask;
    const int* row_map;
    float* out; int64_t out_n;
    uint32_t* out16; int64_t out16_n;
    float* energy4; int64_t energy4_n;
    const float* head_w; const float* head_b;
    float* head_out; int64_t head_out_n; int head_ld;
} cald_conv_probe;
int cald_op_conv_probe(cald_ctx* ctx, int precision, cald_conv_probe* probs, int n, int path, int tile, char* kernel, int kernel_cap);
int cald_op_mfma_f16(cald_ctx* ctx, const uint16_t* A, const uint16_t* B, const uint32_t* C, uint32_t* D, int64_t n);
int cald_op_conv_bench(cald_ctx* ctx, int n_views, int H, int W, int Cin, int Cout, int KH, int stride, int pad, int residual,
                       int relu, int iters, int group, double* ms_out, double* tflops_out);
int cald_op_transform_size(int H, int W, int min_size, int max_size, int* Hr, int* Wr, int* Hp, int* Wp);
int cald_debug_tensor(cald_model* m, const char* name, int view, float* host_out, int64_t capacity, int64_t* shape3);

#define CALD_JPEG_BASELINE 0
#define CALD_JPEG_GPU_EXTENDED 1
#define CALD_JPEG_HOST_ONLY 2
int cald_jpeg_info(const uint8_t* data, size_t size, int* H, int* W, int* ncomp);
int cald_jpeg_decode_batch(cald_ctx* ctx, int n, const uint8_t* const* data, const size_t* sizes, uint8_t* const* out_dev);
int cald_jpeg_probe(const uint8_t* data, size_t size, int* H, int* W, int* ncomp, int* kind);
int cald_jpeg_decode_batch_any(cald_ctx* ctx, int n, const uint8_t* const* data, const size_t* sizes, uint8_t* const* out_dev);
int cald_jpeg_decode_host(const uint8_t* data, size_t size, uint8_t* out_host);

int cald_profile_enable(cald_ctx* ctx, int on);
int cald_profile_read(cald_ctx* ctx, double* gemm_ms, double* gemm_flops, int64_t* gemm_launches, double* total_ms);
int cald_profile_prune(cald_ctx* ctx, double* lookahead_ms, double* lookahead_flops, double* selected_fraction_p2_p3, double* worst_bound_ratio,
                       double* pruned_flops);
int cald_profile_prune_fallbacks(cald_ctx* ctx, int64_t* n);
int cald_model_set_cutout_reuse(cald_model* m, int mode, int* was);
int cald_model_set_look_fuse(cald_model* m, int mode, int* was);
int cald_model_set_box_min_size(cald_model* m, float min_size, float* was);
int cald_profile_cutout(cald_ctx* ctx, double* rows3, double* dense_rows3, int64_t* batches, int64_t* fallbacks);
int cald_profile_roi_rows(cald_ctx* ctx, double* mean_rows_per_view, int64_t* views);
int cald_profile_dump(cald_ctx* ctx, const char* path);

int cald_train_packed_floats(int Cout, int Cin, int KH, int KW, int CinK, int mode, int64_t* floats_out);
int cald_train_pack_conv(cald_ctx* ctx, const float* weight, const float* bias, const float* bn_scale, const float* bn_shift,
                         int Cout, int Cin, int KH, int KW, int CinK, int mode, float* packed);
typedef struct cald_pack_job {
    const float *weight, *bias, *bn_scale, *bn_shift;
    int Cout, Cin, KH, KW, CinK, mode;
    float* packed;
} cald_pack_job;
typedef struct cald_pack_plan cald_pack_plan;
int cald_train_pack_plan_scratch_floats(int n, const cald_pack_job* jobs, int64_t* floats_out);
int cald_train_pack_plan_create(cald_ctx* ctx, int n, const cald_pack_job* jobs, float* scratch, int64_t scratch_floats, cald_pack_plan** plan_out);
int cald_train_pack_plan_run(cald_ctx* ctx, const cald_pack_plan* plan);
int cald_train_pack_plan_destroy(cald_pack_plan* plan);
int cald_train_conv(cald_ctx* ctx, int N, int H, int W, const float* in, int CinK, const float* packed, int Cout, int Cin,
                    int KH, int KW, int stride, int pad, int mode, int flags, const float* residual, const float* up,
                    int Hup, int Wup, const float* mask, float* out, int out_ld);
int cald_train_conv_group(cald_ctx* ctx, int n, int N, const int* hw, const float* const* ins, int CinK, const float* const* packed,
                          int Cout, int Cin, int KH, int KW, int stride, int pad, int mode, int flags, const float* const* masks,
                          float* const* outs, int out_ld);
int cald_train_conv_wgrad(cald_ctx* ctx, int N, int H, int W, const float* x, int Cin, int ldx, const float* g, int Cout, int ldg,
                          int KH, int KW, int stride, int pad, const float* row_scale, float* dw, float* db, int accumulate);
int cald_train_linear_wgrad(cald_ctx* ctx, int R, const float* x, int K, const float* g, int Cout, int ldg, int taps,
                            float* dw, float* db, int accumulate);
enum { CALD_WGRAD_POINTWISE = 0, CALD_WGRAD_TABLE = 1, CALD_WGRAD_GENERAL = 2, CALD_WGRAD_GENERAL32 = 3, CALD_WGRAD_WIDE = 4 };
enum { CALD_WGRAD_REDUCE_FLAT = 0, CALD_WGRAD_REDUCE_TAPS = 1 };
typedef struct cald_wgrad_plan {
    int variant, reduce;
    int MT, JT;
    long long S, chunk;
    long long csplit, rows_per_block;
    long long scratch_bytes;
    char kernel[48], reduce_kernel[32];
} cald_wgrad_plan;
int cald_train_wgrad_plan(long long Q, int N, int H, int W, int Cin, int ldx, int Cout, int ldg, int KH, int KW, int stride, int pad,
                          int red_taps, cald_wgrad_plan* out);
int cald_train_relu_bwd(cald_ctx* ctx, long long rows, int C, float* g, const float* act, const float* scale);
int cald_train_add(cald_ctx* ctx, long long n, float* dst, const float* a, const float* b);
int cald_train_dilate(cald_ctx* ctx, int N, int Ho, int Wo, int C, int s, int Hd, int Wd, const float* g, float* out);
int cald_train_upsample_bwd(cald_ctx* ctx, int N, int Hf, int Wf, int Hc, int Wc, int C, const float* fine, float* coarse);
int cald_train_rpn_proposals(cald_ctx* ctx, int N, int Hp, int Wp, const int* image_sizes, const float* const* heads,
                             const int* level_hw, int head_ld, int pre_n, int post_n, float nms_thr, float min_size,
                             float* proposals_out, int* counts_out);
int cald_train_roi_sample_host(int N, const int* slots, const int* n_gt, const int* counts, const int32_t* matched,
                               const int64_t* gt_labels, const double* keys, int batch, double pos_fraction, int pred_ld, int num_classes,
                               int64_t* keep_rows, int64_t* gt_sel, int64_t* labels_out, float* img_col, int64_t* pos_rows,
                               int64_t* pred_idx, int* R_out, int* n_pos_out, int* per_image_out);
int cald_train_roi_gather(cald_ctx* ctx, const float* table, const float* gts, const int64_t* idx, int cap, int R, int n_pos,
                          float wx, float wy, float ww, float wh, float* rois_out, float* box_tgt_out);
int cald_train_anchors(cald_ctx* ctx, int kind, int Hp, int Wp, const int* level_hw, float* anchors_out);
int cald_train_match(cald_ctx* ctx, int n_boxes, const float* boxes, int n_gt, const float* gt, float hi, float lo,
                     int allow_low_quality, int* matched_out, float* best_iou_out);
int cald_train_box_encode(cald_ctx* ctx, int n, const float* reference, const float* proposals, float wx, float wy, float ww,
                          float wh, float* out);
int cald_train_roi_align(cald_ctx* ctx, const float* const* feats, const int* level_hw, int C, int R, const float* rois, float* out);
int cald_train_roi_align_bwd(cald_ctx* ctx, int N, float* const* gfeats, const int* level_hw, int C, int R, const float* rois,
                             const float* gout);
int cald_train_softmax_ce(cald_ctx* ctx, int R, int C, int ld, const float* logits, const int64_t* labels, float gscale,
                          float* loss_out, float* grad_out);
int cald_train_smooth_l1(cald_ctx* ctx, int n, const float* pred, const int64_t* idx, const float* target, float beta, float denom,
                         const float* weights, float gscale, float* loss_out, float* grad);
int cald_train_focal_loss(cald_ctx* ctx, int N, const int* level_pix, int A, int K, int ld, const float* logits, const int* matched,
                          const int64_t* gt_labels, const int* gt_off, const float* img_weight, float alpha, float gscale,
                          float* loss_out, float* grad);
int cald_train_bce_logits(cald_ctx* ctx, int n, const float* logits, const int64_t* idx, const float* labels, float gscale,
                          float* loss_out, float* grad);
int cald_train_softmax_ce_seg(cald_ctx* ctx, int N, const int* seg_off, int C, int ld, const float* logits, const int64_t* labels,
                              const float* gscale, float* loss_out, float* grad_out);
int cald_train_smooth_l1_seg(cald_ctx* ctx, int N, const int* seg_off, const float* pred, const int64_t* idx, const float* target, float beta,
                             const float* denom, const float* gscale, float* loss_out, float* grad);
int cald_train_bce_logits_seg(cald_ctx* ctx, int N, const int* seg_off, const float* logits, const int64_t* idx, const float* labels,
                              const float* gscale, float* loss_out, float* grad);
int cald_train_focal_loss_seg(cald_ctx* ctx, int N, const int* level_pix, int A, int K, int ld, const float* logits, const int* matched,
                              const int64_t* gt_labels, const int* gt_off, const float* denom, float alpha, const float* gscale,
                              float* loss_out, float* mean_out, float* grad);
int cald_train_seg_mean(cald_ctx* ctx, int N, const float* losses, float* mean_out);
int cald_train_add_bcast(cald_ctx* ctx, int N, long long HW, int C, float* dst, const float* a, const float* b, const float* g,
                         long long g_stride);
int cald_train_preprocess(cald_ctx* ctx, int N, const uint8_t* const* images, const float* const* remainders, const int* hw,
                          int Hp, int Wp, float* out);
int cald_train_maxpool(cald_ctx* ctx, int N, int H, int W, int C, const float* in, float* out);
int cald_train_subsample2(cald_ctx* ctx, int N, int H, int W, int C, const float* in, float* out);
int cald_train_sgd(cald_ctx* ctx, long long n, float* param, const float* grad, float* momentum_buf, float lr, float momentum,
                   float weight_decay, int first_step);
typedef struct cald_comm cald_comm;
int cald_comm_unique_id(void* id128_out);
int cald_comm_init_rank(cald_ctx* ctx, const void* id128, int world_size, int rank, cald_comm** out);
int cald_comm_adopt(cald_ctx* ctx, void* rccl_comm, cald_comm** out);
int cald_comm_info(const cald_comm* comm, int* world_size, int* rank);
int cald_comm_destroy(cald_comm* comm);
int cald_allgather_scores(cald_comm* comm, const double* send_dev, double* recv_dev, int64_t rows_per_rank, int row_len);

int cald_train_seg_cache_size(void);

#ifdef __cplusplus
}
#endif
#endif
```

Measured before the change: 173.3.

## Pack conv row tiles across views to eliminate per-view tail padding

Convolution M-tiles in the p4 kernel now cover the concatenated pixel rows of all views as one packed range, so a 128-row tile may straddle view boundaries. Before, each view was padded up to a tile boundary. Straddling tiles resolve each row's view on the fly, with per-row input offsets, tap strides and upsample source lookups. This removes the partially empty tail tiles in each view's tiling, at the cost of extra per-row index math and a slower generic addressing path in straddling tiles. Packing is on by default, can be turned off with an env var or a model setter, and is skipped for masked, gathered, dynamic-row and Cin=4 convs.

```diff
diff --git a/cald_amd/_ffi.py b/cald_amd/_ffi.py
--- a/cald_amd/_ffi.py
+++ b/cald_amd/_ffi.py
@@ -87,7 +87,8 @@
                 ("residual", c_f), ("up", c_f), ("ex16", C.c_int), ("mask", c_f), ("row_map", c_i),
                 ("out", c_f), ("out_n", C.c_int64), ("out16", C.POINTER(C.c_uint32)), ("out16_n", C.c_int64),
                 ("energy4", c_f), ("energy4_n", C.c_int64),
-                ("head_w", c_f), ("head_b", c_f), ("head_out", c_f), ("head_out_n", C.c_int64), ("head_ld", C.c_int)]
+                ("head_w", c_f), ("head_b", c_f), ("head_out", c_f), ("head_out_n", C.c_int64), ("head_ld", C.c_int),
+                ("row_packing", C.c_int)]
 
 
 PRUNE_PROBE_MAX_VIEWS = 8
@@ -174,6 +175,7 @@
     "cald_op_conv2d_f16x3": (C.c_int, [C.c_void_p, c_f, C.c_int, C.c_int, C.c_int, c_f, C.c_int, C.c_int, C.c_int, C.c_int,
                                        C.c_int, c_f, c_f, c_f, c_f, C.c_int, c_f]),
     "cald_op_conv_bench": (C.c_int, [C.c_void_p] + [C.c_int] * 12 + [c_d, c_d]),
+    "cald_op_row_pack_lookup": (C.c_int, [C.c_int, c_i, c_i, C.c_int, C.c_int, C.c_int64, c_i64, c_i, c_i64, c_i64]),
     "cald_op_transform_size": (C.c_int, [C.c_int, C.c_int, C.c_int, C.c_int, c_i, c_i, c_i, c_i]),
     "cald_debug_tensor": (C.c_int, [C.c_void_p, C.c_char_p, C.c_int, c_f, C.c_int64, c_i64]),
     "cald_jpeg_info": (C.c_int, [C.c_void_p, C.c_size_t, c_i, c_i, c_i]),
@@ -188,6 +190,7 @@
     "cald_profile_cutout": (C.c_int, [C.c_void_p, c_d, c_d, c_i64, c_i64]),
     "cald_model_set_cutout_reuse": (C.c_int, [C.c_void_p, C.c_int, c_i]),
     "cald_model_set_look_fuse": (C.c_int, [C.c_void_p, C.c_int, c_i]),
+    "cald_model_set_row_packing": (C.c_int, [C.c_void_p, C.c_int, c_i]),
     "cald_model_set_box_min_size": (C.c_int, [C.c_void_p, C.c_float, c_f]),
     "cald_profile_dump": (C.c_int, [C.c_void_p, C.c_char_p]),
     "cald_train_packed_floats": (C.c_int, [C.c_int] * 6 + [c_i64]),
diff --git a/cald_amd/csrc/common.h b/cald_amd/csrc/common.h
--- a/cald_amd/csrc/common.h
+++ b/cald_amd/csrc/common.h
@@ -24,7 +24,32 @@
     }
     return lo;
 }
+__host__ __device__ __forceinline__ int seg_find_row(const LevelSeg* __restrict__ seg, const int V, const long long row) {
+    int lo = 0, hi = V - 1;
+    while (lo < hi) {
+        const int mid = (lo + hi + 1) >> 1;
+        if (seg[mid].pix_off <= row) lo = mid; else hi = mid - 1;
+    }
+    return lo;
+}
 #endif
+
+static inline int conv_pack_rows(const LevelSeg* si, const LevelSeg* so, const LevelSeg* su, int V, int Cin, int out_ld) {
+    const long long total = so[V].pix_off, LIM = 0x7FFE0000LL - (1 << 16);
+    if (V < 1 || total < 1 || total > 0x7FFFFFFFLL - 128) return 0;
+    int vf = 0;
+    for (int v = 0; v < V; v++) {
+        const long long b = so[v].pix_off, e = so[v + 1].pix_off;
+        if (e == b) continue;
+        if ((e - b + 128) * out_ld * 4 > LIM) return 0;
+        if (b % 128 == 0) continue;
+        const long long t0 = b / 128 * 128;
+        while (so[vf + 1].pix_off <= t0) vf++;
+        if ((si[v + 1].pix_off - si[vf].pix_off) * Cin * 4 > LIM) return 0;
+        if (su && (su[v + 1].pix_off - su[vf].pix_off) * out_ld * 4 > LIM) return 0;
+    }
+    return (int)total;
+}
 
 struct BatchPlan {
     LevelSeg seg[CALD_MAX_LEVELS][CALD_MAX_VIEWS + 1];
@@ -80,6 +105,7 @@
     float head_b[3];
     float* head_out;
     int head_ld;
+    int packed_rows;
 };
 
 #define CALD_MAX_GROUP 10
diff --git a/cald_amd/csrc/conv_p4.hip b/cald_amd/csrc/conv_p4.hip
--- a/cald_amd/csrc/conv_p4.hip
+++ b/cald_amd/csrc/conv_p4.hip
@@ -6,7 +6,7 @@
 
 template <int EPI, bool MASK, int TM, int TN, bool GATHER = false>
 __device__ __forceinline__ void p4_epilogue(const ConvArgs& a, const f32x16 (&acc)[TM][TN], float* smem, const int v, const LevelSeg& so,
-                                            const int m0, const int Mv, const int n0) {
+                                            const int m0, const int Mv, const int n0, const bool straddle = false) {
     constexpr int BM = 128, WN = 2;
     const int tid = threadIdx.x, lane = tid & 63, wave = tid >> 6;
     const int wm = wave / WN, wn = wave % WN;
@@ -17,9 +17,11 @@
     const float* __restrict__ ex_v = nullptr;
     int upH = 1, upW = 1;
     float uph_s = 0.f, upw_s = 0.f;
+    long long up_off = 0;
     if (EPI == 1) ex_v = a.residual + so.pix_off * (long long)out_ld;
     if (EPI == 2) {
         const LevelSeg su = a.seg_up[v];
+        up_off = su.pix_off;
         ex_v = a.up + su.pix_off * (long long)out_ld;
         upH = su.H; upW = su.W;
         uph_s = (float)upH / (float)Ho; upw_s = (float)upW / (float)Wo;
@@ -41,6 +43,20 @@
             int m = m0 + tid;
             if (GATHER) {
                 s_src[tid] = m < Mv ? gather_pixel(a.gather[v], m, Wo) * row_b : 0x7FFF0000;
+            } else if (EPI == 2 && straddle) {
+                int src = 0;
+                if (m < Mv) {
+                    const long long r = so.pix_off + m;
+                    int vr = v;
+                    while (vr + 1 < a.V && a.seg_out[vr + 1].pix_off <= r) vr++;
+                    const LevelSeg sor = a.seg_out[vr], sur = a.seg_up[vr];
+                    const int ml = (int)(r - sor.pix_off), oy = ml / sor.W, ox = ml - oy * sor.W;
+                    const float hs = (float)sur.H / (float)sor.H, ws = (float)sur.W / (float)sor.W;
+                    int sy = (int)floorf((float)oy * hs); sy = sy > sur.H - 1 ? sur.H - 1 : sy;
+                    int sx = (int)floorf((float)ox * ws); sx = sx > sur.W - 1 ? sur.W - 1 : sx;
+                    src = ((int)(sur.pix_off - up_off) + sy * sur.W + sx) * out_ld * 4;
+                }
+                s_src[tid] = src;
             } else {
                 m = m < Mlast ? m : Mlast;
                 const int oy = m / Wo, ox = m - oy * Wo;
@@ -232,14 +248,24 @@
         else { const int r = b - MT8 * NT; mt = MT8 + r / NT; nt = r % NT; }
     }
     const int n0 = nt * BN;
-    const int v = seg_find_view(a.seg_out, a.V, mt);
+    constexpr bool CAN_PACK = !C4 && !MASK && !FUSE && !GATHER;
+    const bool packed = CAN_PACK && a.packed_rows != 0;
+    const int v = packed ? seg_find_row(a.seg_out, a.V, (long long)mt * BM) : seg_find_view(a.seg_out, a.V, mt);
     const LevelSeg so = a.seg_out[v];
     const LevelSeg si = a.seg_in[v];
     const int Ho = so.H, Wo = so.W, Hi = si.H, Wi = si.W;
     int Mv = Ho * Wo;
     if (a.dyn_rows) { const int d = a.dyn_rows[v]; Mv = d < Mv ? d : Mv; }
     if (GATHER) Mv = a.gather[v].cum[a.gather[v].nr];
-    const int m0 = (mt - so.tile_start) * BM;
+    int m0 = (mt - so.tile_start) * BM;
+    bool straddle = false;
+    if (CAN_PACK && packed) {
+        const int row0 = mt * BM, left = a.packed_rows - row0;
+        m0 = row0 - (int)so.pix_off;
+        const int end = m0 + (left < BM ? left : BM);
+        straddle = end > Mv;
+        Mv = end;
+    }
     if (m0 >= Mv) return;
     const float* __restrict__ in_v = a.in + si.pix_off * (long long)a.Cin;
     const int Cin = a.Cin, KW = a.KW, KH = a.KH, CoutPad = a.CoutPad;
@@ -248,25 +274,36 @@
     const int g = tid & 3, arow = tid >> 2;
     unsigned rowmask[2];
     int rowvoff[2], riy0[2], rix0[2];
+    int tapw[2] = {0, 0};
 #pragma unroll
     for (int p = 0; p < 2; p++) {
         const int m = m0 + arow + 64 * p;
-        const int mp = GATHER ? (m < Mv ? gather_pixel(a.gather[v], m, Wo) : 0) : (a.row_map && m < Mv) ? a.row_map[so.pix_off + m] : m;
-        const int oy = mp / Wo, ox = mp - oy * Wo;
+        int ml = m, Wo_r = Wo, Hi_r = Hi, Wi_r = Wi, dpix = 0;
+        if (CAN_PACK && straddle && m < Mv) {
+            const long long r = so.pix_off + m;
+            int vr = v;
+            while (vr + 1 < a.V && a.seg_out[vr + 1].pix_off <= r) vr++;
+            const LevelSeg sor = a.seg_out[vr], sir = a.seg_in[vr];
+            ml = (int)(r - sor.pix_off); Wo_r = sor.W; Hi_r = sir.H; Wi_r = sir.W; dpix = (int)(sir.pix_off - si.pix_off);
+        }
+        const int mp = GATHER ? (m < Mv ? gather_pixel(a.gather[v], m, Wo) : 0) : (a.row_map && m < Mv) ? a.row_map[so.pix_off + m] : ml;
+        const int oy = mp / Wo_r, ox = mp - oy * Wo_r;
         const int iy0 = oy * a.stride - a.pad, ix0 = ox * a.stride - a.pad;
         unsigned msk = 0;
         if (!C4 && m < Mv)
             for (int t = 0; t < KH * KW; t++) {
                 const int th = t / KW, tw = t - th * KW;
                 const int iy = iy0 + th, ix = ix0 + tw;
-                if (iy >= 0 && iy < Hi && ix >= 0 && ix < Wi) msk |= 1u << t;
+                if (iy >= 0 && iy < Hi_r && ix >= 0 && ix < Wi_r) msk |= 1u << t;
             }
         rowmask[p] = msk;
         rowvoff[p] = (((oy * a.stride) * Wi + ox * a.stride) * Cin + (C4 ? 0 : 4 * g)) * 4;
+        if (CAN_PACK && straddle) { rowvoff[p] = ((dpix + iy0 * Wi_r + ix0) * Cin + 4 * g) * 4; tapw[p] = Wi_r; }
         riy0[p] = m < Mv ? iy0 : -0x40000000; rix0[p] = ix0;
     }
+    const int Wi_s = straddle ? 0 : Wi, Cin_s = straddle ? 0 : Cin, cin_v4 = straddle ? Cin * 4 : 0;
     const __amdgpu_buffer_rsrc_t rsA = __builtin_amdgcn_make_buffer_rsrc(
-        (void*)(in_v - (long long)a.pad * (Wi + 1) * Cin), 0, 0x7FFE0000, 0x00020000);
+        (void*)(in_v - (straddle ? 0ll : (long long)a.pad * (Wi + 1) * Cin)), 0, 0x7FFE0000, 0x00020000);
     const __amdgpu_buffer_rsrc_t rsB = __builtin_amdgcn_make_buffer_rsrc((void*)(a.w4 + (long long)n0 * 8), 0, 0x7FFE0000, 0x00020000);
     int u_kh = 0, u_kw = 0, u_ci = 0, u_kt = 0;
     const int a_kq = g >> 1, a_j = 2 * (g & 1);
@@ -298,9 +335,10 @@
             v1 = ok1 ? rowvoff[1] + toff : 0x7FFF0000;                                                     \
         } else {                                                                                           \
             const unsigned u_bit = 1u << (u_kh * KW + u_kw);                                               \
-            soffA = ((u_kh * Wi + u_kw) * Cin + u_ci) * 4;                                                 \
-            v0 = (rowmask[0] & u_bit) ? rowvoff[0] : 0x7FFF0000;                                           \
-            v1 = (rowmask[1] & u_bit) ? rowvoff[1] : 0x7FFF0000;                                           \
+            soffA = ((u_kh * Wi_s + u_kw) * Cin_s + u_ci) * 4;                                             \
+                          \
+            v0 = (rowmask[0] & u_bit) ? rowvoff[0] + (CAN_PACK ? (u_kh * tapw[0] + u_kw) * cin_v4 : 0) : 0x7FFF0000; \
+            v1 = (rowmask[1] & u_bit) ? rowvoff[1] + (CAN_PACK ? (u_kh * tapw[1] + u_kw) * cin_v4 : 0) : 0x7FFF0000; \
         }                                                                                                  \
         ra0 = __builtin_bit_cast(f32x4, __builtin_amdgcn_raw_buffer_load_b128(rsA, v0, soffA, 0));         \
         ra1 = __builtin_bit_cast(f32x4, __builtin_amdgcn_raw_buffer_load_b128(rsA, v1, soffA, 0));         \
@@ -349,6 +387,13 @@
         for (int p = 0; p < 2; p++)
 #pragma unroll
             for (int t = 0; t < (TAPS > 0 ? TAPS : 1); t++) voffA[p][t] = ((rowmask[p] >> t) & 1u) ? rowvoff[p] : 0x7FFF0000;
+        if (CAN_PACK && TAPS == 9 && straddle) {
+#pragma unroll
+            for (int p = 0; p < 2; p++)
+#pragma unroll
+                for (int t = 0; t < 9; t++)
+                    if ((rowmask[p] >> t) & 1u) voffA[p][t < TAPS ? t : 0] = rowvoff[p] + ((t / 3) * tapw[p] + t % 3) * cin_v4;
+        }
     }
     if (TAPS == 0) {
         P4_LOAD();
@@ -358,7 +403,7 @@
 #define U_LOAD0(T)                                                                                         \
     {                                                                                                      \
         const int soffB = u_kt * 2 * CoutPad * 8 * 4;                                                      \
-        const int soffA = (TAPS == 9 ? ((((T) / 3) * Wi + ((T) % 3)) * Cin + ci_ld) : ci_ld) * 4;          \
+        const int soffA = (TAPS == 9 ? ((((T) / 3) * Wi_s + ((T) % 3)) * Cin_s + ci_ld) : ci_ld) * 4;      \
         ra0 = __builtin_bit_cast(f32x4, __builtin_amdgcn_raw_buffer_load_b128(rsA, voffA[0][T], soffA, 0)); \
         ra1 = __builtin_bit_cast(f32x4, __builtin_amdgcn_raw_buffer_load_b128(rsA, voffA[1][T], soffA, 0)); \
         rb0 = __builtin_bit_cast(f32x4, __builtin_amdgcn_raw_buffer_load_b128(rsB, bvoff0, soffB, 0));     \
@@ -439,7 +484,7 @@
 #define U_LOAD(T)                                                                                          \
     {                                                                                                      \
         const int soffB = u_kt * 2 * CoutPad * 8 * 4;                                                      \
-        const int soffA = (TAPS == 9 ? ((((T) / 3) * Wi + ((T) % 3)) * Cin + ci_ld) : ci_ld) * 4;          \
+        const int soffA = (TAPS == 9 ? ((((T) / 3) * Wi_s + ((T) % 3)) * Cin_s + ci_ld) : ci_ld) * 4;      \
         ra0 = __builtin_bit_cast(f32x4, __builtin_amdgcn_raw_buffer_load_b128(rsA, voffA[0][T], soffA, 0)); \
         ra1 = __builtin_bit_cast(f32x4, __builtin_amdgcn_raw_buffer_load_b128(rsA, voffA[1][T], soffA, 0)); \
         rb0 = __builtin_bit_cast(f32x4, __builtin_amdgcn_raw_buffer_load_b128(rsB, bvoff0, soffB, 0));     \
@@ -609,7 +654,7 @@
             }
         }
     } else {
-        p4_epilogue<EPI, MASK, TM, TN, GATHER>(a, acc, smem, v, so, m0, Mv, n0);
+        p4_epilogue<EPI, MASK, TM, TN, GATHER>(a, acc, smem, v, so, m0, Mv, n0, CAN_PACK && straddle);
     }
     if (trace && tid == 0) {
         trace[3] = __builtin_amdgcn_s_memtime();
@@ -651,6 +696,12 @@
     return !(a.energy4 && !wide);
 }
 
+static inline ConvArgs p4_tiled(ConvArgs a) {
+    if (a.packed_rows > 0 && a.Cin != 4 && !a.dyn_rows && !a.row_map && !a.gather && !a.mask) a.total_mtiles = (a.packed_rows + 127) / 128;
+    else a.packed_rows = 0;
+    return a;
+}
+
 #define P4_NAME(K, EPIV, C4V, TNV, TAPSV) K "<" #EPIV "," #C4V "," #TNV "," #TAPSV ">"
 template <int EPI, bool C4, int TN, int TAPS>
 static const char* p4_go(const dim3 grid, hipStream_t stream, const ConvArgs& a, const char* name) {
@@ -668,7 +719,7 @@
     const bool wide = f.tile == TILE_NARROW ? false : p[0].CoutPad % 128 == 0;
     ConvGroup g; g.n = n; int blk = 0;
     for (int i = 0; i < n; i++) {
-        const ConvArgs& a = p[i];
+        const ConvArgs a = p4_tiled(p[i]);
         if (p4_refuses(a) || !p4_tile_ok(a, wide, f) || (a.CoutPad % 128 == 0) != (p[0].CoutPad % 128 == 0)) return nullptr;
         if (a.Cin % 16 != 0 || a.KH * a.KW > 32 || a.residual || a.up || a.gather) return nullptr;
         if ((a.mask != nullptr) != (p[0].mask != nullptr)) return nullptr;
@@ -701,7 +752,8 @@
     return "conv_p4_fused_kernel";
 }
 
-const char* launch_conv_p4(const ConvArgs& a, hipStream_t stream, ConvForce f) {
+const char* launch_conv_p4(const ConvArgs& a_in, hipStream_t stream, ConvForce f) {
+    const ConvArgs a = p4_tiled(a_in);
     if (p4_refuses(a)) return nullptr;
     bool wide = a.CoutPad % 128 == 0;
     if (wide) {
diff --git a/cald_amd/csrc/forward.hip b/cald_amd/csrc/forward.hip
--- a/cald_amd/csrc/forward.hip
+++ b/cald_amd/csrc/forward.hip
@@ -174,7 +174,7 @@
     a.dyn_rows = dyn; a.row_map = nullptr; a.gather = nullptr; a.V = V;
     a.Cin = L.Cin; a.Cout = L.Cout; a.CoutPad = L.CoutPad; a.Kpad = L.Kpad;
     a.KH = L.KH; a.KW = L.KW; a.stride = L.stride; a.pad = L.pad; a.relu = relu ? 1 : 0;
-    a.total_mtiles = level_tiles(m->plan, lout, V);
+    a.total_mtiles = level_tiles(m->plan, lout, V); a.packed_rows = 0;
     a.out_ld = L.Cout; a.in_relu = in_relu ? 1 : 0; a.zeros = m->ctx->d_zeros;
     a.mask = nullptr;
     for (int v = 0; v < V; v++) {
@@ -209,12 +209,21 @@
     a.wstem = L.wstem && stem_grid_exact(m->plan.seg[lout], V) ? L.wstem : nullptr;
     return 2.0 * (double)level_pix(m->plan, lout, V) * (double)L.Cout * (double)(L.KH * L.KW * L.CinTrue);
 }
+bool cald_host::conv_pack_default() {
+    static const bool on = !(getenv("CALD_CONV_PACK") && atoi(getenv("CALD_CONV_PACK")) == 0);
+    return on;
+}
+static void offer_packing(cald_model* m, ConvArgs& a, int lin, int lout, int lup, int V) {
+    if (!(m->row_packing < 0 ? conv_pack_default() : m->row_packing != 0) || a.dyn_rows || a.row_map || a.gather || a.mask) return;
+    a.packed_rows = conv_pack_rows(m->plan.seg[lin], m->plan.seg[lout], a.up ? m->plan.seg[lup] : nullptr, V, a.Cin, a.out_ld);
+}
 static int conv_on(cald_model* m, const ConvLayer& L, const float* in, float* out, int lin, int lout, int V, bool relu,
                    const float* residual = nullptr, const float* up = nullptr, int lup = 0, const int* dyn = nullptr,
                    bool in_relu = false) {
     ConvArgs a;
     const double flops = fill_conv_args(m, a, L, in, out, lin, lout, V, relu, residual, up, lup, dyn, in_relu);
     if (flops < 0.0) return (int)flops;
+    offer_packing(m, a, lin, lout, lup, V);
     return run_conv(m->ctx, a, flops);
 }
 static int conv_pair_on(cald_model* m, const ConvLayer& L2, const ConvLayer& L3, const float* in, float* mid, float* out, int lin, int lout,
@@ -245,6 +254,7 @@
         if (sp[i].in16) a[i].in16 = sp[i].in16;
         if (sp[i].out16) a[i].out16 = sp[i].out16;
         a[i].energy4 = sp[i].energy4;
+        offer_packing(m, a[i], sp[i].level, sp[i].level, 0, V);
         flops += f; tiles += a[i].total_mtiles;
     }
     cald_ctx* c = m->ctx;
diff --git a/cald_amd/csrc/host.h b/cald_amd/csrc/host.h
--- a/cald_amd/csrc/host.h
+++ b/cald_amd/csrc/host.h
@@ -113,6 +113,7 @@
     ConvLayer rpn_conv16; bool prune = false; float prune_c1[3] = {0, 0, 0}, prune_c0[3] = {0, 0, 0};
     bool prune_allowed = false;
     int look_fuse = 1; float* look_head_w = nullptr; float look_head_b[3] = {0, 0, 0};
+    int row_packing = -1;
     bool prune_bound_voided = false;
     bool prune_capture = false;
     ConvLayer p6, p7, cls_tower[4], reg_tower[4], cls_out, reg_out;
@@ -204,6 +205,7 @@
                bool want16, ConvPack* P);
 void build_plan(BatchPlan& P, int V, const ViewDesc* views, const int (*hp)[2], bool retina);
 bool stem_grid_exact(const LevelSeg* seg, int V);
+bool conv_pack_default();
 int forward_model(cald_model* m, int V, ViewDesc* views, const DetBuffers& det, float* audit_out = nullptr, bool prune_ok = false,
                   const FwdReuse* ru = nullptr, FwdFeatures* feat = nullptr, FwdSsm* ssm = nullptr);
 void free_det(DetBuffers& d);
diff --git a/cald_amd/csrc/model.hip b/cald_amd/csrc/model.hip
--- a/cald_amd/csrc/model.hip
+++ b/cald_amd/csrc/model.hip
@@ -320,6 +320,12 @@
     m->cr.mode = mode;
     return 0;
 }
+extern "C" int cald_model_set_row_packing(cald_model* m, int mode, int* was) {
+    if (!m || mode < -1 || mode > 1) return fail(CALD_ERR_INVALID, "bad argument");
+    if (was) *was = m->row_packing;
+    m->row_packing = mode;
+    return 0;
+}
 extern "C" int cald_model_set_look_fuse(cald_model* m, int mode, int* was) {
     if (!m || mode < 0 || mode > 2) return fail(CALD_ERR_INVALID, "bad argument");
     if (was) *was = m->look_fuse;
diff --git a/cald_amd/csrc/ops.hip b/cald_amd/csrc/ops.hip
--- a/cald_amd/csrc/ops.hip
+++ b/cald_amd/csrc/ops.hip
@@ -268,6 +268,11 @@
         A.V = p.V; A.Cin = p.Cin; A.Cout = p.Cout;
         A.KH = p.KH; A.KW = p.KW; A.stride = p.stride; A.pad = p.pad; A.relu = p.relu ? 1 : 0; A.in_relu = p.in_relu ? 1 : 0;
         A.total_mtiles = so[p.V].tile_start; A.out_ld = p.out_ld; A.zeros = c->d_zeros;
+        if (p.row_packing < CALD_PROBE_PACK_AUTO || p.row_packing > CALD_PROBE_PACK_ON) return fail(CALD_ERR_INVALID, "cald_op_conv_probe: problem %d: bad row_packing", i);
+        const bool packable = !p.has_dyn && !p.row_map && !p.gather && !p.mask && p.Cin != 4 && path != CONV_P4_FUSED;
+        if (packable && (p.row_packing == CALD_PROBE_PACK_ON || (p.row_packing == CALD_PROBE_PACK_AUTO && conv_pack_default())))
+            A.packed_rows = conv_pack_rows(si, so, p.up ? su : nullptr, p.V, p.Cin, p.out_ld);
+        if (p.row_packing == CALD_PROBE_PACK_ON && !A.packed_rows) return fail(CALD_ERR_INVALID, "cald_op_conv_probe: problem %d cannot run on packed row tiles", i);
     }
     if (path == CONV_P4_FUSED) a[1].in = a[0].out;
     const ConvForce f{path, tile};
@@ -284,6 +289,26 @@
     }
     for (const Back& b : back) HIPCHK(hipMemcpy(b.host, b.dev, b.bytes, hipMemcpyDeviceToHost));
     snprintf(kernel, (size_t)kernel_cap, "%s", all.c_str());
+    return 0;
+}
+extern "C" int cald_op_row_pack_lookup(int V, const int* in_hw, const int* out_hw, int Cin, int out_ld, int64_t n, const int64_t* rows,
+                                       int* view_out, int64_t* local_out, int64_t* packed_rows_out) {
+    if (V < 1 || V > CALD_MAX_VIEWS || !in_hw || !out_hw || n < 0 || (n && (!rows || !view_out || !local_out)))
+        return fail(CALD_ERR_INVALID, "cald_op_row_pack_lookup: bad arguments");
+    std::vector<LevelSeg> si(V + 1), so(V + 1);
+    memset(si.data(), 0, si.size() * sizeof(LevelSeg)); memset(so.data(), 0, so.size() * sizeof(LevelSeg));
+    for (int v = 0; v < V; v++) {
+        if (in_hw[2 * v] < 0 || in_hw[2 * v + 1] < 0 || out_hw[2 * v] < 0 || out_hw[2 * v + 1] < 0) return fail(CALD_ERR_INVALID, "cald_op_row_pack_lookup: negative size");
+        si[v].H = in_hw[2 * v]; si[v].W = in_hw[2 * v + 1]; so[v].H = out_hw[2 * v]; so[v].W = out_hw[2 * v + 1];
+        si[v + 1].pix_off = si[v].pix_off + (long long)si[v].H * si[v].W;
+        so[v + 1].pix_off = so[v].pix_off + (long long)so[v].H * so[v].W;
+    }
+    for (int64_t i = 0; i < n; i++) {
+        if (rows[i] < 0 || rows[i] >= so[V].pix_off) return fail(CALD_ERR_INVALID, "cald_op_row_pack_lookup: row %lld outside the level", (long long)rows[i]);
+        const int v = seg_find_row(so.data(), V, rows[i]);
+        view_out[i] = v; local_out[i] = rows[i] - so[v].pix_off;
+    }
+    if (packed_rows_out) *packed_rows_out = conv_pack_rows(si.data(), so.data(), nullptr, V, Cin, out_ld);
     return 0;
 }
 void launch_mfma_f16_probe(const unsigned short* A, const unsigned short* B, const unsigned* C, unsigned* D, long long n, hipStream_t stream);
diff --git a/include/cald_hip.h b/include/cald_hip.h
--- a/include/cald_hip.h
+++ b/include/cald_hip.h
@@ -251,8 +251,14 @@
     float* energy4; int64_t energy4_n;
     const float* head_w; const float* head_b;
     float* head_out; int64_t head_out_n; int head_ld;
+    int row_packing;
 } cald_conv_probe;
+#define CALD_PROBE_PACK_AUTO 0
+#define CALD_PROBE_PACK_OFF 1
+#define CALD_PROBE_PACK_ON 2
 int cald_op_conv_probe(cald_ctx* ctx, int precision, cald_conv_probe* probs, int n, int path, int tile, char* kernel, int kernel_cap);
+int cald_op_row_pack_lookup(int V, const int* in_hw, const int* out_hw, int Cin, int out_ld, int64_t n, const int64_t* rows,
+                            int* view_out, int64_t* local_out, int64_t* packed_rows_out);
 int cald_op_mfma_f16(cald_ctx* ctx, const uint16_t* A, const uint16_t* B, const uint32_t* C, uint32_t* D, int64_t n);
 int cald_op_conv_bench(cald_ctx* ctx, int n_views, int H, int W, int Cin, int Cout, int KH, int stride, int pad, int residual,
                        int relu, int iters, int group, double* ms_out, double* tflops_out);
@@ -275,6 +281,7 @@
 int cald_profile_prune_fallbacks(cald_ctx* ctx, int64_t* n);
 int cald_model_set_cutout_reuse(cald_model* m, int mode, int* was);
 int cald_model_set_look_fuse(cald_model* m, int mode, int* was);
+int cald_model_set_row_packing(cald_model* m, int mode, int* was);
 int cald_model_set_box_min_size(cald_model* m, float min_size, float* was);
 int cald_profile_cutout(cald_ctx* ctx, double* rows3, double* dense_rows3, int64_t* batches, int64_t* fallbacks);
 int cald_profile_roi_rows(cald_ctx* ctx, double* mean_rows_per_view, int64_t* views);
```

New measurement: 175.2 (median of 6 runs). +1.1%, better.
